# DEEPDIP-project/IncompressibleNavierStokes.jl

Measured on AMD Instinct MI355X. Metric: M lattice-cell updates/sec (RK4 step incl. Poisson), 3D TGV fp64, higher is better.
Workload: dtype f64; 1 GPU; TaylorGreenVortex3D 256^3 periodic fp64, RK44 + spectral Poisson, dt=0.001, Re=1e3; decomposition=single GPU, loop=timesteps_ (K steps, one native call)

## Files before the change

incompressiblenavierstokes.jl_amd/csrc/ins_fast3d_flux.hip:

```cpp
#include <algorithm>
#include <cstdlib>

#include "ins_internal.h"


namespace {

__global__ __launch_bounds__(256) void k_build_recs(GridDev g, double visc, Rec* __restrict__ r0, Rec* __restrict__ r1,
                                                    Rec* __restrict__ r2, int diffusion_only) {
  const int d = blockIdx.y;
  Rec* out = d == 0 ? r0 : (d == 1 ? r1 : r2);
  const int n = g.N[d];
  for (int idx = blockIdx.x * 256 + threadIdx.x; idx < n; idx += gridDim.x * 256) {
    const int ip = min(idx + 1, n - 1);
    Rec r;
    r.vs = visc * g.mdx[d][ip];
    r.vo = visc * g.mdxu[d][idx];
    r.a0 = 0.5 * g.A2[0][d][idx];
    r.b0 = 0.5 * g.A1[0][d][ip];
    r.a1 = 0.5 * g.A2[1][d][idx];
    r.b1 = 0.5 * g.A1[1][d][ip];
    r.a2 = 0.5 * g.A2[2][d][idx];
    r.b2 = 0.5 * g.A1[2][d][ip];
    r.rs = g.rdxu[d][idx];
// ... 334 lines not shown
      load_plane(B, k + 2);
      load_p(Pa, k + 3);
      if (bar) __builtin_amdgcn_s_barrier();
      body(Cc, A, k);
      if (++k >= k1) break;
      correct(B, Pb, Pa, k + 1);
      load_plane(Cc, k + 2);
      load_p(Pb, k + 3);
      if (bar) __builtin_amdgcn_s_barrier();
      body(A, B, k);
      if (++k >= k1) break;
    }
  }
}

__global__ __launch_bounds__(256) void k_zero_shell(GridDev g, double* __restrict__ F) {
  const int N0 = g.N[0], N1 = g.N[1], N2 = g.N[2];
  const long long nface_z = (long long)N0 * N1, nface_y = (long long)N0 * N2, nface_x = (long long)N1 * N2;
  const long long total = 2 * (nface_z + nface_y + nface_x);
  for (long long t = (long long)blockIdx.x * 256 + threadIdx.x; t < total; t += (long long)gridDim.x * 256) {
    long long r = t;
    long long c;
    if (r < 2 * nface_z) {
      const int side = r >= nface_z;
      r -= side * nface_z;
      c = r + (side ? (long long)(N2 - 1) * g.sx[2] : 0);
    } else if ((r -= 2 * nface_z) < 2 * nface_y) {
      const int side = r >= nface_y;
      r -= side * nface_y;
      const int ii = (int)(r % N0), kk = (int)(r / N0);
      c = ii + (side ? (long long)(N1 - 1) * g.sx[1] : 0) + kk * g.sx[2];
    } else {
      r -= 2 * nface_y;
      const int side = r >= nface_x;
      r -= side * nface_x;
      const int jj = (int)(r % N1), kk = (int)(r / N1);
      c = (side ? N0 - 1 : 0) + jj * g.sx[1] + kk * g.sx[2];
    }
    F[c] = 0.0;
    F[c + g.sc] = 0.0;
    F[c + 2 * g.sc] = 0.0;
  }
}

}

#define g_rows ((int)ins_opt(OPT_INS_FLUX_ROWS))
#define g_zchunk ((int)ins_opt(OPT_INS_FLUX_ZC))
#define g_xw ((int)ins_opt(OPT_INS_FLUX_XW))

extern "C" void ins_tune_flux3d(int rows, int zchunk, int xw) {
  ins_set_option("INS_FLUX_ROWS", (rows >= 2 && rows <= 4) ? rows : 0);
  ins_set_option("INS_FLUX_ZC", zchunk >= 1 ? zchunk : 0);
  ins_set_option("INS_FLUX_XW", (xw == 1 || xw == 2 || xw == 4) ? xw : 0);
}

int ins_flux3d_prepare(const ins_grid* G, double visc, hipStream_t s) {
  ins_grid* M = const_cast<ins_grid*>(G);
  const GridDev& g = G->g;
  if (!M->rec_dev) {
    const size_t n = (size_t)g.N[0] + g.N[1] + g.N[2];
    INS_HIP_TRY(hipMalloc(&M->rec_dev, n * sizeof(Rec)));
    M->rec_visc = -1.0;
  }
  if (M->rec_visc != visc) {
    Rec* r0 = reinterpret_cast<Rec*>(M->rec_dev);
    Rec* r1 = r0 + g.N[0];
    Rec* r2 = r1 + g.N[1];
    const int nmax = std::max(g.N[0], std::max(g.N[1], g.N[2]));
    hipLaunchKernelGGL(k_build_recs, dim3(cdiv(nmax, 256), 3), dim3(256), 0, s, g, visc, r0, r1, r2, 0);
    INS_LAUNCH_CHECK();
    M->rec_visc = visc;
  }
  return INS_OK;
}

template <int R, int XW, bool FUSE>
static int launch_flux(const ins_grid* G, const double* u, double* F, const RkEpi& epi, const double* pI, int corr_mode, hipStream_t s,
                       const void* recs = nullptr) {
  const GridDev& g = G->g;
  const Rec* r0 = reinterpret_cast<const Rec*>(recs ? recs : G->rec_dev);
  const Rec* r1 = r0 + g.N[0];
  const Rec* r2 = r1 + g.N[1];
  const int zc = g_zchunk ? g_zchunk : ((g.N[2] >= 384 || (pI && corr_mode == 3 && g.N[2] >= 128)) ? 8 : 4);
  const int bar = ins_opt(OPT_INS_FLUX_BAR) ? 1 : 0;
  const bool corr = pI != nullptr;
  const bool masked = !G->all_dof;
  constexpr int RC = R > 3 ? 3 : R;
  constexpr int RK = R > 2 ? 2 : R;
  const int reff = corr ? RK : (masked ? RC : R);
  const int xo = corr ? XOUT - 1 : XOUT;
  const int ntx = cdiv(g.N[0] - 2, xo * XW), nty = cdiv(g.N[1] - 2, (4 / XW) * reff), ntz = cdiv(g.N[2] - 2, zc);
  dim3 block(64, 4, 1);
  const unsigned nb = (unsigned)(8LL * ntx * ((nty + 7) / 8) * ntz);
  if (corr && corr_mode == 3) {
    if constexpr (FUSE) {
      constexpr int R3 = R > 2 ? 2 : R;
      const int nty3 = cdiv(g.N[1] - 2, (4 / XW) * R3), ntx3 = cdiv(g.N[0] - 2, (XOUT - 1) * XW);
      const unsigned nb3 = (unsigned)(8LL * ntx3 * ((nty3 + 7) / 8) * ntz);
      hipLaunchKernelGGL((k_momentum_flux<R3, false, true, XW, true, 3>), dim3(nb3), block, 0, s, g, r0, r1, r2, u, F, zc, ntx3, nty3, ntz, epi, pI, bar);
      INS_LAUNCH_CHECK();
      return INS_OK;
    } else {
      ins_set_error("in-kernel pressure correction needs the fused epilogue");
      return INS_ERR_UNSUPPORTED;
    }
  } else if (corr) {
    if (!(FUSE && G->uniform_exact && !masked)) {
      ins_set_error("in-kernel pressure correction needs the fused path on an exactly uniform periodic grid");
      return INS_ERR_UNSUPPORTED;
    }
    if constexpr (FUSE)
      {
        if (corr_mode == 2)
          hipLaunchKernelGGL((k_momentum_flux<RK, true, false, XW, true, 2>), dim3(nb), block, 0, s, g, r0, r1, r2, u, F, zc, ntx, nty, ntz, epi, pI, bar);
        else
          hipLaunchKernelGGL((k_momentum_flux<RK, true, false, XW, true, 1>), dim3(nb), block, 0, s, g, r0, r1, r2, u, F, zc, ntx, nty, ntz, epi, pI, bar);
      }
  } else if (G->uniform_exact && !masked)
    hipLaunchKernelGGL((k_momentum_flux<R, true, false, XW, FUSE, 0>), dim3(nb), block, 0, s, g, r0, r1, r2, u, F, zc, ntx, nty, ntz, epi, pI, bar);
  else if (!masked)
    hipLaunchKernelGGL((k_momentum_flux<R, false, false, XW, FUSE, 0>), dim3(nb), block, 0, s, g, r0, r1, r2, u, F, zc, ntx, nty, ntz, epi, pI, bar);
  else
    hipLaunchKernelGGL((k_momentum_flux<RC, false, true, XW, FUSE, 0>), dim3(nb), block, 0, s, g, r0, r1, r2, u, F, zc, ntx, nty, ntz, epi, pI, bar);
  INS_LAUNCH_CHECK();
  return INS_OK;
}

template <bool FUSE>
static int launch_flux_any(const ins_grid* G, const double* u, double* F, const RkEpi& epi, const double* pI, int corr_mode, hipStream_t s,
                           const void* recs = nullptr) {
  const int waves_x = cdiv(G->g.N[0] - 2, pI ? XOUT - 1 : XOUT);
  int xw = g_xw;
  if (!xw) {
    xw = waves_x >= 8 ? 4 : (waves_x >= 2 ? 2 : 1);
    while (xw > 1 && cdiv(waves_x, xw) * xw > waves_x) xw >>= 1;
  }
  const int rows = g_rows ? g_rows : 4;
#define INS_FLUX_CASE(RR)                                                          \
  if (rows == RR) {                                                                \
    if (xw == 4) return launch_flux<RR, 4, FUSE>(G, u, F, epi, pI, corr_mode, s, recs);  \
    if (xw == 2) return launch_flux<RR, 2, FUSE>(G, u, F, epi, pI, corr_mode, s, recs);  \
    return launch_flux<RR, 1, FUSE>(G, u, F, epi, pI, corr_mode, s, recs);               \
  }
  INS_FLUX_CASE(2)
  INS_FLUX_CASE(3)
  INS_FLUX_CASE(4)
#undef INS_FLUX_CASE
  return INS_ERR_INVALID;
}

bool ins_flux64_supported(const ins_grid* G);
int ins_k_flux64(const ins_grid* G, double visc, const double* u, double* F, const RkEpi* epi, const double* pI, int corr_mode, hipStream_t s,
                 int part = 0);

int ins_k_momentum_flux3d(const ins_grid* G, double visc, const double* u, double* F, bool zero_shell, hipStream_t s) {
  int rc;
  const long long from62 = ins_opt(OPT_INS_FLUX64_62_FROM);
  if (ins_flux64_supported(G) && (from62 <= 0 || G->g.N[0] - 2 < from62)) {
    if ((rc = ins_k_flux64(G, visc, u, F, nullptr, nullptr, 0, s))) return rc;
  } else {
    if ((rc = ins_flux3d_prepare(G, visc, s))) return rc;
    RkEpi epi;
    memset(&epi, 0, sizeof(epi));
    if ((rc = launch_flux_any<false>(G, u, F, epi, nullptr, 0, s))) return rc;
  }
  if (zero_shell) {
    const GridDev& g = G->g;
    const long long total = 2LL * ((long long)g.N[0] * g.N[1] + (long long)g.N[0] * g.N[2] + (long long)g.N[1] * g.N[2]);
    hipLaunchKernelGGL(k_zero_shell, dim3((unsigned)std::min<long long>((total + 255) / 256, 2048)), dim3(256), 0, s, g, F);
    INS_LAUNCH_CHECK();
  }
  return INS_OK;
}

bool ins_fast3d_supported(const ins_grid* G);
int ins_k_diffusion_flux3d(const ins_grid* G, double visc, const double* u, double* F, bool zero_shell, hipStream_t s) {
  const GridDev& g = G->g;
  if (!ins_fast3d_supported(G)) return INS_ERR_UNSUPPORTED;
  ins_grid* M = const_cast<ins_grid*>(G);
  if (!M->rec_diff_dev) {
    const size_t n = (size_t)g.N[0] + g.N[1] + g.N[2];
    INS_HIP_TRY(hipMalloc(&M->rec_diff_dev, n * sizeof(Rec)));
    M->rec_diff_visc = -1.0;
  }
  if (M->rec_diff_visc != visc) {
    Rec* r0 = reinterpret_cast<Rec*>(M->rec_diff_dev);
    Rec* r1 = r0 + g.N[0];
    Rec* r2 = r1 + g.N[1];
    const int nmax = std::max(g.N[0], std::max(g.N[1], g.N[2]));
    hipLaunchKernelGGL(k_build_recs, dim3(cdiv(nmax, 256), 3), dim3(256), 0, s, g, visc, r0, r1, r2, 1);
    INS_LAUNCH_CHECK();
    M->rec_diff_visc = visc;
  }
  RkEpi epi;
  memset(&epi, 0, sizeof(epi));
  int rc = launch_flux_any<false>(G, u, F, epi, nullptr, 0, s, M->rec_diff_dev);
  if (rc || !zero_shell) return rc;
  const long long total = 2LL * ((long long)g.N[0] * g.N[1] + (long long)g.N[0] * g.N[2] + (long long)g.N[1] * g.N[2]);
  hipLaunchKernelGGL(k_zero_shell, dim3((unsigned)std::min<long long>((total + 255) / 256, 2048)), dim3(256), 0, s, g, F);
  INS_LAUNCH_CHECK();
  return INS_OK;
}

bool ins_flux64m_supported(const ins_grid* G);
int ins_k_flux64m(const ins_grid* G, double visc, const double* u, double* k_out, const RkEpi& epi, const double* p_padded, hipStream_t s);

int ins_k_momentum_rk_fused(const ins_grid* G, double visc, const double* u_in, double* k_out, const RkEpi& epi, hipStream_t s) {
  if (ins_flux64_supported(G)) return ins_k_flux64(G, visc, u_in, k_out, &epi, nullptr, 0, s);
  if ((!ins_opt(OPT_INS_FLUX64M_SKIP_FIRST) || epi.wout) && ins_flux64m_supported(G)) return ins_k_flux64m(G, visc, u_in, k_out, epi, nullptr, s);
  int rc = ins_flux3d_prepare(G, visc, s);
  if (rc) return rc;
  return launch_flux_any<true>(G, u_in, k_out, epi, nullptr, 0, s);
}

int ins_k_momentum_rk_fused_corr(const ins_grid* G, double visc, const double* ustar_prev, const double* pI, double* k_out, const RkEpi& epi,
                                 hipStream_t s) {
  if (ins_flux64_supported(G)) return ins_k_flux64(G, visc, ustar_prev, k_out, &epi, pI, 1, s);
  int rc = ins_flux3d_prepare(G, visc, s);
  if (rc) return rc;
  return launch_flux_any<true>(G, ustar_prev, k_out, epi, pI, 1, s);
}

bool ins_fast3d_supported(const ins_grid* G);
bool ins_corr3_supported(const ins_grid* G) {
  const GridDev& g = G->g;
  if (g.D != 3 || !ins_fast3d_supported(G) || g.N[0] < 8 || g.N[1] < 8 || g.N[2] < 8) return false;
  for (int a = 0; a < 3; ++a)
    for (int sd = 0; sd < 2; ++sd)
      if (g.bc[a][sd] != INS_BC_PERIODIC && g.bc[a][sd] != INS_BC_DIRICHLET) return false;
  return true;
}
int ins_k_momentum_rk_fused_corr3(const ins_grid* G, double visc, const double* ustar_prev, const double* p_padded, double* k_out, const RkEpi& epi,
                                  hipStream_t s) {
  if (ins_flux64m_supported(G)) return ins_k_flux64m(G, visc, ustar_prev, k_out, epi, p_padded, s);
  int rc = ins_flux3d_prepare(G, visc, s);
  if (rc) return rc;
  return launch_flux_any<true>(G, ustar_prev, k_out, epi, p_padded, 3, s);
}

int ins_k_momentum_rk_fused_corr_slab(const ins_grid* G, double visc, const double* ustar_prev, const double* p_ext, double* k_out,
                                      const RkEpi& epi, hipStream_t s, int part) {
  if (ins_flux64_supported(G)) return ins_k_flux64(G, visc, ustar_prev, k_out, &epi, p_ext, 2, s, part);
  if (part == 1) return INS_OK;
  int rc = ins_flux3d_prepare(G, visc, s);
  if (rc) return rc;
  return launch_flux_any<true>(G, ustar_prev, k_out, epi, p_ext, 2, s);
}
```

incompressiblenavierstokes.jl_amd/csrc/ins_fft.hip:

```cpp
#include <cmath>

#include "ins_internal.h"

namespace {

template <typename C>
struct real_of;
template <>
struct real_of<double2> {
  using t = double;
};
template <>
struct real_of<float2> {
  using t = float;
};
template <typename C>
using real_t = typename real_of<C>::t;
template <typename C>
__device__ __forceinline__ C mkc(real_t<C> x, real_t<C> y) {
  C c;
  c.x = x;
  c.y = y;
  return c;
}
template <typename C>
__device__ __forceinline__ C cmul(C a, C b) { return mkc<C>(a.x * b.x - a.y * b.y, a.x * b.y + a.y * b.x); }
template <typename C>
__device__ __forceinline__ C cmulc(C a, C b) { return mkc<C>(a.x * b.x + a.y * b.y, a.y * b.x - a.x * b.y); }
template <typename C>
__device__ __forceinline__ C cadd(C a, C b) { return mkc<C>(a.x + b.x, a.y + b.y); }
template <typename C>
__device__ __forceinline__ C csub(C a, C b) { return mkc<C>(a.x - b.x, a.y - b.y); }
template <typename C>
__device__ __forceinline__ C mul_mi(C a) { return mkc<C>(a.y, -a.x); }
template <typename C>
__device__ __forceinline__ C mul_pi(C a) { return mkc<C>(-a.y, a.x); }

constexpr int fft_r3(int code) { return code >= 64 ? 5 : (code >= 32 ? 3 : 1); }
constexpr int fft_lg(int code) { return code & 31; }
constexpr int fft_len(int code) { return fft_r3(code) << fft_lg(code); }

template <int LOGN>
__host__ __device__ __forceinline__ int pos_of_freq(int k) {
  constexpr int LG = fft_lg(LOGN), R3 = fft_r3(LOGN);
  constexpr bool ODD = LG & 1;
  int p = 0, L = 1 << LG;
  if (R3 != 1) {
    p = (k % R3) * L;
    k /= R3;
  }
  if (ODD) {
    p += (k & 1) * (L / 2);
    k >>= 1;
    L /= 2;
  }
#pragma unroll
  for (int s = 0; s < LG / 2; ++s) {
    p += (k & 3) * (L / 4);
    k >>= 2;
    L /= 4;
  }
  return p;
}

template <int LOGN>
constexpr bool fft_swz_on() { return fft_r3(LOGN) == 1 && fft_len(LOGN) % 256 == 0; }
template <bool ON>
__host__ __device__ __forceinline__ int fft_swz(int i) {
  return ON ? ((i & ~15) | ((i + ((i >> 4) & 3) + 4 * ((i >> 6) & 3)) & 15)) : i;
}
__device__ __forceinline__ int fft_swz_g(int gg) { return (gg & ~15) | ((gg & 3) << 2) | ((gg >> 2) & 3); }

template <bool INV, typename C>
__device__ __forceinline__ void bfly3(C& x0, C& x1, C& x2) {
  using T = real_t<C>;
  constexpr T h = (T)0.86602540378443864676;
  const C t1 = cadd(x1, x2), d = csub(x1, x2);
  const C t2 = mkc<C>(x0.x - (T)0.5 * t1.x, x0.y - (T)0.5 * t1.y);
  const C t3 = INV ? mkc<C>(-h * d.y, h * d.x) : mkc<C>(h * d.y, -h * d.x);
  x0 = cadd(x0, t1);
  x1 = cadd(t2, t3);
  x2 = csub(t2, t3);
}

template <bool INV, typename C>
__device__ __forceinline__ void bfly5(C& x0, C& x1, C& x2, C& x3, C& x4) {
  using T = real_t<C>;
  constexpr T c1 = (T)0.30901699437494742410, c2 = (T)-0.80901699437494742410;
  constexpr T s1 = (T)0.95105651629515357212, s2 = (T)0.58778525229247312917;
  const C a = cadd(x1, x4), b = cadd(x2, x3), d = csub(x1, x4), e = csub(x2, x3);
  const C m1 = mkc<C>(x0.x + c1 * a.x + c2 * b.x, x0.y + c1 * a.y + c2 * b.y);
  const C m2 = mkc<C>(x0.x + c2 * a.x + c1 * b.x, x0.y + c2 * a.y + c1 * b.y);
  const C u = mkc<C>(s1 * d.x + s2 * e.x, s1 * d.y + s2 * e.y), v = mkc<C>(s2 * d.x - s1 * e.x, s2 * d.y - s1 * e.y);
  const C iu = INV ? mkc<C>(-u.y, u.x) : mkc<C>(u.y, -u.x), iv = INV ? mkc<C>(-v.y, v.x) : mkc<C>(v.y, -v.x);
  x0 = mkc<C>(x0.x + a.x + b.x, x0.y + a.y + b.y);
  x1 = cadd(m1, iu);
  x4 = csub(m1, iu);
  x2 = cadd(m2, iv);
  x3 = csub(m2, iv);
}

template <int LOGN, int NC, int SR, int SC, bool RFAST, int NT = 256, typename C>
__device__ __forceinline__ void fft_dif(C* __restrict__ buf, const C* __restrict__ tw, int t) {
  constexpr int N = fft_len(LOGN), R3 = fft_r3(LOGN), M = N / R3;
  constexpr bool ODD = fft_lg(LOGN) & 1;
  if (R3 == 3) {
    for (int w = t; w < M * NC; w += NT) {
      const int c = RFAST ? w / M : w % NC, j = RFAST ? w % M : w / NC;
      C* x = buf + c * SC;
      C a0 = x[j * SR], a1 = x[(j + M) * SR], a2 = x[(j + 2 * M) * SR];
      bfly3<false>(a0, a1, a2);
      x[j * SR] = a0;
      x[(j + M) * SR] = cmul(a1, tw[j]);
      x[(j + 2 * M) * SR] = cmul(a2, tw[2 * j]);
    }
    __syncthreads();
  }
  if (R3 == 5) {
    for (int w = t; w < M * NC; w += NT) {
      const int c = RFAST ? w / M : w % NC, j = RFAST ? w % M : w / NC;
      C* x = buf + c * SC;
      C a0 = x[j * SR], a1 = x[(j + M) * SR], a2 = x[(j + 2 * M) * SR], a3 = x[(j + 3 * M) * SR], a4 = x[(j + 4 * M) * SR];
      bfly5<false>(a0, a1, a2, a3, a4);
      x[j * SR] = a0;
      x[(j + M) * SR] = cmul(a1, tw[j]);
      x[(j + 2 * M) * SR] = cmul(a2, tw[2 * j]);
      x[(j + 3 * M) * SR] = cmul(a3, tw[3 * j]);
      x[(j + 4 * M) * SR] = cmul(a4, tw[4 * j]);
    }
    __syncthreads();
  }
  constexpr bool SWZ = RFAST && fft_swz_on<LOGN>();
  int L = M;
  if (ODD) {
    for (int w = t; w < (N / 2) * NC; w += NT) {
      const int c = RFAST ? w / (N / 2) : w % NC, jj = RFAST ? w % (N / 2) : w / NC;
      const int sub = jj / (M / 2), j = jj - sub * (M / 2);
      C* x = buf + c * SC + sub * M * SR;
      const int i0 = fft_swz<SWZ>(j) * SR, i1 = fft_swz<SWZ>(j + M / 2) * SR;
      const C a0 = x[i0], a1 = x[i1];
      x[i0] = cadd(a0, a1);
      x[i1] = cmul(csub(a0, a1), tw[fft_swz<SWZ>(j * R3)]);
    }
    L = M / 2;
    __syncthreads();
  }
#pragma unroll 1
  for (; L >= 4; L >>= 2) {
    const int Q = L / 4, step = N / L;
    for (int w = t; w < (N / 4) * NC; w += NT) {
      const int c = RFAST ? w / (N / 4) : w % NC, bb = RFAST ? w % (N / 4) : w / NC;
      const int sub = bb / (M / 4), b = bb - sub * (M / 4);
// ... 4 lines not shown
      const int e = g * L + j;
      const int i0 = fft_swz<SWZ>(e) * SR, i1 = fft_swz<SWZ>(e + Q) * SR, i2 = fft_swz<SWZ>(e + 2 * Q) * SR, i3 = fft_swz<SWZ>(e + 3 * Q) * SR;
      const C a0 = x[i0], a1 = x[i1], a2 = x[i2], a3 = x[i3];
      const C t0 = cadd(a0, a2), t1 = csub(a0, a2), t2 = cadd(a1, a3), t3 = mul_mi(csub(a1, a3));
      C y1 = cadd(t1, t3), y2 = csub(t0, t2), y3 = csub(t1, t3);
      if (L > 4) {
        const C w1 = tw[fft_swz<SWZ>(j * step)], w2 = cmul(w1, w1), w3 = cmul(w2, w1);
        y1 = cmul(y1, w1);
        y2 = cmul(y2, w2);
        y3 = cmul(y3, w3);
      }
      x[i0] = cadd(t0, t2);
      x[i1] = y1;
      x[i2] = y2;
      x[i3] = y3;
    }
    __syncthreads();
  }
}

template <int LOGN, int NC, int SR, int SC, bool RFAST, int NT = 256, typename C>
__device__ __forceinline__ void fft_dit(C* __restrict__ buf, const C* __restrict__ tw, int t) {
  constexpr int N = fft_len(LOGN), R3 = fft_r3(LOGN), M = N / R3;
  constexpr bool ODD = fft_lg(LOGN) & 1;
  constexpr bool SWZ = RFAST && fft_swz_on<LOGN>();
#pragma unroll 1
  for (int L = 4; L <= (ODD ? M / 2 : M); L <<= 2) {
    const int Q = L / 4, step = N / L;
    for (int w = t; w < (N / 4) * NC; w += NT) {
      const int c = RFAST ? w / (N / 4) : w % NC, bb = RFAST ? w % (N / 4) : w / NC;
      const int sub = bb / (M / 4), b = bb - sub * (M / 4);
      int g = b / Q;
      const int j = b - g * Q;
      if (SWZ && Q == 4) g = fft_swz_g(g);
      C* x = buf + c * SC + sub * M * SR;
      const int e = g * L + j;
      const int i0 = fft_swz<SWZ>(e) * SR, i1 = fft_swz<SWZ>(e + Q) * SR, i2 = fft_swz<SWZ>(e + 2 * Q) * SR, i3 = fft_swz<SWZ>(e + 3 * Q) * SR;
      C x0 = x[i0], x1 = x[i1], x2 = x[i2], x3 = x[i3];
      if (L > 4) {
        const C w1 = tw[fft_swz<SWZ>(j * step)], w2 = cmul(w1, w1), w3 = cmul(w2, w1);
        x1 = cmulc(x1, w1);
        x2 = cmulc(x2, w2);
        x3 = cmulc(x3, w3);
      }
      const C t0 = cadd(x0, x2), t1 = csub(x0, x2), t2 = cadd(x1, x3), t3 = mul_pi(csub(x1, x3));
      x[i0] = cadd(t0, t2);
      x[i1] = cadd(t1, t3);
      x[i2] = csub(t0, t2);
      x[i3] = csub(t1, t3);
    }
    __syncthreads();
  }
  if (ODD) {
    for (int w = t; w < (N / 2) * NC; w += NT) {
      const int c = RFAST ? w / (N / 2) : w % NC, jj = RFAST ? w % (N / 2) : w / NC;
      const int sub = jj / (M / 2), j = jj - sub * (M / 2);
      C* x = buf + c * SC + sub * M * SR;
      const int i0 = fft_swz<SWZ>(j) * SR, i1 = fft_swz<SWZ>(j + M / 2) * SR;
      const C x0 = x[i0], x1 = cmulc(x[i1], tw[fft_swz<SWZ>(j * R3)]);
      x[i0] = cadd(x0, x1);
      x[i1] = csub(x0, x1);
    }
    __syncthreads();
  }
  if (R3 == 3) {
    for (int w = t; w < M * NC; w += NT) {
      const int c = RFAST ? w / M : w % NC, j = RFAST ? w % M : w / NC;
      C* x = buf + c * SC;
      C a0 = x[j * SR], a1 = cmulc(x[(j + M) * SR], tw[j]), a2 = cmulc(x[(j + 2 * M) * SR], tw[2 * j]);
      bfly3<true>(a0, a1, a2);
      x[j * SR] = a0;
      x[(j + M) * SR] = a1;
      x[(j + 2 * M) * SR] = a2;
    }
    __syncthreads();
  }
  if (R3 == 5) {
    for (int w = t; w < M * NC; w += NT) {
      const int c = RFAST ? w / M : w % NC, j = RFAST ? w % M : w / NC;
      C* x = buf + c * SC;
      C a0 = x[j * SR], a1 = cmulc(x[(j + M) * SR], tw[j]), a2 = cmulc(x[(j + 2 * M) * SR], tw[2 * j]), a3 = cmulc(x[(j + 3 * M) * SR], tw[3 * j]),
        a4 = cmulc(x[(j + 4 * M) * SR], tw[4 * j]);
      bfly5<true>(a0, a1, a2, a3, a4);
      x[j * SR] = a0;
      x[(j + M) * SR] = a1;
      x[(j + 2 * M) * SR] = a2;
      x[(j + 3 * M) * SR] = a3;
      x[(j + 4 * M) * SR] = a4;
    }
    __syncthreads();
  }
}

struct PackMap {
  double2* packed;
  int nyl, nzl, cw;
};

template <int LOGN, int TK, bool INVERSE, bool PACKED, typename C = double2>
__global__ __launch_bounds__(256) void k_yfft(C* __restrict__ data, int kxn, int kxs, const C* __restrict__ tw_g, PackMap pm) {
  constexpr int N = fft_len(LOGN);
  extern __shared__ __align__(16) unsigned char lds_raw[];
  C* lds_dyn = reinterpret_cast<C*>(lds_raw);
  C* buf = lds_dyn;
  C* tw = lds_dyn + N * TK;
  const int t = threadIdx.x;
  const int col = t % TK;
  const int kx = blockIdx.x * TK + col;
  const bool live = kx < kxn;
  C* base = data + (long long)blockIdx.y * N * kxs + kx;
  long long pbase = 0, prow = 0, pq = 0;
  if (PACKED) {
    const int c = kx / pm.cw, kxl = kx - c * pm.cw;
    const int kxc = min(pm.cw, kxn - c * pm.cw);
    const long long nranks = N / pm.nyl;
    pbase = nranks * pm.nzl * pm.nyl * (long long)(c * pm.cw) + kxl + (long long)kxc * pm.nyl * blockIdx.y;
    prow = kxc;
    pq = (long long)kxc * pm.nyl * pm.nzl;
  }
  auto paddr = [&](int r) {
    const int q = r / pm.nyl, kyl = r - q * pm.nyl;
    return pbase + prow * kyl + pq * q;
  };
  for (int m = t; m < N; m += 256) tw[m] = tw_g[m];
  constexpr int RPT = 256 / TK;
  constexpr int NIT = N / RPT;
  {
    C v[NIT];
#pragma unroll
    for (int q = 0; q < NIT; ++q) {
      const int r = t / TK + q * RPT;
      v[q] = mkc<C>(0.0, 0.0);
      if (live) v[q] = (PACKED && INVERSE) ? static_cast<C*>((void*)pm.packed)[paddr(r)] : base[(long long)r * kxs];
    }
#pragma unroll
    for (int q = 0; q < NIT; ++q) buf[(t / TK + q * RPT) * TK + col] = v[q];
  }
  __syncthreads();
  if (INVERSE)
    fft_dit<LOGN, TK, TK, 1, false>(buf, tw, t);
  else
    fft_dif<LOGN, TK, TK, 1, false>(buf, tw, t);
  if (live)
#pragma unroll
    for (int q = 0; q < NIT; ++q) {
      const int r = t / TK + q * RPT;
      if (PACKED && !INVERSE)
        static_cast<C*>((void*)pm.packed)[paddr(r)] = buf[r * TK + col];
      else
        base[(long long)r * kxs] = buf[r * TK + col];
    }
}

template <int LOGN, int NP, int SRC, typename C = double2>
__global__ __launch_bounds__(256) void k_xfwd(GridDev g, const double* __restrict__ src, C* __restrict__ out, int n1,
                                              const C* __restrict__ tw_g, int kxs, int kz0, int skel) {
  using T = real_t<C>;
  constexpr int N = fft_len(LOGN);
  constexpr int KXN = N / 2 + 1;
  extern __shared__ __align__(16) unsigned char lds_raw[];
  C* lds_dyn = reinterpret_cast<C*>(lds_raw);
  C* buf = lds_dyn;
  C* tw = lds_dyn + NP * N;
  const int t = threadIdx.x;
  const int kz = kz0 + blockIdx.y;
  const int j0 = blockIdx.x * 2 * NP;
  constexpr bool SWZ = fft_swz_on<LOGN>();
  for (int m = t; m < N; m += 256) tw[fft_swz<SWZ>(m)] = tw_g[m];
  T* bufd = reinterpret_cast<T*>(buf);
  constexpr int NIT = (2 * NP * N) / 256;
  {
    T v[NIT];
#pragma unroll
    for (int q = 0; q < NIT; ++q) {
      const int idx = t + 256 * q;
      const int row = idx / N, i = idx - row * N;
      const int j = min(j0 + row, n1 - 1);
      if (SRC == 0) {
        v[q] = reinterpret_cast<const T*>(src)[i + (long long)N * (j + (long long)n1 * kz)];
      } else if (SRC == 6) {
        v[q] = (T)src[(g.ip_lo[0] + i) + (g.ip_lo[1] + j) * g.sx[1] + (g.ip_lo[2] + kz) * g.sx[2]];
      } else if (SRC == 5) {
        const float* sf = reinterpret_cast<const float*>(src);
        const int I0 = i + 1, I1 = j + 1, I2 = kz + 1;
        const long long c = I0 + I1 * g.sx[1] + I2 * g.sx[2];
        const long long cx = I0 == 1 ? c + (long long)(g.N[0] - 3) : c - 1;
        const long long cy = I1 == 1 ? c + (long long)(g.N[1] - 3) * g.sx[1] : c - g.sx[1];
        const long long cz = I2 == 1 ? c + (long long)(g.N[2] - 3) * g.sx[2] : c - g.sx[2];
        double d = ((double)sf[c] - (double)sf[cx]) * g.rdx[0][I0];
        d += ((double)sf[g.sc + c] - (double)sf[g.sc + cy]) * g.rdx[1][I1];
        d += ((double)sf[2 * g.sc + c] - (double)sf[2 * g.sc + cz]) * g.rdx[2][I2];
        v[q] = (T)(d * (g.dx[0][I0] * g.dx[1][I1] * g.dx[2][I2]));
      } else if (SRC == 4) {
        const int I0 = g.ip_lo[0] + i, I1 = g.ip_lo[1] + j, I2 = g.ip_lo[2] + kz;
        const long long c = I0 + I1 * g.sx[1] + I2 * g.sx[2];
        double d = (src[c] - src[c - 1]) * g.rdx[0][I0];
        d += (src[g.sc + c] - src[g.sc + c - g.sx[1]]) * g.rdx[1][I1];
        d += (src[2 * g.sc + c] - src[2 * g.sc + c - g.sx[2]]) * g.rdx[2][I2];
        v[q] = (T)(d * (g.dx[0][I0] * g.dx[1][I1] * g.dx[2][I2]));
      } else if (SRC == 3) {
        const int I0 = i + 1, I1 = j + 1;
        const long long c = I0 + I1 * g.sx[1];
        const long long cx = I0 == 1 ? c + (long long)(g.N[0] - 3) : c - 1;
        const long long cy = I1 == 1 ? c + (long long)(g.N[1] - 3) * g.sx[1] : c - g.sx[1];
        const double d = (src[c] - src[cx]) * g.rdx[0][I0] + (src[g.sc + c] - src[g.sc + cy]) * g.rdx[1][I1];
        v[q] = (T)(d * (g.dx[0][I0] * g.dx[1][I1]));
      } else {
        const int I0 = i + 1, I1 = j + 1, I2 = kz + 1;
        const long long c = I0 + I1 * g.sx[1] + I2 * g.sx[2];
        const long long cx = I0 == 1 ? c + (long long)(g.N[0] - 3) : c - 1;
        const long long cy = I1 == 1 ? c + (long long)(g.N[1] - 3) * g.sx[1] : c - g.sx[1];
        const long long cz = (SRC == 1 && I2 == 1) ? c + (long long)(g.N[2] - 3) * g.sx[2] : c - g.sx[2];
        double d = 0.0;
        d += (src[c] - src[cx]) * g.rdx[0][I0];
        d += (src[g.sc + c] - src[g.sc + cy]) * g.rdx[1][I1];
        d += (src[2 * g.sc + c] - src[2 * g.sc + cz]) * g.rdx[2][I2];
        const double om = g.dx[0][I0] * g.dx[1][I1] * g.dx[2][I2];
        v[q] = (T)(d * om);
      }
    }
#pragma unroll
    for (int q = 0; q < NIT; ++q) {
      const int idx = t + 256 * q;
      const int row = idx / N, i = idx - row * N;
      bufd[2 * ((row >> 1) * N + fft_swz<SWZ>(i)) + (row & 1)] = (j0 + row < n1) ? v[q] : (T)0;
    }
  }
  __syncthreads();
  if (!skel) fft_dif<LOGN, NP, 1, N, true>(buf, tw, t);
  for (int idx = t; idx < NP * KXN; idx += 256) {
    const int p = idx / KXN, s = idx - p * KXN;
    const int j = j0 + 2 * p;
    if (j >= n1) continue;
    const C zk = buf[p * N + fft_swz<SWZ>(pos_of_freq<LOGN>(s))];
    const C zm = buf[p * N + fft_swz<SWZ>(pos_of_freq<LOGN>((N - s) % N))];
    const C a = mkc<C>((T)0.5 * (zk.x + zm.x), (T)0.5 * (zk.y - zm.y));
    const C b = mkc<C>((T)0.5 * (zk.y + zm.y), (T)-0.5 * (zk.x - zm.x));
    const long long o = s + (long long)kxs * (j + (long long)n1 * kz);
    out[o] = a;
    out[o + kxs] = b;
  }
}

template <int LOGN, int NP, typename C = double2>
__global__ __launch_bounds__(256) void k_xinv(const C* __restrict__ in, real_t<C>* __restrict__ pI, int n1,
                                              const C* __restrict__ tw_g, int kxs, int skel) {
  using T = real_t<C>;
  constexpr int N = fft_len(LOGN);
  constexpr int KXN = N / 2 + 1;
  extern __shared__ __align__(16) unsigned char lds_raw[];
  C* lds_dyn = reinterpret_cast<C*>(lds_raw);
  C* buf = lds_dyn;
  C* tw = lds_dyn + NP * N;
  const int t = threadIdx.x;
  const int kz = blockIdx.y;
  const int j0 = blockIdx.x * 2 * NP;
  constexpr bool SWZ = fft_swz_on<LOGN>();
  for (int m = t; m < N; m += 256) tw[fft_swz<SWZ>(m)] = tw_g[m];
  constexpr int NIT = (NP * KXN + 255) / 256;
  {
    C av[NIT], bv[NIT];
#pragma unroll
    for (int q = 0; q < NIT; ++q) {
      const int idx = min(t + 256 * q, NP * KXN - 1);
      const int p = idx / KXN, s = idx - p * KXN;
      const int j = min(j0 + 2 * p, n1 - 2);
      const long long o = s + (long long)kxs * (j + (long long)n1 * kz);
      av[q] = in[o];
      bv[q] = in[o + kxs];
    }
#pragma unroll
    for (int q = 0; q < NIT; ++q) {
      const int idx = t + 256 * q;
      if (idx >= NP * KXN) break;
      const int p = idx / KXN, s = idx - p * KXN;
      C a = av[q], b = bv[q];
      if (j0 + 2 * p >= n1) a = b = mkc<C>(0, 0);
      if (s == 0 || s == N / 2) {
        a.y = 0;
        b.y = 0;
      }
      buf[p * N + fft_swz<SWZ>(pos_of_freq<LOGN>(s))] = mkc<C>(a.x - b.y, a.y + b.x);
      if (s != 0 && s != N / 2) buf[p * N + fft_swz<SWZ>(pos_of_freq<LOGN>(N - s))] = mkc<C>(a.x + b.y, b.x - a.y);
    }
  }
  __syncthreads();
  if (!skel) fft_dit<LOGN, NP, 1, N, true>(buf, tw, t);
  const T* bufd = reinterpret_cast<const T*>(buf);
  for (int idx = t; idx < 2 * NP * N; idx += 256) {
    const int row = idx / N, i = idx - row * N;
    const int j = j0 + row;
    if (j < n1) pI[i + (long long)N * (j + (long long)n1 * kz)] = bufd[2 * ((row >> 1) * N + fft_swz<SWZ>(i)) + (row & 1)];
  }
}

struct FdmZArgs {
  double2* data;
  long long nl;
  int n0h;
  const double *lx, *ly;
  const double* lz;
  const double2* wq;
  const double *ox, *oy;
  double h, tol;
  int singular;
  const double* meanf;
  double* partial;
};

template <int LOGN, int TK, bool DCT = false>
__global__ __launch_bounds__(256) void k_fdm_z(FdmZArgs a, const double2* __restrict__ tw_g) {
  constexpr int N = fft_len(LOGN);
  extern __shared__ double2 lds_dyn[];
  double2* buf = lds_dyn;
  double2* tw = lds_dyn + N * TK;
  __shared__ double red[4];
  const int t = threadIdx.x;
  const int col = t % TK;
  const long long line = (long long)blockIdx.x * TK + col;
  const bool live = line < a.nl;
  for (int m = t; m < N; m += 256) tw[m] = tw_g[m];
  constexpr int RPT = 256 / TK;
  constexpr int NIT = N / RPT;
  {
    double2 v[NIT];
#pragma unroll
    for (int q = 0; q < NIT; ++q) v[q] = live ? a.data[(long long)(t / TK + q * RPT) * a.nl + line] : make_double2(0.0, 0.0);
#pragma unroll
    for (int q = 0; q < NIT; ++q) {
      const int z = t / TK + q * RPT;
      const int r = DCT ? ((z & 1) ? N - 1 - (z >> 1) : (z >> 1)) : z;
      buf[r * TK + col] = v[q];
    }
  }
  __syncthreads();
  fft_dif<LOGN, TK, TK, 1, false>(buf, tw, t);
  __syncthreads();
  const double mf = a.singular ? *a.meanf : 0.0;
  const double inv = 1.0 / (a.h * (double)N);
  double acc = 0.0;
  for (int idx = t; idx < (N / 2 + 1) * TK; idx += 256) {
    const int c = idx % TK, k = idx / TK;
    const long long ln = (long long)blockIdx.x * TK + c;
    if (ln >= a.nl) continue;
    const int m = (int)(ln % a.n0h), j = (int)(ln / a.n0h);
    const int ia = 2 * m, ib = ia + 1;
    const int pk = pos_of_freq<LOGN>(k), pm = pos_of_freq<LOGN>((N - k) % N);
    const double2 zk = buf[pk * TK + c], zm = buf[pm * TK + c];
    const bool self = k == 0 || k == N / 2;
    double2 A = self ? make_double2(zk.x, 0.0) : make_double2(0.5 * (zk.x + zm.x), 0.5 * (zk.y - zm.y));
    double2 B = self ? make_double2(zk.y, 0.0) : make_double2(0.5 * (zk.y + zm.y), -0.5 * (zk.x - zm.x));
    if constexpr (DCT) {
      const double2 w = a.wq[k];
      const double2 ya = cmul(A, w), yb = cmul(B, w);
      double ca[2] = {ya.x, -ya.y}, cb[2] = {yb.x, -yb.y};
      const int kk[2] = {k, N - k};
#pragma unroll
      for (int q = 0; q < 2; ++q) {
        if (q == 1 && self) {
          ca[1] = k == 0 ? 0.0 : ca[0];
          cb[1] = k == 0 ? 0.0 : cb[0];
          break;
        }
        const double lyz = a.ly[j] + a.lz[kk[q]];
        const double la = a.lx[ia] + lyz, lb = a.lx[ib] + lyz;
        if (a.singular) {
          const double oa = a.ox[ia] * a.oy[j], ob = a.ox[ib] * a.oy[j];
          if (kk[q] == 0) {
            ca[q] -= mf * oa * (double)N;
            cb[q] -= mf * ob * (double)N;
          }
          ca[q] *= fabs(la) <= a.tol ? 0.0 : 1.0 / la;
          cb[q] *= fabs(lb) <= a.tol ? 0.0 : 1.0 / lb;
          if (kk[q] == 0) acc += (oa * ca[q] + ob * cb[q]) / a.h;
        } else {
          ca[q] /= la;
          cb[q] /= lb;
        }
      }
      const double2 wc = make_double2(w.x, -w.y);
      A = cmul(make_double2(ca[0], -ca[1]), wc);
      B = cmul(make_double2(cb[0], -cb[1]), wc);
      buf[pk * TK + c] = make_double2(inv * (A.x - B.y), inv * (A.y + B.x));
      if (!self) buf[pm * TK + c] = make_double2(inv * (A.x + B.y), inv * (B.x - A.y));
      continue;
    }
    const double lyz = a.ly[j] + a.lz[k];
    const double la = a.lx[ia] + lyz, lb = a.lx[ib] + lyz;
    if (a.singular) {
      const double oa = a.ox[ia] * a.oy[j], ob = a.ox[ib] * a.oy[j];
      if (k == 0) {
        A.x -= mf * oa * (double)N;
        B.x -= mf * ob * (double)N;
      }
      const double sa = fabs(la) <= a.tol ? 0.0 : 1.0 / la, sb = fabs(lb) <= a.tol ? 0.0 : 1.0 / lb;
      A.x *= sa;
      A.y *= sa;
      B.x *= sb;
      B.y *= sb;
      if (k == 0) acc += (oa * A.x + ob * B.x) / a.h;
    } else {
      A.x /= la;
      A.y /= la;
      B.x /= lb;
      B.y /= lb;
    }
    buf[pk * TK + c] = make_double2(inv * (A.x - B.y), inv * (A.y + B.x));
    if (!self) buf[pm * TK + c] = make_double2(inv * (A.x + B.y), inv * (B.x - A.y));
  }
  __syncthreads();
  fft_dit<LOGN, TK, TK, 1, false>(buf, tw, t);
  __syncthreads();
  if (live)
#pragma unroll
    for (int q = 0; q < NIT; ++q) {
      const int z = t / TK + q * RPT;
      const int r = DCT ? ((z & 1) ? N - 1 - (z >> 1) : (z >> 1)) : z;
      a.data[(long long)z * a.nl + line] = buf[r * TK + col];
    }
  if (a.singular) {
#pragma unroll
    for (int off = 32; off > 0; off >>= 1) acc += __shfl_down(acc, off, 64);
    if ((t & 63) == 0) red[t >> 6] = acc;
    __syncthreads();
    if (t == 0) a.partial[blockIdx.x] = red[0] + red[1] + red[2] + red[3];
  }
}

template <typename K>
int set_lds(K kernel, size_t lds) {
  if (lds > 64 * 1024) INS_HIP_TRY(hipFuncSetAttribute(reinterpret_cast<const void*>(kernel), hipFuncAttributeMaxDynamicSharedMemorySize, (int)lds));
  return INS_OK;
}

template <int LOGN, typename C = double2>
int launch_y(C* data, int kxn, int kxs, int nplanes, const C* tw, bool inverse, const PackMap* pm, hipStream_t s) {
  constexpr int N = fft_len(LOGN);
  constexpr int TK = (N <= 256 ? 16 : (N <= 512 ? 8 : 4)) * (int)(sizeof(double2) / sizeof(C));
  constexpr size_t lds = ((size_t)N * TK + N) * sizeof(C);
  dim3 grid((kxn + TK - 1) / TK, nplanes);
  PackMap none{nullptr, 1, 1, 1};
#define INS_Y_LAUNCH(INV, PK)                                                                                   \
  do {                                                                                                          \
    int rc = set_lds(&k_yfft<LOGN, TK, INV, PK, C>, lds);                                                       \
    if (rc) return rc;                                                                                          \
    hipLaunchKernelGGL((k_yfft<LOGN, TK, INV, PK, C>), grid, dim3(256), lds, s, data, kxn, kxs, tw, pm ? *pm : none);   \
  } while (0)
  if constexpr (sizeof(C) == sizeof(double2)) {
    if (pm) {
      if (inverse)
        INS_Y_LAUNCH(true, true);
      else
        INS_Y_LAUNCH(false, true);
      INS_LAUNCH_CHECK();
      return INS_OK;
    }
  }
  if (inverse)
    INS_Y_LAUNCH(true, false);
  else
    INS_Y_LAUNCH(false, false);
#undef INS_Y_LAUNCH
  INS_LAUNCH_CHECK();
  return INS_OK;
}

template <int LOGN>
int launch_xfwd(const GridDev& g, const double* src, int from_u, double2* out, int n1, int n2, const double2* tw, int kxs, hipStream_t s, int kz0) {
  constexpr int N = fft_len(LOGN);
  constexpr int NP = fft_r3(LOGN) == 5 ? 640 / N : (fft_r3(LOGN) == 3 ? 768 / N : (N >= 1024 ? 2 : (1024 / N > 16 ? 16 : 1024 / N)));
  constexpr size_t lds = ((size_t)NP * N + N) * sizeof(double2);
  dim3 grid((n1 + 2 * NP - 1) / (2 * NP), n2);
  if (from_u == 6)
    hipLaunchKernelGGL((k_xfwd<LOGN, NP, 6>), grid, dim3(256), lds, s, g, src, out, n1, tw, kxs, kz0, (int)ins_opt(OPT_INS_X_SKEL));
  else if (from_u == 5)
    hipLaunchKernelGGL((k_xfwd<LOGN, NP, 5>), grid, dim3(256), lds, s, g, src, out, n1, tw, kxs, kz0, (int)ins_opt(OPT_INS_X_SKEL));
  else if (from_u == 4)
    hipLaunchKernelGGL((k_xfwd<LOGN, NP, 4>), grid, dim3(256), lds, s, g, src, out, n1, tw, kxs, kz0, (int)ins_opt(OPT_INS_X_SKEL));
  else if (from_u == 3)
    hipLaunchKernelGGL((k_xfwd<LOGN, NP, 3>), grid, dim3(256), lds, s, g, src, out, n1, tw, kxs, kz0, (int)ins_opt(OPT_INS_X_SKEL));
  else if (from_u == 2)
    hipLaunchKernelGGL((k_xfwd<LOGN, NP, 2>), grid, dim3(256), lds, s, g, src, out, n1, tw, kxs, kz0, (int)ins_opt(OPT_INS_X_SKEL));
  else if (from_u)
    hipLaunchKernelGGL((k_xfwd<LOGN, NP, 1>), grid, dim3(256), lds, s, g, src, out, n1, tw, kxs, kz0, (int)ins_opt(OPT_INS_X_SKEL));
  else
    hipLaunchKernelGGL((k_xfwd<LOGN, NP, 0>), grid, dim3(256), lds, s, g, src, out, n1, tw, kxs, kz0, (int)ins_opt(OPT_INS_X_SKEL));
  INS_LAUNCH_CHECK();
  return INS_OK;
}
template <int LOGN>
int launch_xfwd32(const GridDev& g, const float* src, int from_u, float2* out, int n1, int n2, const float2* tw, int kxs, hipStream_t s) {
  constexpr int N = fft_len(LOGN);
  constexpr int NP = fft_r3(LOGN) == 5 ? 640 / N : (fft_r3(LOGN) == 3 ? 768 / N : (N >= 1024 ? 2 : (1024 / N > 16 ? 16 : 1024 / N)));
  constexpr size_t lds = ((size_t)NP * N + N) * sizeof(float2);
  dim3 grid((n1 + 2 * NP - 1) / (2 * NP), n2);
  const double* srcd = reinterpret_cast<const double*>(src);
  if (from_u)
    hipLaunchKernelGGL((k_xfwd<LOGN, NP, 5, float2>), grid, dim3(256), lds, s, g, srcd, out, n1, tw, kxs, 0, (int)ins_opt(OPT_INS_X_SKEL));
  else
    hipLaunchKernelGGL((k_xfwd<LOGN, NP, 0, float2>), grid, dim3(256), lds, s, g, srcd, out, n1, tw, kxs, 0, (int)ins_opt(OPT_INS_X_SKEL));
  INS_LAUNCH_CHECK();
  return INS_OK;
}

template <int LOGN, typename C = double2>
int launch_xinv(const C* in, real_t<C>* pI, int n1, int n2, const C* tw, int kxs, hipStream_t s) {
  constexpr int N = fft_len(LOGN);
  constexpr int NP = fft_r3(LOGN) == 5 ? 640 / N : (fft_r3(LOGN) == 3 ? 768 / N : (N >= 1024 ? 2 : (1024 / N > 16 ? 16 : 1024 / N)));
  constexpr size_t lds = ((size_t)NP * N + N) * sizeof(C);
  dim3 grid((n1 + 2 * NP - 1) / (2 * NP), n2);
  hipLaunchKernelGGL((k_xinv<LOGN, NP, C>), grid, dim3(256), lds, s, in, pI, n1, tw, kxs, (int)ins_opt(OPT_INS_X_SKEL));
  INS_LAUNCH_CHECK();
  return INS_OK;
}


struct YzArgs {
  double2* data;
  int kxn, kxs, n2, m, P;
  const double* ax;
  const double* ay;
  double c, scale;
  double2* edges;
  long long stride;
  double2* bc;
  double2* sol0;
  int skel;
};

__device__ __forceinline__ double yz_rcp(double x) {
  const double y = __builtin_amdgcn_rcp(x);
  return y * (2.0 - x * y);
}

template <int LOGN, int TK, int NT, int B, int PF>
__global__ __launch_bounds__(NT) void k_yz_fwd(YzArgs a, const double2* __restrict__ tw_g) {
  constexpr int N = fft_len(LOGN);
  constexpr int RPT = NT / TK, NIT = N / RPT;
  constexpr int NC = TK * B;
  static_assert(N % RPT == 0 && NIT >= 1, "tile shape");
  extern __shared__ __align__(16) unsigned char lds_raw[];
  double2* buf = reinterpret_cast<double2*>(lds_raw);
  double2* tw = buf + N * NC;
  const int t = threadIdx.x, col = t % TK, r0 = t / TK;
  const int kx = blockIdx.x * TK + col;
  const bool live = kx < a.kxn;
  const int part = blockIdx.y, z0 = part * a.m;
  const long long ps = (long long)N * a.kxs;
  double2* base = a.data + (long long)z0 * ps + kx;
  for (int i = t; i < N; i += NT) tw[i] = tw_g[i];
  const long long lines = (long long)N * a.kxn;
  double r_[NIT], pa[NIT];
  double2 gp[NIT], SA[NIT];
  bool sing[NIT];
#pragma unroll
  for (int q = 0; q < NIT; ++q) {
    const int row = r0 + q * RPT;
    const double sxy = live ? a.ax[kx] + a.ay[row] : 1.0;
    sing[q] = sxy == 0.0;
    const double sc = sing[q] ? 1.0 : sxy / a.c;
    const double sq = sqrt(sc * (4.0 + sc));
    const double lnr = -log1p(0.5 * (sc + sq));
    r_[q] = exp(lnr);
    pa[q] = r_[q];
    gp[q] = make_double2(0.0, 0.0);
    SA[q] = gp[q];
  }
  const int R = a.m / B;
  auto load_round = [&](double2 (&v)[B][NIT], int r) {
    const int rc = min(r, R - 1);
#pragma unroll
    for (int b = 0; b < B; ++b)
#pragma unroll
      for (int q = 0; q < NIT; ++q)
        if (live) v[b][q] = base[(long long)(rc * B + b) * ps + (long long)(r0 + q * RPT) * a.kxs];
  };
  auto pin = [&](double2 (&v)[B][NIT]) {
#pragma unroll
    for (int b = 0; b < B; ++b)
#pragma unroll
      for (int q = 0; q < NIT; ++q) asm volatile("" ::"v"(v[b][q].x), "v"(v[b][q].y));
  };
  auto round = [&](double2 (&v)[B][NIT], double2 (&vnext)[B][NIT], int r) {
#pragma unroll
    for (int b = 0; b < B; ++b)
#pragma unroll
      for (int q = 0; q < NIT; ++q) buf[(r0 + q * RPT) * NC + b * TK + col] = v[b][q];
    __syncthreads();
    load_round(v, r + PF);
    if (a.skel != 1) fft_dif<LOGN, NC, NC, 1, false, NT>(buf, tw, t);
    pin(vnext);
    if (live) {
#pragma unroll
      for (int b = 0; b < B; ++b) {
        const int k = r * B + b;
#pragma unroll
        for (int q = 0; q < NIT; ++q) {
          const int row = r0 + q * RPT;
          double2 g = buf[row * NC + b * TK + col];
          g.x *= a.scale;
          g.y *= a.scale;
          double2 out = g;
          if (sing[q]) {
            a.edges[(long long)part * a.stride + 2 * lines + k] = g;
          } else if (a.skel != 2) {
            const double rr = r_[q], E = pa[q] * pa[q];
            const double inv = (rr / a.c) * (1.0 - E) * yz_rcp(1.0 - E * rr * rr);
            gp[q].x = inv * (g.x + a.c * gp[q].x);
            gp[q].y = inv * (g.y + a.c * gp[q].y);
            SA[q].x += pa[q] * g.x;
            SA[q].y += pa[q] * g.y;
            pa[q] *= rr;
            out = gp[q];
          }
          base[(long long)k * ps + (long long)row * a.kxs] = out;
        }
      }
    }
    __syncthreads();
  };
  double2 va[B][NIT], vb[B][NIT];
#pragma unroll
  for (int b = 0; b < B; ++b)
#pragma unroll
    for (int q = 0; q < NIT; ++q) va[b][q] = vb[b][q] = make_double2(0.0, 0.0);
  load_round(va, 0);
  if constexpr (PF == 2) {
    load_round(vb, 1);
    for (int r = 0; r < R; r += 2) {
      round(va, vb, r);
      round(vb, va, r + 1);
    }
  } else {
    for (int r = 0; r < R; ++r) round(va, va, r);
  }
  if (live) {
    double2* e = a.edges + (long long)part * a.stride;
#pragma unroll
    for (int q = 0; q < NIT; ++q) {
      const long long l = (long long)(r0 + q * RPT) * a.kxn + kx;
      if (sing[q]) {
        e[l] = e[lines + l] = make_double2(0.0, 0.0);
      } else {
        const double lnr = log(r_[q]);
        const double rm1 = exp((a.m + 1.0) * lnr);
        const double idc = 1.0 / (-expm1((2.0 * a.m + 2.0) * lnr) * a.c);
        const double f = idc * (1.0 - rm1 * rm1);
        e[l] = make_double2(f * SA[q].x - rm1 * gp[q].x, f * SA[q].y - rm1 * gp[q].y);
        e[lines + l] = gp[q];
      }
    }
  }
}
// ... 434 lines not shown
  }
  __syncthreads();
  fft_dit<LX, NP, 1, N0, true, NT>(bufx, twx, t);
  for (int idx = t; idx < N1 * N0; idx += NT) {
    const int j = idx / N0, i = idx - j * N0;
    pI[i + (long long)N0 * j] = bufd[2 * ((j >> 1) * N0 + i) + (j & 1)];
  }
}

template <int LX, int LY>
int launch_xysolve2d(const GridDev& g, const double* src, int from_u, double* pI, const double2* twx, const double2* twy, const double* ax, const double* ay,
                     hipStream_t s) {
  constexpr int N0 = 1 << LX, N1 = 1 << LY, KXN = N0 / 2 + 1;
  constexpr int NT = N0 * N1 >= 2048 ? 1024 : 256;
  constexpr size_t lds = ((size_t)(N1 / 2) * N0 + (size_t)N1 * KXN + N0 + N1) * sizeof(double2);
  const double inv_n = 1.0 / ((double)N0 * N1);
  int rc;
  if (from_u) {
    if ((rc = set_lds(&k_xysolve2d<LX, LY, 3, NT>, lds))) return rc;
    hipLaunchKernelGGL((k_xysolve2d<LX, LY, 3, NT>), dim3(1), dim3(NT), lds, s, g, src, pI, twx, twy, ax, ay, inv_n);
  } else {
    if ((rc = set_lds(&k_xysolve2d<LX, LY, 0, NT>, lds))) return rc;
    hipLaunchKernelGGL((k_xysolve2d<LX, LY, 0, NT>), dim3(1), dim3(NT), lds, s, g, src, pI, twx, twy, ax, ay, inv_n);
  }
  INS_LAUNCH_CHECK();
  return INS_OK;
}

template <int LX, int LY>
int launch_xy(const GridDev& g, const double* src, int from_u, double2* spec, double* pI, int n2, const double2* twx, const double2* twy, int kxs,
              bool inverse, hipStream_t s) {
  constexpr int N0 = 1 << LX, N1 = 1 << LY, KXN = N0 / 2 + 1;
  constexpr int NT = N0 * N1 >= 2048 ? 1024 : 256;
  constexpr size_t lds = ((size_t)(N1 / 2) * N0 + (size_t)N1 * KXN + N0 + N1) * sizeof(double2);
  int rc;
  if (inverse) {
    if ((rc = set_lds(&k_xyinv<LX, LY, NT>, lds))) return rc;
    hipLaunchKernelGGL((k_xyinv<LX, LY, NT>), dim3(n2), dim3(NT), lds, s, spec, pI, twx, twy, kxs);
  } else if (from_u) {
    if ((rc = set_lds(&k_xyfwd<LX, LY, 1, NT>, lds))) return rc;
    hipLaunchKernelGGL((k_xyfwd<LX, LY, 1, NT>), dim3(n2), dim3(NT), lds, s, g, src, spec, twx, twy, kxs);
  } else {
    if ((rc = set_lds(&k_xyfwd<LX, LY, 0, NT>, lds))) return rc;
    hipLaunchKernelGGL((k_xyfwd<LX, LY, 0, NT>), dim3(n2), dim3(NT), lds, s, g, src, spec, twx, twy, kxs);
  }
  INS_LAUNCH_CHECK();
  return INS_OK;
}

}

#define INS_POW2_SWITCH(n, CALL)            \
  switch (n) {                              \
    case 16: return CALL(4);                \
    case 32: return CALL(5);                \
    case 64: return CALL(6);                \
    case 128: return CALL(7);               \
    case 256: return CALL(8);               \
    case 512: return CALL(9);               \
    case 1024: return CALL(10);             \
    case 96: return CALL(32 + 5);           \
    case 192: return CALL(32 + 6);          \
    case 384: return CALL(32 + 7);          \
    case 160: return CALL(64 + 5);          \
    case 320: return CALL(64 + 6);          \
    case 640: return CALL(64 + 7);          \
  }                                         \
  ins_set_error("own FFT: unsupported length %d", n); \
  return INS_ERR_UNSUPPORTED;

bool ins_ownfft_supported(const int np[3]) {
  if (ins_opt(OPT_INS_DISABLE_OWNFFT)) return false;
  for (int a = 0; a < 3; ++a)
    if (np[a] < 16 || np[a] > 1024 || (np[a] & (np[a] - 1))) return false;
  return ins_zsolve_supported(np[2]);
}
bool ins_ownfft_supported_slab(const int np[3]) {
  if (ins_opt(OPT_INS_DISABLE_OWNFFT)) return false;
  for (int a = 0; a < 2; ++a) {
    const bool pow2 = np[a] >= 16 && np[a] <= 1024 && !(np[a] & (np[a] - 1));
    const bool r3 = (np[a] == 96 || np[a] == 192 || np[a] == 384 || np[a] == 160 || np[a] == 320 || np[a] == 640) && !ins_opt(OPT_INS_OWNFFT_POW2_ONLY);
    if (!pow2 && !r3) return false;
  }
  return np[2] >= 2;
}
bool ins_ownfft_supported_mixed(const int np[3]) {
  if (ins_opt(OPT_INS_DISABLE_OWNFFT)) return false;
  for (int a = 0; a < 3; ++a) {
    const bool pow2 = np[a] >= 16 && np[a] <= 1024 && !(np[a] & (np[a] - 1));
    const bool r3 = (np[a] == 96 || np[a] == 192 || np[a] == 384 || np[a] == 160 || np[a] == 320 || np[a] == 640) && !ins_opt(OPT_INS_OWNFFT_POW2_ONLY);
    if (!pow2 && !r3) return false;
  }
  return ins_zsolve_supported(np[2]);
}

void ins_ownfft_permute_symbol(int n, const double* ay, double* out) {
  const int r3 = (n % 5 == 0) ? 5 : ((n % 3 == 0) ? 3 : 1), m = n / r3;
  int logm = 0;
  while ((1 << logm) < m) ++logm;
  for (int k = 0; k < n; ++k) {
    int p = 0, kk = k, L = m;
    if (r3 != 1) {
      p = (kk % r3) * m;
      kk /= r3;
    }
    if (logm & 1) {
      p += (kk & 1) * (L / 2);
      kk >>= 1;
      L /= 2;
    }
    for (int s = 0; s < logm / 2; ++s) {
      p += (kk & 3) * (L / 4);
      kk >>= 2;
      L /= 4;
    }
    out[p] = ay[k];
  }
}

bool ins_ownfft_xy_supported(int n0, int n1) {
  auto small = [](int n) { return n == 16 || n == 32 || n == 64; };
  return !ins_opt(OPT_INS_DISABLE_XYFUSED) && small(n0) && small(n1);
}
int ins_k_ownfft_xy(const ins_grid* G, const double* src, int from_u, double* phat, double* pI, int n0, int n1, int n2, const double* twx, const double* twy,
                    bool inverse, hipStream_t s, int kxs) {
  static const GridDev no_grid{};
  const GridDev& g = G ? G->g : no_grid;
  double2* sp = reinterpret_cast<double2*>(phat);
  const double2 *wx = reinterpret_cast<const double2*>(twx), *wy = reinterpret_cast<const double2*>(twy);
  auto lg = [](int n) { return n == 16 ? 4 : (n == 32 ? 5 : 6); };
#define INS_XY(A, B) \
  if (lg(n0) == A && lg(n1) == B) return launch_xy<A, B>(g, src, from_u, sp, pI, n2, wx, wy, kxs, inverse, s);
  INS_XY(4, 4) INS_XY(4, 5) INS_XY(4, 6) INS_XY(5, 4) INS_XY(5, 5) INS_XY(5, 6) INS_XY(6, 4) INS_XY(6, 5) INS_XY(6, 6)
#undef INS_XY
  ins_set_error("ins_k_ownfft_xy: unsupported plane %d x %d", n0, n1);
  return INS_ERR_UNSUPPORTED;
}

int ins_k_ownfft_xysolve2d(const ins_grid* G, const double* src, int from_u, double* pI, int n0, int n1, const double* twx, const double* twy, const double* ax,
                           const double* ay, hipStream_t s) {
  static const GridDev no_grid{};
  const GridDev& g = G ? G->g : no_grid;
  const double2 *wx = reinterpret_cast<const double2*>(twx), *wy = reinterpret_cast<const double2*>(twy);
  auto lg = [](int n) { return n == 16 ? 4 : (n == 32 ? 5 : 6); };
#define INS_XY(A, B) \
  if (lg(n0) == A && lg(n1) == B) return launch_xysolve2d<A, B>(g, src, from_u, pI, wx, wy, ax, ay, s);
  INS_XY(4, 4) INS_XY(4, 5) INS_XY(4, 6) INS_XY(5, 4) INS_XY(5, 5) INS_XY(5, 6) INS_XY(6, 4) INS_XY(6, 5) INS_XY(6, 6)
#undef INS_XY
  ins_set_error("ins_k_ownfft_xysolve2d: unsupported grid %d x %d", n0, n1);
  return INS_ERR_UNSUPPORTED;
}

int ins_k_ownfft_xfwd(const ins_grid* G, const double* src, int from_u, double* phat, int n0, int n1, int n2, const double* tw,
                      hipStream_t s, int kxs, int kz0) {
  if (kxs <= 0) kxs = n0 / 2 + 1;
  static const GridDev no_grid{};
  const GridDev& g = G ? G->g : no_grid;
  double2* out = reinterpret_cast<double2*>(phat);
  const double2* w = reinterpret_cast<const double2*>(tw);
#define CALL(LG) launch_xfwd<LG>(g, src, from_u, out, n1, n2, w, kxs, s, kz0)
  INS_POW2_SWITCH(n0, CALL)
#undef CALL
}

int ins_k_ownfft_xinv(const double* phat, double* pI, int n0, int n1, int n2, const double* tw, hipStream_t s, int kxs) {
  if (kxs <= 0) kxs = n0 / 2 + 1;
  const double2* in = reinterpret_cast<const double2*>(phat);
  const double2* w = reinterpret_cast<const double2*>(tw);
#define CALL(LG) launch_xinv<LG>(in, pI, n1, n2, w, kxs, s)
  INS_POW2_SWITCH(n0, CALL)
#undef CALL
}

int ins_ownfft_yz_partitions(int kxn, int n1, int n2) {
  if (ins_opt(OPT_INS_DISABLE_YZ_FUSED)) return 0;
  if (!ins_opt(OPT_INS_YZ_FUSED) && !ins_opt(OPT_INS_YZ_PARTITIONS)) return 0;
  if (!(n1 == 128 || n1 == 256 || n1 == 512) || n2 < 64 || (n2 & (n2 - 1))) return 0;
  const int forced = (int)ins_opt(OPT_INS_YZ_PARTITIONS);
  if (forced == 2 || forced == 4 || forced == 8 || forced == 16) return (n2 % forced == 0 && (n2 / forced) % 4 == 0) ? forced : 0;
  const int tiles = (kxn + 7) / 8;
  int P = 2;
  while (P < 16 && tiles * P < 240 && n2 / (2 * P) >= 8) P *= 2;
  return tiles * P >= 128 ? P : 0;
}
long long ins_ownfft_yz_scratch(int kxn, int n1, int n2, int P) {
  const long long lines = (long long)n1 * kxn;
  return (long long)P * (2 * lines + n2 / P) + (long long)P * 2 * lines + n2;
}
int ins_k_ownfft_yz_solve(double* phat, int kxn, int n1, int n2, int kxs, int P, const double* ax, const double* ay, double c, double scale, const double* tw_y,
                          double* scratch, hipStream_t s) {
  YzArgs a;
  a.data = reinterpret_cast<double2*>(phat);
  a.kxn = kxn;
  a.kxs = kxs;
  a.n2 = n2;
  a.m = n2 / P;
  a.P = P;
  a.ax = ax;
  a.ay = ay;
  a.c = c;
  a.scale = scale;
  const long long lines = (long long)n1 * kxn;
  a.stride = 2 * lines + a.m;
  a.edges = reinterpret_cast<double2*>(scratch);
  a.bc = a.edges + (long long)P * a.stride;
  a.sol0 = a.bc + (long long)P * 2 * lines;
  a.skel = (int)ins_opt(OPT_INS_YZ_SKEL);
  const double2* w = reinterpret_cast<const double2*>(tw_y);
  switch (n1) {
    case 128: return launch_yz<7>(a, w, s);
    case 256: return launch_yz<8>(a, w, s);
    case 512: return launch_yz<9>(a, w, s);
  }
  ins_set_error("fused y/z passes: unsupported length %d", n1);
  return INS_ERR_UNSUPPORTED;
}

int ins_k_ownfft_y(double* phat, int kxn, int n1, int n2, const double* tw, bool inverse, hipStream_t s, int kxs) {
  if (kxs <= 0) kxs = kxn;
  double2* d = reinterpret_cast<double2*>(phat);
  const double2* w = reinterpret_cast<const double2*>(tw);
#define CALL(LG) launch_y<LG>(d, kxn, kxs, n2, w, inverse, nullptr, s)
  INS_POW2_SWITCH(n1, CALL)
#undef CALL
}

int ins_k_ownfft_xfwd_f32(const ins_grid* G, const float* src, int from_u, float* phat, int n0, int n1, int n2, const float* tw, hipStream_t s, int kxs) {
  static const GridDev no_grid{};
  const GridDev& g = G ? G->g : no_grid;
  float2* out = reinterpret_cast<float2*>(phat);
  const float2* w = reinterpret_cast<const float2*>(tw);
#define CALL(LG) launch_xfwd32<LG>(g, src, from_u, out, n1, n2, w, kxs, s)
  INS_POW2_SWITCH(n0, CALL)
#undef CALL
}
int ins_k_ownfft_xinv_f32(const float* phat, float* pI, int n0, int n1, int n2, const float* tw, hipStream_t s, int kxs) {
  const float2* in = reinterpret_cast<const float2*>(phat);
  const float2* w = reinterpret_cast<const float2*>(tw);
#define CALL(LG) launch_xinv<LG, float2>(in, pI, n1, n2, w, kxs, s)
  INS_POW2_SWITCH(n0, CALL)
#undef CALL
}
int ins_k_ownfft_y_f32(float* phat, int kxn, int n1, int n2, const float* tw, bool inverse, hipStream_t s, int kxs) {
  float2* d = reinterpret_cast<float2*>(phat);
  const float2* w = reinterpret_cast<const float2*>(tw);
#define CALL(LG) launch_y<LG, float2>(d, kxn, kxs, n2, w, inverse, nullptr, s)
  INS_POW2_SWITCH(n1, CALL)
#undef CALL
}

int ins_k_ownfft_y_packed(double* phat, double* packed, int kxn, int n1, int nzl, int nyl, int cw, const double* tw, bool inverse,
                          hipStream_t s) {
  double2* d = reinterpret_cast<double2*>(phat);
  const double2* w = reinterpret_cast<const double2*>(tw);
  PackMap pm{reinterpret_cast<double2*>(packed), nyl, nzl, cw};
#define CALL(LG) launch_y<LG>(d, kxn, kxn, nzl, w, inverse, &pm, s)
  INS_POW2_SWITCH(n1, CALL)
#undef CALL
}

int ins_k_fdm_z(double* data, int n0, int n1, int nz, const double* lx, const double* ly, const double* lz, const double* ox, const double* oy,
                double h, double tol, int singular, const double* meanf, double* partial, const double* tw, int* nblk, hipStream_t s, const double* dct_w) {
  FdmZArgs a;
  a.wq = reinterpret_cast<const double2*>(dct_w);
  a.data = reinterpret_cast<double2*>(data);
  a.n0h = n0 / 2;
  a.nl = (long long)a.n0h * n1;
  a.lx = lx; a.ly = ly; a.lz = lz; a.ox = ox; a.oy = oy;
  a.h = h; a.tol = tol; a.singular = singular; a.meanf = meanf; a.partial = partial;
  constexpr int TK = 8;
  const unsigned nb = (unsigned)((a.nl + TK - 1) / TK);
  if (nblk) *nblk = (int)nb;
  const double2* w = reinterpret_cast<const double2*>(tw);
#define INS_FDMZ(LOG)                                                                                          \
  {                                                                                                             \
    const size_t lds = ((size_t)(1 << LOG) * TK + (1 << LOG)) * sizeof(double2);                                \
    if (dct_w) {                                                                                                \
      int rc = set_lds(&k_fdm_z<LOG, TK, true>, lds);                                                           \
      if (rc) return rc;                                                                                        \
      hipLaunchKernelGGL((k_fdm_z<LOG, TK, true>), dim3(nb), dim3(256), lds, s, a, w);                          \
    } else {                                                                                                    \
      int rc = set_lds(&k_fdm_z<LOG, TK>, lds);                                                                 \
      if (rc) return rc;                                                                                        \
      hipLaunchKernelGGL((k_fdm_z<LOG, TK>), dim3(nb), dim3(256), lds, s, a, w);                                \
    }                                                                                                           \
    break;                                                                                                      \
  }
  switch (nz) {
    case 32: INS_FDMZ(5)
    case 64: INS_FDMZ(6)
    case 128: INS_FDMZ(7)
    case 256: INS_FDMZ(8)
    case 512: INS_FDMZ(9)
    default: ins_set_error("ins_k_fdm_z: unsupported nz = %d", nz); return INS_ERR_UNSUPPORTED;
  }
#undef INS_FDMZ
  INS_LAUNCH_CHECK();
  return INS_OK;
}
```

incompressiblenavierstokes.jl_amd/csrc/ins_flux64.hip:

```cpp
#include <algorithm>
#include <cstdlib>
#include <cstring>

#include "ins_internal.h"
#include "ins_wave64.h"
#include "ins_flux_common.h"

namespace {

template <typename T, int R>
struct Plane {
  T v[3][R + 2];
  T h[3];
  T raw[3][R];
};

template <typename T, int R>
struct TExt {
  T t[R + 2];
  T th;
  T vm1;
};

template <typename T, int R, int XW, bool FUSE, int CORR, bool SKEL = false, int NW = 4, bool EXTRA = false>
// ... 383 lines not shown
        Wo = Wc;
      }
      C.v[0][rr] = ldb<T>(n0r, ucol, urow[rr]);
      C.v[1][rr] = ldb<T>(n1r, ucol, urow[rr]);
      C.v[2][rr] = ldb<T>(n2r, ucol, urow[rr]);
    }
    C.v[0][R + 1] = ldb<T>(n0r, ucol, urow[R + 1]);
    C.v[1][R + 1] = ldb<T>(n1r, ucol, urow[R + 1]);
    C.v[2][R + 1] = ldb<T>(n2r, ucol, urow[R + 1]);
    C.h[0] = ldb<T>(n0r, uhoff, 0);
    C.h[1] = ldb<T>(n1r, uhoff, 0);
    C.h[2] = ldb<T>(n2r, uhoff, 0);
    if constexpr (TMK) {
      if (tm) {
        hU_prev = ch0;
        CT.t[R + 1] = ldb<T>(ntr, ucol, urow[R + 1]);
        CT.th = ldb<T>(ntr, uhoff, 0);
        CT.vm1 = ldb<T>(n1r, ucol, urowm1);
      }
    }
  };

  Plane<T, R> P0, P1;
  TExt<T, R> TE0, TE1;
  if (!CORR) {
    load_plane(P0, k0 - 1);
    load_plane(P1, k0);
    zflux0(P0, P1);
    if constexpr (EXTRA) {
#pragma unroll
      for (int c = 0; c < 3; ++c)
#pragma unroll
        for (int rr = 0; rr < R; ++rr) Pz[c][rr] = P0.v[c][rr + 1];
      if (a.tm) {
        load_text(TE0, k0 - 1);
        load_text(TE1, k0);
        PzV0 = P0.v[1][0];
        hU_prev = P0.h[0];
        const rsrc_t rw = plane_rsrc(a_u + (long long)uplane(max(k0 - 2, 0)) * sz + 2 * a.sc, ubytes);
#pragma unroll
        for (int rr = 1; rr <= R; ++rr) {
          const T Wc = P0.v[2][rr], Wm2 = ldb<T>(rw, ucol, urow[rr]);
          const T Wn = next_h(Wc, rdlane(P0.h[2], 16 + rr)), Wp = prev_h(Wc, rdlane(P0.h[2], rr));
          wwprev[rr - 1] = k0 > 1 ? Wc * ((Wn + Wp - 2 * Wc) * nux + (P0.v[2][rr + 1] + P0.v[2][rr - 1] - 2 * Wc) * nuy + (P1.v[2][rr] + Wm2 - 2 * Wc) * nuz) : (T)0;
          Tz[rr - 1] = TE0.t[rr];
        }
      }
    }
    load_plane(P0, min(k0 + 1, k1));
    if constexpr (EXTRA) {
      if (a.tm) load_text(TE0, min(k0 + 1, k1));
    }
    int k = k0;
    while (true) {
      if (a.bar) __builtin_amdgcn_s_barrier();
      body(P1, P0, TE1, TE0, k, min(k + 2, k1));
      if (++k >= k1) break;
      if (a.bar) __builtin_amdgcn_s_barrier();
      body(P0, P1, TE0, TE1, k, min(k + 2, k1));
      if (++k >= k1) break;
    }
  } else {
    T Pa[R + 3], Pb[R + 3], Ha, Hb;
    load_p(Pa, Ha, k0 - 1);
    load_p(Pb, Hb, k0);
    load_plane(P0, k0 - 1);
    load_plane(P1, k0);
    correct(P0, Pa, Ha, Pb, Hb);
    load_p(Pa, Ha, k0 + 1);
    correct(P1, Pb, Hb, Pa, Ha);
    zflux0(P0, P1);
    if constexpr (EXTRA) {
#pragma unroll
      for (int c = 0; c < 3; ++c)
#pragma unroll
        for (int rr = 0; rr < R; ++rr) Pz[c][rr] = P0.v[c][rr + 1];
    }
    load_plane(P0, min(k0 + 1, k1));
    load_p(Pb, Hb, min(k0 + 2, k1 + 1));
    int k = k0;
    while (true) {
      if (a.bar) __builtin_amdgcn_s_barrier();
      correct(P0, Pa, Ha, Pb, Hb);
      load_p(Pa, Ha, min(k + 3, k1 + 1));
      body(P1, P0, TE1, TE0, k, min(k + 2, k1));
      if (++k >= k1) break;
      if (a.bar) __builtin_amdgcn_s_barrier();
      correct(P1, Pb, Hb, Pa, Ha);
      load_p(Pb, Hb, min(k + 3, k1 + 1));
      body(P0, P1, TE0, TE1, k, min(k + 2, k1));
      if (++k >= k1) break;
    }
  }
}

#define g_disable ((int)ins_opt(OPT_INS_DISABLE_FLUX64))
#define g_rows ((int)ins_opt(OPT_INS_FLUX64_ROWS))
#define g_rows_corr ((int)ins_opt(OPT_INS_FLUX64_ROWS_CORR))
#define g_zchunk ((int)ins_opt(OPT_INS_FLUX64_ZC))
#define g_zchunk_corr ((int)ins_opt(OPT_INS_FLUX64_ZC_CORR))
#define g_xw ((int)ins_opt(OPT_INS_FLUX64_XW))
#define g_lds ((int)ins_opt(OPT_INS_FLUX64_LDS))
#define g_skel ((int)ins_opt(OPT_INS_FLUX64_SKEL))

template <typename T, int R, int XW, bool FUSE, int NW>
int launch_range(const ins_grid* G, FluxArgs& a, int corr_mode, hipStream_t s) {
  const unsigned nb = (unsigned)(8LL * a.ntx * ((a.nty + 7) / 8) * a.ntz);
  if (nb == 0) return INS_OK;
  const dim3 block(64, NW, 1);
  if constexpr (NW <= 8 && R == 4 && sizeof(T) == 8) {
    if (g_skel && corr_mode == 0) {
      hipLaunchKernelGGL((k_flux64<T, R, XW, FUSE, 0, true, NW>), dim3(nb), block, (size_t)g_lds, s, a);
      INS_LAUNCH_CHECK();
      return INS_OK;
    }
  }
  if (a.tm && corr_mode != 0) {
    ins_set_error("temperature stage inside the stage kernel: no in-kernel pressure correction");
    return INS_ERR_UNSUPPORTED;
  }
  if (a.epi.extra || a.epi.gtemp || a.epi.wout || a.tm) {
    if constexpr (FUSE && R == 2 && NW == 4 && sizeof(T) == 8) {
      if (corr_mode == 0) {
        hipLaunchKernelGGL((k_flux64<T, R, XW, true, 0, false, NW, true>), dim3(nb), block, (size_t)g_lds, s, a);
        INS_LAUNCH_CHECK();
        return INS_OK;
      }
      if (corr_mode == 1) {
        hipLaunchKernelGGL((k_flux64<T, R, XW, true, 1, false, NW, true>), dim3(nb), block, (size_t)g_lds, s, a);
        INS_LAUNCH_CHECK();
        return INS_OK;
      }
    }
    ins_set_error("stage kernel with an extra force term: fp64, fused epilogue, 2 rows, 4 wavefronts, no slab correction");
    return INS_ERR_UNSUPPORTED;
  }
  if (corr_mode == 0)
    hipLaunchKernelGGL((k_flux64<T, R, XW, FUSE, 0, false, NW>), dim3(nb), block, (size_t)g_lds, s, a);
  else if constexpr (FUSE && R <= 5) {
    if (corr_mode == 1)
      hipLaunchKernelGGL((k_flux64<T, R, XW, true, 1, false, NW>), dim3(nb), block, (size_t)g_lds, s, a);
    else
      hipLaunchKernelGGL((k_flux64<T, R, XW, true, 2, false, NW>), dim3(nb), block, (size_t)g_lds, s, a);
  } else {
    ins_set_error("in-kernel pressure correction needs the fused epilogue and <= 5 rows per thread");
    return INS_ERR_UNSUPPORTED;
  }
  INS_LAUNCH_CHECK();
  return INS_OK;
}

constexpr int ZB = 4;
template <typename T, int R, int XW, bool FUSE, int NW = 4>
int launch(const ins_grid* G, FluxArgs& a, int corr_mode, int part, hipStream_t s) {
  const GridDev& g = G->g;
  a.ntx = cdiv(g.N[0] - 2, 64 * XW);
  a.nty = cdiv(g.N[1] - 2, (NW / XW) * R);
  const int nzl = g.N[2] - 2;
  a.k_lo = 1;
  a.k_hi = nzl + 1;
  a.kB = 0;
  if (part != 0 && nzl <= 2 * ZB) {
    if (part == 1) return INS_OK;
    part = 0;
  }
  if (part == 1) {
    a.k_lo = 1 + ZB;
    a.k_hi = nzl + 1 - ZB;
  } else if (part == 2) {
    a.zc = ZB;
    a.kB = nzl + 1 - ZB;
  }
  a.ntz = part == 2 ? 2 : cdiv(a.k_hi - a.k_lo, a.zc);
  return launch_range<T, R, XW, FUSE, NW>(G, a, corr_mode, s);
}

}

extern "C" void ins_tune_flux64(int disable, int rows, int rows_corr, int zchunk, int xw, int skel, int burst_unused, int lds) {
  if (disable >= 0) ins_set_option("INS_DISABLE_FLUX64", disable);
  if (rows >= 0) ins_set_option("INS_FLUX64_ROWS", rows);
  if (rows_corr >= 0) ins_set_option("INS_FLUX64_ROWS_CORR", rows_corr);
  if (zchunk >= 0) ins_set_option("INS_FLUX64_ZC", zchunk);
  if (xw >= 0) ins_set_option("INS_FLUX64_XW", xw);
  if (skel >= 0) ins_set_option("INS_FLUX64_SKEL", skel);
  (void)burst_unused;
  if (lds >= 0) ins_set_option("INS_FLUX64_LDS", lds);
}

bool ins_flux64_supported(const ins_grid* G) {
  const GridDev& g = G->g;
  return !g_disable && g.D == 3 && G->all_dof && G->uniform_exact && g.N[0] - 2 >= 66 && g.N[1] - 2 >= 8 && g.N[2] - 2 >= 4;
}

template <typename T>
static int flux64_dispatch(const ins_grid* G, double visc, const T* u, T* F, const RkEpi* epi, const T* pI, int corr_mode, hipStream_t s, int part) {
  const GridDev& g = G->g;
  FluxArgs a;
  memset(&a, 0, sizeof(a));
  a.u = u;
  a.pI = pI;
  a.F = F;
  a.sc = g.sc;
  a.N0 = g.N[0];
  a.N1 = g.N[1];
  a.N2 = g.N[2];
  const int n2 = g.N[2] - 2;
  a.X = make_dir(G, 0, visc);
  a.Y = make_dir(G, 1, visc);
  a.Z = make_dir(G, 2, visc);
  if (epi) a.epi = *epi;
  if (epi && epi->tstage) {
    a.te = *epi->tstage;
    a.tm = 1;
    a.epi.tstage = nullptr;
  }
  const int waves_x = cdiv(g.N[0] - 2, 64);
  const int xwo = (corr_mode && ins_opt(OPT_INS_FLUX64_XW_CORR)) ? (int)ins_opt(OPT_INS_FLUX64_XW_CORR) : g_xw;
  int xw = xwo ? xwo : (waves_x >= 8 ? 2 : (waves_x >= 4 ? 4 : (waves_x >= 2 ? 2 : 1)));
  if (!xwo)
    while (xw > 1 && cdiv(waves_x, xw) * xw > waves_x) xw >>= 1;
  int rows = corr_mode ? (g_rows_corr ? g_rows_corr : 2) : (g_rows ? g_rows : 4);
  rows = std::min(std::max(rows, 2), corr_mode ? 5 : 6);
  constexpr bool F32 = sizeof(T) == 4;
  if (F32) rows = corr_mode ? (ins_opt(OPT_INS_F32_CORR_ROWS) == 4 ? 4 : 2) : 4;
  const int nwo = (int)ins_opt(OPT_INS_FLUX64_NW);
  const int zco = (corr_mode && g_zchunk_corr) ? g_zchunk_corr : g_zchunk;
  auto tiles = [&](int nw_, int zc_) {
    return (long long)cdiv(g.N[0] - 2, 64 * xw) * cdiv(g.N[1] - 2, (nw_ / xw) * rows) * cdiv(n2, zc_);
  };
  const long long mintiles = ins_opt(OPT_INS_FLUX64_MINTILES) > 0 ? ins_opt(OPT_INS_FLUX64_MINTILES) : 256;
  int nw = nwo == 16 ? 16 : (nwo == 8 ? 8 : (nwo == 4 ? 4 : 0));
  int zc = zco;
  if (!nw) {
    nw = 4;
    if (xw <= 8 && !g_lds) {
      for (int z : {64}) {
        const int zt = zco ? zco : z;
        if (n2 >= zt && tiles(8, zt) >= mintiles) {
          nw = 8;
          zc = zt;
          break;
        }
      }
    }
  }
  if (!zc) {
    const bool small_plane = (long long)(g.N[0] - 2) * (g.N[1] - 2) <= 256LL * 256;
    zc = n2 >= 256 && small_plane ? 64 : (n2 >= 128 ? 32 : (n2 >= 64 ? 16 : (n2 >= 32 ? 8 : 4)));
    if (n2 < 256)
      while (zc > 4 && tiles(nw, zc) < 2 * mintiles) zc >>= 1;
  }
  if (rows != 2 && nw == 16) nw = 8;
  if (epi && (epi->extra || epi->gtemp || epi->wout || epi->tstage)) {
    rows = 2;
    nw = 4;
    if (!zco) zc = n2 >= 128 ? 32 : (n2 >= 64 ? 16 : (n2 >= 32 ? 8 : 4));
  }
  a.zc = zc;
  a.bar = ins_opt(OPT_INS_FLUX64_NOBAR) ? 0 : 1;
  {
    const long long o = ins_opt(OPT_INS_FLUX64_NT);
    a.nt = o == 0 ? ((epi && !F32) ? 9 : 0) : (o == 16 ? 0 : (int)o);
  }
#define INS_F64_CASE(RR, FUSE)                                                        \
  if constexpr (!F32 || RR == 2 || RR == 4) {                                         \
    if (rows == RR) {                                                                 \
      if constexpr (RR == 2 && !F32) {                                                \
        if (nw == 16) {                                                               \
          if (xw == 4) return launch<T, RR, 4, FUSE, 16>(G, a, corr_mode, part, s);   \
          if (xw == 2) return launch<T, RR, 2, FUSE, 16>(G, a, corr_mode, part, s);   \
          return launch<T, RR, 1, FUSE, 16>(G, a, corr_mode, part, s);                \
        }                                                                             \
      }                                                                               \
      if (nw >= 8) {                                                                  \
        if (xw == 4) return launch<T, RR, 4, FUSE, 8>(G, a, corr_mode, part, s);      \
        if (xw == 2) return launch<T, RR, 2, FUSE, 8>(G, a, corr_mode, part, s);      \
        return launch<T, RR, 1, FUSE, 8>(G, a, corr_mode, part, s);                   \
      }                                                                               \
      if (xw == 4) return launch<T, RR, 4, FUSE>(G, a, corr_mode, part, s);           \
      if (xw == 2) return launch<T, RR, 2, FUSE>(G, a, corr_mode, part, s);           \
      return launch<T, RR, 1, FUSE>(G, a, corr_mode, part, s);                        \
    }                                                                                 \
  }
  if (epi) {
    INS_F64_CASE(2, true)
    INS_F64_CASE(3, true)
    INS_F64_CASE(4, true)
    INS_F64_CASE(5, true)
    INS_F64_CASE(6, true)
  } else {
    INS_F64_CASE(2, false)
    INS_F64_CASE(3, false)
    INS_F64_CASE(4, false)
    INS_F64_CASE(5, false)
    INS_F64_CASE(6, false)
  }
#undef INS_F64_CASE
  return INS_ERR_INVALID;
}

bool ins_flux128_supported(const ins_grid* G, const RkEpi* epi, int corr_mode, bool f32);
int ins_k_flux128(const ins_grid* G, double visc, const double* u, double* F, const RkEpi* epi, const double* pI, int corr_mode, hipStream_t s, int part);
int ins_k_flux128_f32(const ins_grid* G, double visc, const float* u, float* F, const RkEpi* epi, const float* pI, int corr_mode, hipStream_t s, int part);

int ins_k_flux64(const ins_grid* G, double visc, const double* u, double* F, const RkEpi* epi, const double* pI, int corr_mode, hipStream_t s,
                 int part) {
  if (ins_flux128_supported(G, epi, corr_mode, false)) return ins_k_flux128(G, visc, u, F, epi, pI, corr_mode, s, part);
  return flux64_dispatch<double>(G, visc, u, F, epi, pI, corr_mode, s, part);
}
int ins_k_flux64_f32(const ins_grid* G, double visc, const float* u, float* F, const RkEpi* epi, const float* pI, int corr_mode, hipStream_t s,
                     int part) {
  if (ins_flux128_supported(G, epi, corr_mode, true) && !ins_opt(OPT_INS_F32_ONE_COLUMN)) return ins_k_flux128_f32(G, visc, u, F, epi, pI, corr_mode, s, part);
  return flux64_dispatch<float>(G, visc, u, F, epi, pI, corr_mode, s, part);
}
```

incompressiblenavierstokes.jl_amd/csrc/ins_internal.h:

```cpp
#pragma once

#include <hip/hip_runtime.h>
#include <hipfft/hipfft.h>

#include <cstdint>
#include <cstdio>
#include <cstring>
#include <string>
#include <vector>

#include "ins_hip.h"

#define INS_EPS 2.220446049250313e-16
#define INS_MAX_STAGES 16

void ins_set_error(const char* fmt, ...);

#define INS_HIP_TRY(expr)                                                                   \
  do {                                                                                      \
    hipError_t _e = (expr);                                                                 \
    if (_e != hipSuccess) {                                                                 \
      ins_set_error("%s:%d: %s -> %s", __FILE__, __LINE__, #expr, hipGetErrorString(_e));   \
      return INS_ERR_HIP;                                                                   \
    }                                                                                       \
  } while (0)

#define INS_FFT_TRY(expr)                                                         \
  do {                                                                            \
    hipfftResult _r = (expr);                                                     \
    if (_r != HIPFFT_SUCCESS) {                                                   \
      ins_set_error("%s:%d: %s -> hipfftResult %d", __FILE__, __LINE__, #expr, (int)_r); \
      return INS_ERR_FFT;                                                         \
    }                                                                             \
  } while (0)

#define INS_REQUIRE(cond, msg)                                        \
  do {                                                                \
    if (!(cond)) {                                                    \
      ins_set_error("%s:%d: %s (%s)", __FILE__, __LINE__, msg, #cond); \
      return INS_ERR_INVALID;                                         \
    }                                                                 \
  } while (0)

#define INS_LAUNCH_CHECK() INS_HIP_TRY(hipGetLastError())

#define INS_OPT_LIST(X)          \
  X(INS_DISABLE_FAST3D)          \
  X(INS_K1_LDS)                  \
  X(INS_FLUX_ROWS)               \
  X(INS_FLUX_ZC)                 \
  X(INS_FLUX_XW)                 \
  X(INS_FLUX_BAR)                \
  X(INS_FLUX64_62_FROM)          \
  X(INS_DISABLE_FLUX128)         \
  X(INS_DISABLE_YZ_FUSED)        \
  X(INS_YZ_FUSED)                \
  X(INS_YZ_SKEL)                 \
  X(INS_YZ_PARTITIONS)           \
  X(INS_F32_ONE_COLUMN)          \
  X(INS_FLUX128_CORR)            \
  X(INS_FLUX128_XW)              \
  X(INS_FLUX128_ROWS)            \
  X(INS_FLUX128_ROWS_CORR)       \
  X(INS_FLUX128_NW)              \
  X(INS_FLUX128_ZC)              \
  X(INS_DISABLE_FDM_ZDCT)        \
  X(INS_DISABLE_FDM_ZFFT)        \
  X(INS_DISABLE_FDM_XFFT)        \
  X(INS_DISABLE_FDM_XYFFT)       \
  X(INS_DISABLE_OWNFFT)          \
  X(INS_OWNFFT_POW2_ONLY)        \
  X(INS_FIELDS_NO_MARCH)         \
  X(INS_FIELDS_ROWS)             \
  X(INS_FIELDS_NOBAR)            \
  X(INS_FIELDS_ZC)               \
  X(INS_DISABLE_FLUX2D)          \
  X(INS_DISABLE_FLUX64M)         \
  X(INS_DISABLE_SMAGFORCE)       \
  X(INS_DISABLE_SMAGFORCE_GEN)   \
  X(INS_SMAGFORCE_FORCE_GEN)     \
  X(INS_SMAGFORCE_ZC)            \
  X(INS_SMAGFORCE_BAR)         \
  X(INS_FLUX64M_ZC)              \
  X(INS_FLUX64M_NOBAR)           \
  X(INS_FLUX64M_XW)              \
  X(INS_FLUX64M_ROWS)            \
  X(INS_FLUX64M_SKIP_FIRST)      \
  X(INS_DISABLE_FLUX64)          \
  X(INS_FLUX64_ROWS)             \
  X(INS_FLUX64_ROWS_CORR)        \
  X(INS_FLUX64_ZC)               \
  X(INS_FLUX64_ZC_CORR)          \
  X(INS_FLUX64_XW)               \
  X(INS_FLUX64_LDS)              \
  X(INS_FLUX64_SKEL)             \
  X(INS_FLUX64_NW)               \
  X(INS_FLUX64_NT)               \
  X(INS_FLUX64_NOBAR)            \
  X(INS_FLUX64_MINTILES)         \
  X(INS_FLUX64_XW_CORR)          \
  X(INS_UNIFORM_BITWISE)         \
  X(INS_PHAT_DENSE)              \
  X(INS_DISABLE_FDM_FUSED)       \
  X(INS_DISABLE_FDM_FOLD)        \
  X(INS_DISABLE_FDM_UNFOLD4)     \
  X(INS_DISABLE_FDM_FOLDFUSE)    \
  X(INS_DISABLE_INKERNEL_CORR)   \
  X(INS_RK_KEEP_K)               \
  X(INS_DISABLE_EXT_FUSED)       \
  X(INS_EXT_TEMP_SPLIT)          \
  X(INS_DISABLE_FUSED_RK)        \
  X(INS_DISABLE_STEP_CHAIN)      \
  X(INS_DISABLE_STEP_GRAPH)      \
  X(INS_DISABLE_LINE3)           \
  X(INS_DISABLE_XYFUSED)         \
  X(INS_DISABLE_CORR2D)          \
  X(INS_SPECTRUM_ROCFFT)         \
  X(INS_X_SKEL)                  \
  X(INS_LINE3_TK)                \
  X(INS_LINE3_WGS)               \
  X(INS_STEP_GRAPH)              \
  X(INS_ZSOLVE_SKEL)             \
  X(INS_ZSOLVE_TK)               \
  X(INS_ZSOLVE_RADIX4)           \
  X(INS_ZSOLVE_NT)               \
  X(INS_ZSOLVE_WGS)              \
  X(INS_DISABLE_ZSOLVE)          \
  X(INS_ZTRI_SKEL)               \
  X(INS_CG_HOSTSYNC)             \
  X(INS_CG_BATCH)                \
  X(INS_F32_CORR_ROWS)           \
  X(INS_F32_FP64_SPECTRA)        \
  X(INS_F32_HIPFFT_PROJECT)      \
  X(INS_F32_SPLIT_GRADIENT)      \
  X(INS_FFT_ALLOW_RESET)         \
  X(INS_DISABLE_ADJ_TILED)     \
  X(INS_DISABLE_FILTER_TILED)
#define INS_OPT_ENUM(id) OPT_##id,
enum InsOptId { INS_OPT_LIST(INS_OPT_ENUM) INS_OPT_COUNT };
#undef INS_OPT_ENUM
long long ins_opt(int id);
long long ins_opt_epoch();

struct GridDev {
  int D;
  int N[3];
  long long sx[3];
  long long sc;
  const double* dx[3];
  const double* dxu[3];
  const double* rdx[3];
  const double* rdxu[3];
  const double* mdx[3];
  const double* mdxu[3];
  const double* A1[3][3];
  const double* A2[3][3];
  int iu_lo[3][3], iu_hi[3][3];
  int ip_lo[3], ip_hi[3];
  int bc[3][2];
  double bc_u[3][2][3];
};

struct ins_grid {
  ins_grid_desc_t desc;
  std::vector<double> host;
  double* dev = nullptr;
  size_t dev_count = 0;
  GridDev g;
  bool all_periodic = false;
  bool uniform = false;
  double h[3] = {0, 0, 0};
  long long ncell = 0;
  bool all_dof = false;
  bool uniform_exact = false;
  void* rec_dev = nullptr;
  double rec_visc = -1.0;
  void* rec_diff_dev = nullptr;
  double rec_diff_visc = -1.0;
  double* red_dev = nullptr;
  double* red_host = nullptr;
  double* gradbar_dev = nullptr;
  size_t gradbar_count = 0;
};

enum PoissonKind { POISSON_SPECTRAL = 0, POISSON_CG = 1, POISSON_FDM = 2 };

struct ins_fdm;
int ins_fdm_create(int D, const int n[3], const double* const V[3], const double* const lam[3], int singular, ins_fdm** out);
int ins_fdm_destroy(ins_fdm* F);
int ins_fdm_enable_zfft(ins_fdm* F, double hz, const double* lam_z_host);
int ins_fdm_enable_zdct(ins_fdm* F, double hz, const double* lam_z_host);
int ins_fdm_enable_xfft(ins_fdm* F, double hx, const double* lam_x_host);
int ins_fdm_enable_xyfft(ins_fdm* F, double hx, double hy, const double* lam_x_host, const double* lam_y_host);
int ins_fdm_solve(ins_fdm* F, hipStream_t s, const ins_grid* G = nullptr, const double* u = nullptr, bool folded_io = false);
int ins_fdm_fold_mask(const ins_fdm* F);
bool ins_fdm_takes_u(const ins_fdm* F);
double* ins_fdm_buffer(ins_fdm* F);
const double* ins_fdm_mean(ins_fdm* F);

struct ins_poisson {
  PoissonKind kind;
  const ins_grid* grid;
  hipfftHandle plan_fwd = 0, plan_inv = 0;
  bool plans = false;
  double* pI = nullptr;
  hipfftDoubleComplex* phat = nullptr;
  double* ahat[3] = {nullptr, nullptr, nullptr};
  int np[3] = {1, 1, 1};
  int kmax[3] = {1, 1, 1};
  void* work = nullptr;
  size_t work_bytes = 0;
  hipStream_t plan_stream = nullptr;
  bool zfused = false;
  bool ownfft = false;
  bool y3 = false;
  int kxs = 0;
  double* tw = nullptr;
  double* tw_x = nullptr;
  double* tw_y = nullptr;
  int yz_P = 0;
  double* yz_scratch = nullptr;
  double abstol = 0, reltol = 0;
  long long maxiter = 0;
  double *r = nullptr, *L = nullptr, *q = nullptr, *dinv = nullptr;
  bool bordered = false;
  bool singular = true;
  long long ndof = 0;
  long long last_iter = 0;
  double last_res = 0;
  double* cg_scal = nullptr;
  double* cg_host = nullptr;
  struct ins_comm* comm = nullptr;
  ins_fdm* fdm = nullptr;
};

struct ins_rk_ext;
void ins_rk_ext_free(ins_rk_ext* e);
struct ins_rk {
  const ins_grid* grid;
  ins_poisson* ps;
  int nstage;
  std::vector<double> A, c;
  double* ustart = nullptr;
  std::vector<double*> ku;
  double* p = nullptr;
  double* ub[2] = {nullptr, nullptr};
  std::vector<double*> vb;
  const double* force = nullptr;
  ins_rk_ext* ext = nullptr;
  bool profiling = false;
  std::vector<hipEvent_t> prof_events;
  void* step_graph = nullptr;
};

struct Rec {
  double vs, vo, a0, b0, a1, b1, a2, b2, rs, ro, pad[6];
};

struct RkEpi {
  int n;
  int write_k;
  double coef[INS_MAX_STAGES + 1];
  const double* k[INS_MAX_STAGES + 1];
  double coef_self;
  double self_in;
  double c0m1;
  const double* ustart;
  double* ustar;
  double* ustart_out;
  const double* extra;
  const double* gtemp;
  double ga2;
  int gdir;
  double* wout;
  const struct TempEpi* tstage;
};

struct TempEpi {
  const double* temp;
  const double* tempstart;
  double* temp_out;
  double* ktemp_out;
  int n;
  double coef[INS_MAX_STAGES];
  const double* k[INS_MAX_STAGES];
  double c_self, a4, dcoef;
};


int ins_k_apply_bc_u(const ins_grid* grid, double* u, int dudt, const double* const* planes, hipStream_t s);
int ins_k_apply_bc_p(const ins_grid* grid, double* p, hipStream_t s);
int ins_k_apply_bc_p_fields(const ins_grid* grid, double* p, int nf, hipStream_t s);
int ins_k_momentum(const ins_grid* grid, double visc, const double* u, double* F, hipStream_t s);
int ins_k_divergence(const ins_grid* grid, const double* u, double* div, hipStream_t s);
int ins_k_diffusion_overwrite(const ins_grid* grid, double visc, const double* u, double* F, hipStream_t s);
int ins_k_scalewithvolume(const ins_grid* grid, double* p, hipStream_t s);
int ins_k_applypressure(const ins_grid* grid, double* u, const double* p, hipStream_t s);
int ins_k_laplacian(const ins_grid* grid, const double* p, double* L, hipStream_t s);
int ins_k_project(const ins_grid* grid, ins_poisson* ps, double* u, double* p, hipStream_t s);
int ins_k_momentum_rk_fused(const ins_grid* G, double visc, const double* u_in, double* k_out, const RkEpi& epi, hipStream_t s);
bool ins_flux2d_supported(const ins_grid* G);
int ins_k_flux2d(const ins_grid* G, double visc, const double* u, double* F, const RkEpi* epi, hipStream_t s, const double* pI = nullptr);
int ins_k_project_periodic_solve_only_2d(const ins_grid* G, ins_poisson* ps, const double* u, hipStream_t s);
int ins_k_momentum_rk_fused_generic(const ins_grid* G, double visc, const double* u_in, double* k_out, const RkEpi& epi, hipStream_t s);
int ins_k_momentum_rk_fused_corr(const ins_grid* G, double visc, const double* ustar_prev, const double* pI, double* k_out, const RkEpi& epi,
                                 hipStream_t s);
int ins_k_momentum_rk_fused_corr_slab(const ins_grid* G, double visc, const double* ustar_prev, const double* p_ext, double* k_out,
                                      const RkEpi& epi, hipStream_t s, int part = 0);
bool ins_corr3_supported(const ins_grid* G);
int ins_k_momentum_rk_fused_corr3(const ins_grid* G, double visc, const double* ustar_prev, const double* p_padded, double* k_out, const RkEpi& epi,
                                  hipStream_t s);
bool ins_k_project_fdm_fused(const ins_poisson* ps);
int ins_k_project_fdm_solve_only(const ins_grid* G, ins_poisson* ps, const double* u, double* p, hipStream_t s);
int ins_k_project_periodic_fused_2d(const ins_grid* G, ins_poisson* ps, double* u, double* p, bool keep_p, hipStream_t s);
bool ins_poisson_own2d(const ins_poisson* ps);
int ins_k_project_periodic_solve_only(const ins_grid* G, ins_poisson* ps, const double* u, hipStream_t s);
int ins_k_poisson_solve(ins_poisson* ps, double* p, hipStream_t s);
int ins_k_reduce(const ins_grid* grid, int op, const double* a, const double* b, const int lo[3], const int hi[3], double* out,
                 hipStream_t s);

int ins_validate_real_plans(hipfftHandle fwd, hipfftHandle inv, int rank, const int* n, int batch);
int ins_fft_make_real_plans(hipfftHandle* fwd, hipfftHandle* inv, int rank, int* n, int batch);
void ins_fft_solver_released();
bool ins_zsolve_supported(int nz);
bool ins_ownfft_supported(const int np[3]);
bool ins_ownfft_supported_slab(const int np[3]);
bool ins_ownfft_supported_mixed(const int np[3]);
void ins_ownfft_permute_symbol(int n, const double* ay, double* out);
int ins_k_ownfft_xfwd(const ins_grid* G, const double* src, int from_u, double* phat, int n0, int n1, int n2, const double* tw, hipStream_t s,
                      int kxs = 0, int kz0 = 0);
int ins_k_ownfft_xinv(const double* phat, double* pI, int n0, int n1, int n2, const double* tw, hipStream_t s, int kxs = 0);
int ins_k_ownfft_y(double* phat, int kxn, int n1, int n2, const double* tw, bool inverse, hipStream_t s, int kxs = 0);
bool ins_ownfft_xy_supported(int n0, int n1);
int ins_k_ownfft_xy(const ins_grid* G, const double* src, int from_u, double* phat, double* pI, int n0, int n1, int n2, const double* twx, const double* twy,
                    bool inverse, hipStream_t s, int kxs);
int ins_k_ownfft_xysolve2d(const ins_grid* G, const double* src, int from_u, double* pI, int n0, int n1, const double* twx, const double* twy, const double* ax,
                           const double* ay, hipStream_t s);
bool ins_line3_supported(int n);
void ins_line3_permute_symbol(int n, const double* ay, double* out);
int ins_line3_pos_of_freq(int n, int k);
int ins_k_line3_z(double* phat, int kxn, int n1, int n2, const double* tw, hipStream_t s, int kxs);
int ins_k_line3_y(double* phat, int kxn, int n1, int n2, const double* tw, bool inverse, hipStream_t s, int kxs);
int ins_k_line3_y_f32(float* phat, int kxn, int n1, int n2, const float* tw, bool inverse, hipStream_t s, int kxs);
int ins_ownfft_yz_partitions(int kxn, int n1, int n2);
long long ins_ownfft_yz_scratch(int kxn, int n1, int n2, int P);
int ins_k_ownfft_yz_solve(double* phat, int kxn, int n1, int n2, int kxs, int P, const double* ax, const double* ay, double c, double scale, const double* tw_y,
                          double* scratch, hipStream_t s);
int ins_k_ownfft_y_packed(double* phat, double* packed, int kxn, int n1, int nzl, int nyl, int cw, const double* tw, bool inverse,
                          hipStream_t s);
int ins_zsolve_twiddles(int nz, double** out);
int ins_k_fdm_z(double* data, int n0, int n1, int nz, const double* lx, const double* ly, const double* lz, const double* ox, const double* oy,
                double h, double tol, int singular, const double* meanf, double* partial, const double* tw, int* nblk, hipStream_t s, const double* dct_w = nullptr);
int ins_k_zsolve(double* data, int nz, long long nl, const double* ax, int kxn, const double* ay, const double* az, const double* tw,
                 double inv_n, bool zero_mean, hipStream_t s, int kxs = 0);

int ins_comm_allreduce_internal(struct ins_comm* c, double* buf, long long count, int op, hipStream_t s);
int ins_comm_halo_scalar_internal(struct ins_comm* c, const ins_grid* G, double* p, hipStream_t s);

static inline hipStream_t as_stream(void* s) { return reinterpret_cast<hipStream_t>(s); }
static inline unsigned cdiv(long long a, long long b) { return (unsigned)((a + b - 1) / b); }
```

incompressiblenavierstokes.jl_amd/csrc/ins_options.hip:

```cpp
#include <atomic>
#include <cstdlib>
#include <cstring>

#include "ins_internal.h"

namespace {

struct Opt {
  const char* name;
  std::atomic<long long> value;
  std::atomic<int> state;
};

#define INS_OPT_ROW(id) {#id, {0}, {0}},
Opt g_opts[INS_OPT_COUNT] = {INS_OPT_LIST(INS_OPT_ROW)};
#undef INS_OPT_ROW

std::atomic<long long> g_epoch{0};

long long from_env(const char* name) {
  const char* v = getenv(name);
  if (!v) return 0;
  if (!*v) return 1;
  char* end = nullptr;
  const long long x = strtoll(v, &end, 10);
  if (end == v) {
    return 1;
  }
  return x;
}

}

long long ins_opt(int id) {
  Opt& o = g_opts[id];
  if (o.state.load(std::memory_order_acquire) == 0) {
    o.value.store(from_env(o.name), std::memory_order_relaxed);
    o.state.store(1, std::memory_order_release);
  }
  return o.value.load(std::memory_order_relaxed);
}

long long ins_opt_epoch() { return g_epoch.load(std::memory_order_relaxed); }

static int find(const char* name) {
  if (!name) return -1;
  for (int i = 0; i < INS_OPT_COUNT; ++i)
    if (!strcmp(name, g_opts[i].name)) return i;
  return -1;
}

extern "C" int ins_set_option(const char* name, int64_t value) {
  const int id = find(name);
  if (id < 0) {
    ins_set_error("ins_set_option: unknown option '%s'", name ? name : "(null)");
    return INS_ERR_INVALID;
  }
  g_opts[id].value.store(value, std::memory_order_relaxed);
  g_opts[id].state.store(1, std::memory_order_release);
  g_epoch.fetch_add(1, std::memory_order_relaxed);
  return INS_OK;
}

extern "C" int ins_get_option(const char* name, int64_t* value) {
  const int id = find(name);
  if (id < 0 || !value) {
    ins_set_error("ins_get_option: unknown option '%s'", name ? name : "(null)");
    return INS_ERR_INVALID;
  }
  *value = ins_opt(id);
  return INS_OK;
}

extern "C" int ins_option_count(void) { return INS_OPT_COUNT; }

extern "C" const char* ins_option_name(int i) { return (i >= 0 && i < INS_OPT_COUNT) ? g_opts[i].name : nullptr; }
```

incompressiblenavierstokes.jl_amd/csrc/ins_poisson.hip:

```cpp
#include <cmath>
#include <cstdlib>

#include "ins_internal.h"

namespace {

template <int D, bool WRAP = false>
__global__ __launch_bounds__(256) void k_div_to_pI(GridDev g, const double* __restrict__ u, double* __restrict__ pI, int n0, int n1) {
  const int ii = blockIdx.x * 64 + threadIdx.x;
  const int jj = blockIdx.y * 4 + threadIdx.y;
  const int kk = D == 3 ? (int)blockIdx.z : 0;
  if (ii >= n0 || jj >= n1) return;
  const int I[3] = {g.ip_lo[0] + ii, g.ip_lo[1] + jj, D == 3 ? g.ip_lo[2] + kk : 0};
  const long long c = I[0] + I[1] * g.sx[1] + I[2] * g.sx[2];
  double d = 0.0;
#pragma unroll
  for (int a = 0; a < D; ++a) {
    const double* ua = u + a * g.sc;
    const long long cm = (WRAP && I[a] == 1) ? c + (long long)(g.N[a] - 3) * g.sx[a] : c - g.sx[a];
    d += (ua[c] - ua[cm]) * g.rdx[a][I[a]];
  }
  double om = g.dx[0][I[0]] * g.dx[1][I[1]];
  if (D == 3) om = om * g.dx[2][I[2]];
  pI[ii + (long long)n0 * (jj + (long long)n1 * kk)] = d * om;
// ... 634 lines not shown
  flat_partial(s, partial);
}
__global__ __launch_bounds__(256) void k_cgd_precond(GridDev g, long long n, const double* __restrict__ sc, const double* __restrict__ r,
                                                     const double* __restrict__ dinv, double* __restrict__ L, double* __restrict__ partial) {
  if (sc[CG_DONE] != 0.0) return;
  double s = 0.0;
  for (long long t = (long long)blockIdx.x * 256 + threadIdx.x; t < n; t += (long long)gridDim.x * 256) {
    bool inp;
    flat_cell(g, t, inp);
    if (inp) {
      const double rv = r[t], z = -rv * dinv[t];
      L[t] = z;
      s += z * rv;
    }
  }
  flat_partial(s, partial);
}
__global__ __launch_bounds__(256) void k_cgd_dir(long long n, const double* __restrict__ sc, const double* __restrict__ L, double* __restrict__ q) {
  if (sc[CG_DONE] != 0.0) return;
  const double beta = sc[CG_BETA];
  for (long long t = (long long)blockIdx.x * 256 + threadIdx.x; t < n; t += (long long)gridDim.x * 256) q[t] = L[t] + beta * q[t];
}
__global__ __launch_bounds__(256) void k_cgd_dot(GridDev g, long long n, const double* __restrict__ sc, const double* __restrict__ a,
                                                 const double* __restrict__ b, double* __restrict__ partial) {
  if (sc[CG_DONE] != 0.0) return;
  double s = 0.0;
  for (long long t = (long long)blockIdx.x * 256 + threadIdx.x; t < n; t += (long long)gridDim.x * 256) {
    bool inp;
    flat_cell(g, t, inp);
    if (inp) s += a[t] * b[t];
  }
  flat_partial(s, partial);
}
__global__ __launch_bounds__(256) void k_cgd_update(GridDev g, long long n, const double* __restrict__ sc, double* __restrict__ p, double* __restrict__ r,
                                                    const double* __restrict__ q, const double* __restrict__ L, double* __restrict__ partial) {
  if (sc[CG_DONE] != 0.0) return;
  const double alpha = sc[CG_ALPHA];
  double s = 0.0;
  for (long long t = (long long)blockIdx.x * 256 + threadIdx.x; t < n; t += (long long)gridDim.x * 256) {
    bool inp;
    flat_cell(g, t, inp);
    p[t] += alpha * q[t];
    const double rv = r[t] - alpha * L[t];
    r[t] = rv;
    if (inp) s += rv * rv;
  }
  flat_partial(s, partial);
}

struct BoxLaunch {
  dim3 grid, block;
  int nblk;
};

inline BoxLaunch full_box(const GridDev& g) {
  BoxLaunch l;
  l.block = dim3(64, 4, 1);
  l.grid = dim3(cdiv(g.N[0], 64), cdiv(g.N[1], 4), (unsigned)g.N[2]);
  l.nblk = (int)(l.grid.x * l.grid.y * l.grid.z);
  return l;
}

}

extern "C" int ins_poisson_spectral_create(const ins_grid_t* G, ins_poisson_t** out) {
  INS_REQUIRE(G && out, "null argument");
  INS_REQUIRE(G->all_periodic, "Spectral psolver requires periodic boundary conditions.");
  INS_REQUIRE(G->uniform, "Spectral psolver requires uniform grid spacing.");
  const GridDev& g = G->g;
  for (int a = 0; a < g.D; ++a) INS_REQUIRE(g.N[a] % 2 == 0, "Spectral psolver requires even number of volumes.");
  ins_poisson* ps = new ins_poisson();
  ps->kind = POISSON_SPECTRAL;
  ps->grid = G;
  const int D = g.D;
  long long nreal = 1, ncplx = 1;
  double om = 1.0;
  for (int a = 0; a < D; ++a) {
    ps->np[a] = g.ip_hi[a] - g.ip_lo[a];
    ps->kmax[a] = a == 0 ? ps->np[a] / 2 + 1 : ps->np[a];
    nreal *= ps->np[a];
    ncplx *= ps->kmax[a];
    om *= G->h[a];
  }
  int rc = INS_OK;
  auto fail = [&](int code) {
    ins_poisson_destroy(ps);
    return code;
  };
  ps->ownfft = D == 3 && ins_ownfft_supported_mixed(ps->np);
  const int np2[3] = {ps->np[0], 16, ps->np[1]};
  const bool own2d = D == 2 && ins_ownfft_supported(np2);
  if (own2d) ps->ownfft = true;
  if (ps->ownfft) {
    ps->kxs = ins_opt(OPT_INS_PHAT_DENSE) ? ps->kmax[0] : ((ps->kmax[0] + 7) & ~7);
    ncplx = (long long)ps->kxs * ps->kmax[1] * ps->kmax[2];
  }
  if (hipMalloc(&ps->pI, nreal * sizeof(double)) != hipSuccess || hipMalloc(&ps->phat, ncplx * sizeof(hipfftDoubleComplex)) != hipSuccess ||
      hipMemset(ps->phat, 0, ncplx * sizeof(hipfftDoubleComplex)) != hipSuccess) {
    ins_set_error("hipMalloc(pI/phat) failed for %lld cells", nreal);
    return fail(INS_ERR_HIP);
  }
  for (int a = 0; a < D; ++a) {
    std::vector<double> ah(ps->kmax[a]);
    for (int k = 0; k < ps->kmax[a]; ++k) {
      const double sn = std::sin(M_PI * ((double)k / ps->np[a]));
      ah[k] = 4 * om * sn * sn / (G->h[a] * G->h[a]);
    }
    if (ps->ownfft && D == 3 && a == 1) {
      ps->y3 = ins_line3_supported(ps->np[1]) && ins_ownfft_yz_partitions(ps->kmax[0], ps->np[1], ps->np[2]) == 0;
      std::vector<double> perm(ah.size());
      if (ps->y3)
        ins_line3_permute_symbol(ps->np[1], ah.data(), perm.data());
      else
        ins_ownfft_permute_symbol(ps->np[1], ah.data(), perm.data());
      ah.swap(perm);
    }
    if (hipMalloc(&ps->ahat[a], ah.size() * sizeof(double)) != hipSuccess ||
        hipMemcpy(ps->ahat[a], ah.data(), ah.size() * sizeof(double), hipMemcpyHostToDevice) != hipSuccess) {
      ins_set_error("ahat upload failed");
      return fail(INS_ERR_HIP);
    }
  }
  if (own2d) {
    if ((rc = ins_zsolve_twiddles(ps->np[0], &ps->tw_x))) return fail(rc);
    if ((rc = ins_zsolve_twiddles(ps->np[1], &ps->tw))) return fail(rc);
    if (hipMalloc(&ps->ahat[2], sizeof(double)) != hipSuccess || hipMemset(ps->ahat[2], 0, sizeof(double)) != hipSuccess) return fail(INS_ERR_HIP);
    ps->zfused = true;
  } else if (ps->ownfft) {
    if ((rc = ins_zsolve_twiddles(ps->np[0], &ps->tw_x))) return fail(rc);
    if ((rc = ins_zsolve_twiddles(ps->np[1], &ps->tw_y))) return fail(rc);
    if ((rc = ins_zsolve_twiddles(ps->np[2], &ps->tw))) return fail(rc);
    ps->zfused = true;
    ps->yz_P = ins_ownfft_yz_partitions(ps->kmax[0], ps->np[1], ps->np[2]);
    if (ps->yz_P) {
      const long long nc = ins_ownfft_yz_scratch(ps->kmax[0], ps->np[1], ps->np[2], ps->yz_P);
      if (hipMalloc(&ps->yz_scratch, nc * 2 * sizeof(double)) != hipSuccess) {
        ins_set_error("hipMalloc(yz scratch) failed");
        return fail(INS_ERR_HIP);
      }
    }
  } else {
    int nfull[3] = {ps->np[2], ps->np[1], ps->np[0]};
    ps->zfused = D == 3 && ins_zsolve_supported(ps->np[2]);
    rc = ps->zfused ? ins_fft_make_real_plans(&ps->plan_fwd, &ps->plan_inv, 2, nfull + 1, ps->np[2])
                    : ins_fft_make_real_plans(&ps->plan_fwd, &ps->plan_inv, D, nfull + (3 - D), 1);
    if (rc) return fail(rc);
    ps->plans = true;
    if (ps->zfused && (rc = ins_zsolve_twiddles(ps->np[2], &ps->tw))) return fail(rc);
  }
  *out = ps;
  return INS_OK;
}

static int ownfft_transform(ins_poisson* ps, const double* from_u, hipStream_t s, int src_code = 1) {
  const int n0 = ps->np[0], n1 = ps->np[1], n2 = ps->np[2], kxn = ps->kmax[0], kxs = ps->kxs;
  double* ph = reinterpret_cast<double*>(ps->phat);
  int rc;
  if (ps->grid->g.D == 2) {
    if (ins_ownfft_xy_supported(n0, n1))
      return ins_k_ownfft_xysolve2d(ps->grid, ps->pI, 0, ps->pI, n0, n1, ps->tw_x, ps->tw, ps->ahat[0], ps->ahat[1], s);
    if ((rc = ins_k_ownfft_xfwd(ps->grid, ps->pI, false, ph, n0, n1, 1, ps->tw_x, s, kxs))) return rc;
    if ((rc = ins_k_zsolve(ph, n1, (long long)kxs, ps->ahat[0], kxn, ps->ahat[2], ps->ahat[1], ps->tw, 1.0 / ((double)n0 * n1), true, s, kxs))) return rc;
    return ins_k_ownfft_xinv(ph, ps->pI, n0, n1, 1, ps->tw_x, s, kxs);
  }
  if (!ps->y3 && !ps->yz_P && (src_code == 1 || !from_u) && ins_ownfft_xy_supported(n0, n1)) {
    if ((rc = ins_k_ownfft_xy(ps->grid, from_u ? from_u : ps->pI, from_u ? 1 : 0, ph, nullptr, n0, n1, n2, ps->tw_x, ps->tw_y, false, s, kxs))) return rc;
    const double inv_n = 1.0 / ((double)n0 * n1 * n2);
    if ((rc = ins_k_zsolve(ph, n2, (long long)kxs * n1, ps->ahat[0], kxn, ps->ahat[1], ps->ahat[2], ps->tw, inv_n, true, s, kxs))) return rc;
    return ins_k_ownfft_xy(nullptr, nullptr, 0, ph, ps->pI, n0, n1, n2, ps->tw_x, ps->tw_y, true, s, kxs);
  }
  if ((rc = ins_k_ownfft_xfwd(ps->grid, from_u ? from_u : ps->pI, from_u ? src_code : 0, ph, n0, n1, n2, ps->tw_x, s, kxs))) return rc;
  if (ps->yz_P && !ins_opt(OPT_INS_DISABLE_YZ_FUSED)) {
    const ins_grid* G = ps->grid;
    const double c = G->h[0] * G->h[1] / G->h[2];
    if ((rc = ins_k_ownfft_yz_solve(ph, kxn, n1, n2, kxs, ps->yz_P, ps->ahat[0], ps->ahat[1], c, -1.0 / ((double)n0 * n1), ps->tw_y, ps->yz_scratch, s))) return rc;
    return ins_k_ownfft_xinv(ph, ps->pI, n0, n1, n2, ps->tw_x, s, kxs);
  }
  if ((rc = ps->y3 ? ins_k_line3_y(ph, kxn, n1, n2, ps->tw_y, false, s, kxs) : ins_k_ownfft_y(ph, kxn, n1, n2, ps->tw_y, false, s, kxs))) return rc;
  const double inv_n = 1.0 / ((double)n0 * n1 * n2);
  if ((rc = ins_k_zsolve(ph, n2, (long long)kxs * n1, ps->ahat[0], kxn, ps->ahat[1], ps->ahat[2], ps->tw, inv_n, true, s, kxs))) return rc;
  if ((rc = ps->y3 ? ins_k_line3_y(ph, kxn, n1, n2, ps->tw_y, true, s, kxs) : ins_k_ownfft_y(ph, kxn, n1, n2, ps->tw_y, true, s, kxs))) return rc;
  return ins_k_ownfft_xinv(ph, ps->pI, n0, n1, n2, ps->tw_x, s, kxs);
}

static int spectral_transform(ins_poisson* ps, hipStream_t s) {
  const GridDev& g = ps->grid->g;
  if (ps->ownfft) return ownfft_transform(ps, nullptr, s);
  INS_FFT_TRY(hipfftSetStream(ps->plan_fwd, s));
  INS_FFT_TRY(hipfftSetStream(ps->plan_inv, s));
  INS_FFT_TRY(hipfftExecD2Z(ps->plan_fwd, ps->pI, ps->phat));
  double inv_n = 1.0;
  for (int a = 0; a < g.D; ++a) inv_n /= ps->np[a];
  if (ps->zfused) {
    int rc = ins_k_zsolve(reinterpret_cast<double*>(ps->phat), ps->np[2], (long long)ps->kmax[0] * ps->kmax[1], ps->ahat[0], ps->kmax[0],
                          ps->ahat[1], ps->ahat[2], ps->tw, inv_n, true, s);
    if (rc) return rc;
    INS_FFT_TRY(hipfftExecZ2D(ps->plan_inv, ps->phat, ps->pI));
    return INS_OK;
  }
  dim3 block(64, 4, 1), grid(cdiv(ps->kmax[0], 64), cdiv(ps->kmax[1], 4), g.D == 3 ? ps->kmax[2] : 1);
  if (g.D == 2)
    hipLaunchKernelGGL(k_symbol<2>, grid, block, 0, s, ps->phat, ps->ahat[0], ps->ahat[1], (const double*)nullptr, ps->kmax[0],
                       ps->kmax[1], inv_n);
  else
    hipLaunchKernelGGL(k_symbol<3>, grid, block, 0, s, ps->phat, ps->ahat[0], ps->ahat[1], ps->ahat[2], ps->kmax[0], ps->kmax[1],
                       inv_n);
  INS_LAUNCH_CHECK();
  INS_FFT_TRY(hipfftExecZ2D(ps->plan_inv, ps->phat, ps->pI));
  return INS_OK;
}

static int spectral_solve(ins_poisson* ps, double* p, hipStream_t s) {
  const GridDev& g = ps->grid->g;
  dim3 block(64, 4, 1), grid(cdiv(ps->np[0], 64), cdiv(ps->np[1], 4), g.D == 3 ? ps->np[2] : 1);
  if (g.D == 2)
    hipLaunchKernelGGL((k_pack<2, true>), grid, block, 0, s, g, p, ps->pI, ps->np[0], ps->np[1]);
  else
    hipLaunchKernelGGL((k_pack<3, true>), grid, block, 0, s, g, p, ps->pI, ps->np[0], ps->np[1]);
  INS_LAUNCH_CHECK();
  int rc = spectral_transform(ps, s);
  if (rc) return rc;
  if (g.D == 2)
    hipLaunchKernelGGL((k_pack<2, false>), grid, block, 0, s, g, p, ps->pI, ps->np[0], ps->np[1]);
  else
    hipLaunchKernelGGL((k_pack<3, false>), grid, block, 0, s, g, p, ps->pI, ps->np[0], ps->np[1]);
  INS_LAUNCH_CHECK();
  return INS_OK;
}

extern "C" int ins_poisson_cg_create(const ins_grid_t* G, double abstol, double reltol, int64_t maxiter, ins_poisson_t** out) {
  INS_REQUIRE(G && out, "null argument");
  const GridDev& g = G->g;
  for (int a = 0; a < 2 && a < g.D; ++a)
    INS_REQUIRE(g.bc[a][0] != INS_BC_HALO && g.bc[a][1] != INS_BC_HALO, "slabs are cut along z only");
  ins_poisson* ps = new ins_poisson();
  ps->kind = POISSON_CG;
  ps->grid = G;
  ps->abstol = abstol;
  ps->reltol = reltol;
  long long ndof = 1;
  for (int a = 0; a < g.D; ++a) ndof *= g.ip_hi[a] - g.ip_lo[a];
  ps->maxiter = maxiter > 0 ? maxiter : ndof;
  ps->ndof = ndof;
  for (int a = 0; a < g.D; ++a)
    if (g.bc[a][0] == INS_BC_PRESSURE || g.bc[a][1] == INS_BC_PRESSURE) ps->singular = false;
  const size_t bytes = G->ncell * sizeof(double);
  if (hipMalloc(&ps->r, bytes) != hipSuccess || hipMalloc(&ps->L, bytes) != hipSuccess || hipMalloc(&ps->q, bytes) != hipSuccess ||
      hipMalloc(&ps->dinv, bytes) != hipSuccess) {
    ins_set_error("hipMalloc(cg scratch) failed");
    ins_poisson_destroy(ps);
    return INS_ERR_HIP;
  }
  BoxLaunch l = full_box(g);
  if (g.D == 2)
    hipLaunchKernelGGL(k_cg_diag<2>, l.grid, l.block, 0, 0, g, ps->dinv);
  else
    hipLaunchKernelGGL(k_cg_diag<3>, l.grid, l.block, 0, 0, g, ps->dinv);
  if (hipDeviceSynchronize() != hipSuccess) {
    ins_set_error("cg diag kernel failed");
    ins_poisson_destroy(ps);
    return INS_ERR_HIP;
  }
  *out = ps;
  return INS_OK;
}

static int finish_sum(const ins_grid* G, double* partial_dev, int nblk, hipStream_t s, double* out) {
  std::vector<double> h(nblk);
  INS_HIP_TRY(hipMemcpyAsync(h.data(), partial_dev, nblk * sizeof(double), hipMemcpyDeviceToHost, s));
  INS_HIP_TRY(hipStreamSynchronize(s));
  double v = 0.0;
  for (int i = 0; i < nblk; ++i) v += h[i];
  *out = v;
  return INS_OK;
}


static int cg_solve_device(ins_poisson* ps, double* p, hipStream_t s) {
  const ins_grid* G = ps->grid;
  const GridDev& g = G->g;
  const long long n = G->ncell;
  if (!ps->cg_scal) {
    INS_HIP_TRY(hipMalloc(&ps->cg_scal, (CG_NSCAL + CG_NPART) * sizeof(double)));
    INS_HIP_TRY(hipHostMalloc(&ps->cg_host, CG_NSCAL * sizeof(double)));
  }
  double* sc = ps->cg_scal;
  double* partial = sc + CG_NSCAL;
  const unsigned nb = (unsigned)std::min<long long>((n + 255) / 256, CG_NPART);
  int rc;
  const double maxit = (double)ps->maxiter;
  auto fold = [&](int stage) -> int {
    hipLaunchKernelGGL(k_cgd_fold, dim3(1), dim3(1024), 0, s, partial, (int)nb, sc);
    if (ps->comm) {
      int r2 = ins_comm_allreduce_internal(ps->comm, sc + CG_SUM, 1, 0, s);
      if (r2) return r2;
    }
    hipLaunchKernelGGL(k_cgd_scalars, dim3(1), dim3(1), 0, s, sc, stage, ps->reltol, ps->abstol, maxit);
    INS_LAUNCH_CHECK();
    return INS_OK;
  };
  const bool bordered = ps->bordered && ps->singular;
  if (bordered) {
    INS_REQUIRE(!ps->comm, "bordered CG on slabs is not implemented");
    double sum;
    if ((rc = ins_k_reduce(G, 3, p, nullptr, g.ip_lo, g.ip_hi, &sum, s))) return rc;
    if (g.D == 2)
      hipLaunchKernelGGL(k_shift<2>, full_box(g).grid, full_box(g).block, 0, s, g, p, sum / (double)ps->ndof);
    else
      hipLaunchKernelGGL(k_shift<3>, full_box(g).grid, full_box(g).block, 0, s, g, p, sum / (double)ps->ndof);
  }
  hipLaunchKernelGGL(k_cgd_init, dim3(nb), dim3(256), 0, s, g, n, p, ps->r, ps->q, ps->L, partial);
  if ((rc = fold(0))) return rc;
  const long long batch = ins_opt(OPT_INS_CG_BATCH) > 0 ? ins_opt(OPT_INS_CG_BATCH) : 32;
  long long issued = 0;
  while (true) {
    INS_HIP_TRY(hipMemcpyAsync(ps->cg_host, sc, CG_NSCAL * sizeof(double), hipMemcpyDeviceToHost, s));
    INS_HIP_TRY(hipStreamSynchronize(s));
    if (ps->cg_host[CG_DONE] != 0.0 || issued >= ps->maxiter) break;
    for (long long b = 0; b < batch && issued < ps->maxiter; ++b, ++issued) {
      hipLaunchKernelGGL(k_cgd_precond, dim3(nb), dim3(256), 0, s, g, n, sc, ps->r, ps->dinv, ps->L, partial);
      if ((rc = fold(1))) return rc;
      hipLaunchKernelGGL(k_cgd_dir, dim3(nb), dim3(256), 0, s, n, sc, ps->L, ps->q);
      if ((rc = ins_k_apply_bc_p(G, ps->q, s))) return rc;
      if (ps->comm && (rc = ins_comm_halo_scalar_internal(ps->comm, G, ps->q, s))) return rc;
// ... 229 lines not shown
    if (uni && (rc = ins_fdm_enable_zdct(ps->fdm, hz, lam[2]))) {
      ins_poisson_destroy(ps);
      return rc;
    }
  }
  *out = ps;
  return INS_OK;
}

int ins_k_poisson_solve(ins_poisson* ps, double* p, hipStream_t s) {
  switch (ps->kind) {
    case POISSON_SPECTRAL: return spectral_solve(ps, p, s);
    case POISSON_FDM: return fdm_solve(ps, p, s);
    default: return cg_solve(ps, p, s);
  }
}

extern "C" int ins_poisson_solve_f64(ins_poisson_t* ps, double* p, void* stream) {
  INS_REQUIRE(ps && p, "null argument");
  return ins_k_poisson_solve(ps, p, as_stream(stream));
}

int ins_fdm_modes(const ins_fdm* F);
extern "C" int ins_dbg_fdm_modes(const ins_poisson_t* ps) { return (ps && ps->kind == POISSON_FDM) ? ins_fdm_modes(ps->fdm) : -1; }
extern "C" int ins_dbg_fdm_fold_mask(const ins_poisson_t* ps) { return (ps && ps->kind == POISSON_FDM) ? ins_fdm_fold_mask(ps->fdm) : -1; }

extern "C" int ins_poisson_last_info(const ins_poisson_t* ps, int64_t* iterations, double* residual) {
  INS_REQUIRE(ps, "null argument");
  if (iterations) *iterations = ps->last_iter;
  if (residual) *residual = ps->last_res;
  return INS_OK;
}

bool ins_k_project_fdm_fused(const ins_poisson* ps) { return ps->kind == POISSON_FDM && !ins_opt(OPT_INS_DISABLE_FDM_FUSED); }
static int fdm_rhs(const ins_grid* G, ins_poisson* ps, const double* u, double* buf, int fm, hipStream_t s) {
  const GridDev& g = G->g;
  const dim3 block(64, 4, 1);
  if (fm) {
    const int n0 = ps->np[0], n1 = ps->np[1], n2 = g.D == 3 ? ps->np[2] : 1;
    const dim3 grid(cdiv((fm & 1) ? n0 / 2 : n0, 64), cdiv((fm & 2) ? n1 / 2 : n1, 4), (g.D == 3 && (fm & 4)) ? n2 / 2 : n2);
#define INS_DIVFOLD(DD, MM) \
  case MM: hipLaunchKernelGGL((k_div_to_pI_fold<DD, MM>), grid, block, 0, s, g, u, buf, n0, n1, n2); break;
    if (g.D == 2) {
      switch (fm & 3) {
        INS_DIVFOLD(2, 1)
        INS_DIVFOLD(2, 2)
        INS_DIVFOLD(2, 3)
      }
    } else {
      switch (fm & 7) {
        INS_DIVFOLD(3, 1)
        INS_DIVFOLD(3, 2)
        INS_DIVFOLD(3, 3)
        INS_DIVFOLD(3, 4)
        INS_DIVFOLD(3, 5)
        INS_DIVFOLD(3, 6)
        INS_DIVFOLD(3, 7)
      }
    }
#undef INS_DIVFOLD
  } else {
    const dim3 grid(cdiv(ps->np[0], 64), cdiv(ps->np[1], 4), g.D == 3 ? ps->np[2] : 1);
    if (g.D == 2)
      hipLaunchKernelGGL(k_div_to_pI<2>, grid, block, 0, s, g, u, buf, ps->np[0], ps->np[1]);
    else
      hipLaunchKernelGGL(k_div_to_pI<3>, grid, block, 0, s, g, u, buf, ps->np[0], ps->np[1]);
  }
  INS_LAUNCH_CHECK();
  return INS_OK;
}

static int fdm_unpack(const ins_grid* G, ins_poisson* ps, double* u, double* p, const double* buf, int fm, hipStream_t s) {
  const GridDev& g = G->g;
  const dim3 block(64, 4, 1);
  const int n0 = ps->np[0], n1 = ps->np[1], n2 = g.D == 3 ? ps->np[2] : 1;
  bool pressure_side = false;
  for (int a = 0; a < g.D; ++a) pressure_side = pressure_side || g.bc[a][0] == INS_BC_PRESSURE || g.bc[a][1] == INS_BC_PRESSURE;
  if (g.D == 3 && fm && !pressure_side && !((fm & 1) && (n0 & 1)) && !((fm & 2) && (n1 & 1)) && !((fm & 4) && (n2 & 1)) && !ins_opt(OPT_INS_DISABLE_FDM_UNFOLD4)) {
    const dim3 grid(cdiv((fm & 1) ? n0 / 2 : n0, 64), cdiv((fm & 2) ? n1 / 2 : n1, 4), (fm & 4) ? n2 / 2 : n2);
    if (u)
      hipLaunchKernelGGL(k_unfold_grad3<true>, grid, block, 0, s, g, u, p, buf, n0, n1, n2, ins_fdm_mean(ps->fdm), fm);
    else
      hipLaunchKernelGGL(k_unfold_grad3<false>, grid, block, 0, s, g, u, p, buf, n0, n1, n2, ins_fdm_mean(ps->fdm), fm);
    INS_LAUNCH_CHECK();
    return INS_OK;
  }
  const dim3 gridp(cdiv(n0 + 2, 64), cdiv(n1 + 2, 4), g.D == 3 ? n2 + 2 : 1);
  if (g.D == 2) {
    if (u)
      hipLaunchKernelGGL((k_unpack_grad_bc<2, true>), gridp, block, 0, s, g, u, p, buf, n0, n1, ins_fdm_mean(ps->fdm), fm, 1);
    else
      hipLaunchKernelGGL((k_unpack_grad_bc<2, false>), gridp, block, 0, s, g, u, p, buf, n0, n1, ins_fdm_mean(ps->fdm), fm, 1);
  } else {
    if (u)
      hipLaunchKernelGGL((k_unpack_grad_bc<3, true>), gridp, block, 0, s, g, u, p, buf, n0, n1, ins_fdm_mean(ps->fdm), fm, n2);
    else
      hipLaunchKernelGGL((k_unpack_grad_bc<3, false>), gridp, block, 0, s, g, u, p, buf, n0, n1, ins_fdm_mean(ps->fdm), fm, n2);
  }
  INS_LAUNCH_CHECK();
  return INS_OK;
}

int ins_k_project_fdm_solve_only(const ins_grid* G, ins_poisson* ps, const double* u, double* p, hipStream_t s) {
  int rc, fm = 0;
  double* buf = ins_fdm_buffer(ps->fdm);
  if (ins_fdm_takes_u(ps->fdm)) {
    if ((rc = ins_fdm_solve(ps->fdm, s, G, u))) return rc;
  } else {
    fm = ins_opt(OPT_INS_DISABLE_FDM_FOLDFUSE) ? 0 : ins_fdm_fold_mask(ps->fdm);
    if ((rc = fdm_rhs(G, ps, u, buf, fm, s))) return rc;
    if ((rc = ins_fdm_solve(ps->fdm, s, nullptr, nullptr, fm != 0))) return rc;
  }
  return fdm_unpack(G, ps, nullptr, p, buf, fm, s);
}

int ins_k_project(const ins_grid* G, ins_poisson* ps, double* u, double* p, hipStream_t s) {
  const GridDev& g = G->g;
  int rc;
  if (ps->kind == POISSON_SPECTRAL) {
    dim3 block(64, 4, 1), grid(cdiv(ps->np[0], 64), cdiv(ps->np[1], 4), g.D == 3 ? ps->np[2] : 1);
    if (g.D == 2)
      hipLaunchKernelGGL(k_div_to_pI<2>, grid, block, 0, s, g, u, ps->pI, ps->np[0], ps->np[1]);
    else
      hipLaunchKernelGGL(k_div_to_pI<3>, grid, block, 0, s, g, u, ps->pI, ps->np[0], ps->np[1]);
    INS_LAUNCH_CHECK();
    if ((rc = spectral_transform(ps, s))) return rc;
    dim3 gridp(cdiv(g.N[0], 64), cdiv(g.N[1], 4), (unsigned)g.N[2]);
    if (g.D == 2)
      hipLaunchKernelGGL(k_grad_from_pI<2>, gridp, block, 0, s, g, u, p, ps->pI, ps->np[0], ps->np[1], 1);
    else
      hipLaunchKernelGGL(k_grad_from_pI<3>, gridp, block, 0, s, g, u, p, ps->pI, ps->np[0], ps->np[1], ps->np[2]);
    INS_LAUNCH_CHECK();
    return INS_OK;
  }
  if (ps->kind == POISSON_FDM && !ins_opt(OPT_INS_DISABLE_FDM_FUSED)) {
    double* buf = ins_fdm_buffer(ps->fdm);
    int fm = 0;
    if (ins_fdm_takes_u(ps->fdm)) {
      if ((rc = ins_fdm_solve(ps->fdm, s, G, u))) return rc;
    } else {
      fm = ins_opt(OPT_INS_DISABLE_FDM_FOLDFUSE) ? 0 : ins_fdm_fold_mask(ps->fdm);
      if ((rc = fdm_rhs(G, ps, u, buf, fm, s))) return rc;
      if ((rc = ins_fdm_solve(ps->fdm, s, nullptr, nullptr, fm != 0))) return rc;
    }
    return fdm_unpack(G, ps, u, p, buf, fm, s);
  }
  if ((rc = ins_k_divergence(G, u, p, s))) return rc;
  if ((rc = ins_k_scalewithvolume(G, p, s))) return rc;
  if ((rc = ins_k_poisson_solve(ps, p, s))) return rc;
  if ((rc = ins_k_apply_bc_p(G, p, s))) return rc;
  return ins_k_applypressure(G, u, p, s);
}

int ins_k_project_periodic_fused(const ins_grid* G, ins_poisson* ps, double* u, double* p, bool keep_p, hipStream_t s, double* uout) {
  const GridDev& g = G->g;
  dim3 block(64, 4, 1), grid(cdiv(ps->np[0], 64), cdiv(ps->np[1], 4), ps->np[2]);
  int rc;
  double* dst = uout ? uout : u;
  if (ps->ownfft) {
    rc = ownfft_transform(ps, u, s);
  } else {
    hipLaunchKernelGGL((k_div_to_pI<3, true>), grid, block, 0, s, g, u, ps->pI, ps->np[0], ps->np[1]);
    INS_LAUNCH_CHECK();
    rc = spectral_transform(ps, s);
  }
  if (rc) return rc;
  if (keep_p)
    hipLaunchKernelGGL(k_grad_ghost3<true>, grid, block, 0, s, g, dst, p, ps->pI, ps->np[0], ps->np[1], ps->np[2], (const double*)u);
  else
    hipLaunchKernelGGL(k_grad_ghost3<false>, grid, block, 0, s, g, dst, p, ps->pI, ps->np[0], ps->np[1], ps->np[2], (const double*)u);
  INS_LAUNCH_CHECK();
  return INS_OK;
}

int ins_k_project_periodic_fused_2d(const ins_grid* G, ins_poisson* ps, double* u, double* p, bool keep_p, hipStream_t s) {
  const GridDev& g = G->g;
  const int n0 = ps->np[0], n1 = ps->np[1], kxn = ps->kmax[0], kxs = ps->kxs;
  double* ph = reinterpret_cast<double*>(ps->phat);
  int rc;
  if (ins_ownfft_xy_supported(n0, n1)) {
    if ((rc = ins_k_ownfft_xysolve2d(G, u, 1, ps->pI, n0, n1, ps->tw_x, ps->tw, ps->ahat[0], ps->ahat[1], s))) return rc;
  } else {
    if ((rc = ins_k_ownfft_xfwd(G, u, 3, ph, n0, n1, 1, ps->tw_x, s, kxs))) return rc;
    if ((rc = ins_k_zsolve(ph, n1, (long long)kxs, ps->ahat[0], kxn, ps->ahat[2], ps->ahat[1], ps->tw, 1.0 / ((double)n0 * n1), true, s, kxs))) return rc;
    if ((rc = ins_k_ownfft_xinv(ph, ps->pI, n0, n1, 1, ps->tw_x, s, kxs))) return rc;
  }
  dim3 block(64, 4, 1), grid(cdiv(n0, 64), cdiv(n1, 4), 1);
  if (keep_p)
    hipLaunchKernelGGL((k_grad_ghost<2, true>), grid, block, 0, s, g, u, p, ps->pI, n0, n1, 1);
  else
    hipLaunchKernelGGL((k_grad_ghost<2, false>), grid, block, 0, s, g, u, p, ps->pI, n0, n1, 1);
  INS_LAUNCH_CHECK();
  return INS_OK;
}

int ins_k_project_periodic_solve_only_2d(const ins_grid* G, ins_poisson* ps, const double* u, hipStream_t s) {
  const int n0 = ps->np[0], n1 = ps->np[1], kxn = ps->kmax[0], kxs = ps->kxs;
  double* ph = reinterpret_cast<double*>(ps->phat);
  int rc;
  if (ins_ownfft_xy_supported(n0, n1)) return ins_k_ownfft_xysolve2d(G, u, 1, ps->pI, n0, n1, ps->tw_x, ps->tw, ps->ahat[0], ps->ahat[1], s);
  if ((rc = ins_k_ownfft_xfwd(G, u, 3, ph, n0, n1, 1, ps->tw_x, s, kxs))) return rc;
  if ((rc = ins_k_zsolve(ph, n1, (long long)kxs, ps->ahat[0], kxn, ps->ahat[2], ps->ahat[1], ps->tw, 1.0 / ((double)n0 * n1), true, s, kxs))) return rc;
  return ins_k_ownfft_xinv(ph, ps->pI, n0, n1, 1, ps->tw_x, s, kxs);
}

bool ins_poisson_own2d(const ins_poisson* ps) { return ps->kind == POISSON_SPECTRAL && ps->ownfft && ps->grid->g.D == 2; }

int ins_k_project_periodic_solve_only(const ins_grid* G, ins_poisson* ps, const double* u, hipStream_t s) {
  const GridDev& g = G->g;
  if (ps->ownfft) return ownfft_transform(ps, u, s);
  dim3 block(64, 4, 1), grid(cdiv(ps->np[0], 64), cdiv(ps->np[1], 4), ps->np[2]);
  hipLaunchKernelGGL((k_div_to_pI<3, true>), grid, block, 0, s, g, u, ps->pI, ps->np[0], ps->np[1]);
  INS_LAUNCH_CHECK();
  return spectral_transform(ps, s);
}

bool ins_k_spectral_own3d(const ins_poisson* ps) { return ps->kind == POISSON_SPECTRAL && ps->ownfft && ps->grid->g.D == 3; }
int ins_k_spectral_solve_from_u32(ins_poisson* ps, const float* u32, hipStream_t s) {
  return ownfft_transform(ps, reinterpret_cast<const double*>(u32), s, 5);
}
const double* ins_k_spectral_pI(const ins_poisson* ps) { return ps->pI; }

bool ins_zsolve_f32_supported(int nz);
int ins_k_zsolve_f32(float* data, int nz, long long nl, const double* ax, int kxn, const double* ay, const double* az, const float* tw, double inv_n,
                     bool zero_mean, hipStream_t s, int kxs);
int ins_k_ownfft_xfwd_f32(const ins_grid* G, const float* src, int from_u, float* phat, int n0, int n1, int n2, const float* tw, hipStream_t s, int kxs);
int ins_k_ownfft_xinv_f32(const float* phat, float* pI, int n0, int n1, int n2, const float* tw, hipStream_t s, int kxs);
int ins_k_ownfft_y_f32(float* phat, int kxn, int n1, int n2, const float* tw, bool inverse, hipStream_t s, int kxs);
bool ins_k_spectral_own3d_f32(const ins_poisson* ps) { return ins_k_spectral_own3d(ps) && ins_zsolve_f32_supported(ps->np[2]); }
int ins_k_spectral_solve_f32(ins_poisson* ps, const float* u32, float* pI32, float* phat32, int kxs32, const float* twx, const float* twy,
                             const float* twz, hipStream_t s) {
  const int n0 = ps->np[0], n1 = ps->np[1], n2 = ps->np[2], kxn = ps->kmax[0];
  int rc;
  if ((rc = ins_k_ownfft_xfwd_f32(ps->grid, u32 ? u32 : pI32, u32 ? 1 : 0, phat32, n0, n1, n2, twx, s, kxs32))) return rc;
  if ((rc = ps->y3 ? ins_k_line3_y_f32(phat32, kxn, n1, n2, twy, false, s, kxs32) : ins_k_ownfft_y_f32(phat32, kxn, n1, n2, twy, false, s, kxs32))) return rc;
  const double inv_n = 1.0 / ((double)n0 * n1 * n2);
  if ((rc = ins_k_zsolve_f32(phat32, n2, (long long)kxs32 * n1, ps->ahat[0], kxn, ps->ahat[1], ps->ahat[2], twz, inv_n, true, s, kxs32))) return rc;
  if ((rc = ps->y3 ? ins_k_line3_y_f32(phat32, kxn, n1, n2, twy, true, s, kxs32) : ins_k_ownfft_y_f32(phat32, kxn, n1, n2, twy, true, s, kxs32))) return rc;
  return ins_k_ownfft_xinv_f32(phat32, pI32, n0, n1, n2, twx, s, kxs32);
}

extern "C" int ins_project_f64(const ins_grid_t* G, ins_poisson_t* ps, double* u, double* p, void* stream) {
  INS_REQUIRE(G && ps && u && p, "null argument");
  INS_REQUIRE(ps->grid == G, "psolver was created for a different grid");
  return ins_k_project(G, ps, u, p, as_stream(stream));
}
```

incompressiblenavierstokes.jl_amd/csrc/ins_rk.hip:

```cpp
#include <cstdlib>

#include "ins_internal.h"


int ins_k_momentum_generic(const ins_grid* G, double visc, const double* u, double* F, hipStream_t s);
int ins_k_momentum_fast3d(const ins_grid* G, double visc, const double* u, double* F, hipStream_t s);
int ins_k_momentum_fast3d_opts(const ins_grid* G, double visc, const double* u, double* F, bool zero_shell, hipStream_t s);
bool ins_fast3d_supported(const ins_grid* G);
bool ins_flux64_supported(const ins_grid* G);

int ins_k_momentum_rk_fused(const ins_grid* G, double visc, const double* u_in, double* k_out, const RkEpi& epi, hipStream_t s);
int ins_k_project_periodic_fused(const ins_grid* G, ins_poisson* ps, double* u, double* p, bool keep_p, hipStream_t s, double* uout = nullptr);

int ins_k_momentum(const ins_grid* G, double visc, const double* u, double* F, hipStream_t s) {
  if (ins_fast3d_supported(G)) return ins_k_momentum_fast3d(G, visc, u, F, s);
  return ins_k_momentum_generic(G, visc, u, F, s);
}

namespace {

struct Combine {
  int n;
  double coef[INS_MAX_STAGES + 1];
  const double* k[INS_MAX_STAGES + 1];
};

__global__ __launch_bounds__(256) void k_combine(long long n, const double* ustart, double* u, Combine cb) {
  const long long stride = (long long)gridDim.x * 256 * 2;
  for (long long t = ((long long)blockIdx.x * 256 + threadIdx.x) * 2; t < n; t += stride) {
    if (t + 1 < n) {
      double2 v = *reinterpret_cast<const double2*>(ustart + t);
      for (int j = 0; j < cb.n; ++j) {
        const double2 kv = *reinterpret_cast<const double2*>(cb.k[j] + t);
        v.x += cb.coef[j] * kv.x;
        v.y += cb.coef[j] * kv.y;
      }
      *reinterpret_cast<double2*>(u + t) = v;
    } else {
      double v = ustart[t];
      for (int j = 0; j < cb.n; ++j) v += cb.coef[j] * cb.k[j][t];
      u[t] = v;
    }
  }
}

}

static int combine_n(long long nvec, const double* base, double* out, int nterms, const double* coefs, const double* const* ks, void* stream);

extern "C" int ins_combine_f64(const ins_grid_t* G, const double* base, double* out, int nterms, const double* coefs,
                               const double* const* ks, void* stream) {
  INS_REQUIRE(G && base && out, "null argument");
  return combine_n(G->ncell * G->g.D, base, out, nterms, coefs, ks, stream);
}

extern "C" int ins_combine_scalar_f64(const ins_grid_t* G, const double* base, double* out, int nterms, const double* coefs,
                                      const double* const* ks, void* stream) {
  INS_REQUIRE(G && base && out, "null argument");
  return combine_n(G->ncell, base, out, nterms, coefs, ks, stream);
}

static int combine_n(long long nvec, const double* base, double* out, int nterms, const double* coefs, const double* const* ks, void* stream) {
  INS_REQUIRE(nterms >= 0 && nterms <= INS_MAX_STAGES + 1 && (nterms == 0 || (coefs && ks)), "bad stage terms");
  Combine cb;
  cb.n = 0;
  for (int q = 0; q < nterms; ++q) {
    if (coefs[q] == 0.0) continue;
    INS_REQUIRE(ks[q], "null stage field");
    cb.coef[cb.n] = coefs[q];
    cb.k[cb.n] = ks[q];
    ++cb.n;
  }
  const unsigned nblk = (unsigned)std::min<long long>((nvec / 2 + 255) / 256, 8192);
  hipLaunchKernelGGL(k_combine, dim3(nblk), dim3(256), 0, as_stream(stream), nvec, base, out, cb);
  INS_LAUNCH_CHECK();
  return INS_OK;
}

static void step_graph_free(ins_rk* rk);
bool ins_k_spectral_own3d(const ins_poisson* ps);

extern "C" int ins_rk_create(const ins_grid_t* G, ins_poisson_t* ps, int nstage, const double* A, const double* c, ins_rk_t** out) {
  INS_REQUIRE(G && ps && A && c && out, "null argument");
  INS_REQUIRE(ps->grid == G, "psolver was created for a different grid");
  INS_REQUIRE(nstage >= 1 && nstage <= INS_MAX_STAGES, "unsupported number of stages");
  for (int i = 0; i < nstage; ++i)
    for (int j = i + 1; j < nstage; ++j) INS_REQUIRE(A[i * nstage + j] == 0.0, "shifted tableau must be lower triangular (explicit method)");
  ins_rk* rk = new ins_rk();
  rk->grid = G;
  rk->ps = ps;
  rk->nstage = nstage;
  rk->A.assign(A, A + nstage * nstage);
  rk->c.assign(c, c + nstage);
  const size_t vbytes = (size_t)G->ncell * G->g.D * sizeof(double);
  bool ok = hipMalloc(&rk->ustart, vbytes) == hipSuccess && hipMalloc(&rk->p, G->ncell * sizeof(double)) == hipSuccess;
  rk->ku.assign(nstage, nullptr);
  for (int i = 0; ok && i < nstage; ++i) ok = hipMalloc(&rk->ku[i], vbytes) == hipSuccess;
  if (ok) ok = hipMemset(rk->p, 0, G->ncell * sizeof(double)) == hipSuccess && hipMemset(rk->ustart, 0, vbytes) == hipSuccess;
  for (int i = 0; ok && i < nstage; ++i) ok = hipMemset(rk->ku[i], 0, vbytes) == hipSuccess;
  if (!ok) {
    ins_set_error("ins_rk_create: device allocation of %d vector fields failed", nstage + 1);
    ins_rk_destroy(rk);
    return INS_ERR_HIP;
  }
  *out = rk;
  return INS_OK;
}

extern "C" int ins_rk_destroy(ins_rk_t* rk) {
  if (!rk) return INS_OK;
  if (rk->ustart) (void)hipFree(rk->ustart);
  if (rk->p) (void)hipFree(rk->p);
  for (double* k : rk->ku)
    if (k) (void)hipFree(k);
  for (double* v : rk->vb)
    if (v && v != rk->ub[0] && v != rk->ub[1]) (void)hipFree(v);
  for (double* b : rk->ub)
    if (b) (void)hipFree(b);
  for (hipEvent_t e : rk->prof_events) (void)hipEventDestroy(e);
  ins_rk_ext_free(rk->ext);
  step_graph_free(rk);
  delete rk;
  return INS_OK;
}

extern "C" int ins_rk_profile_enable(ins_rk_t* rk, int enable) {
  INS_REQUIRE(rk, "null argument");
  rk->profiling = enable != 0;
  return INS_OK;
}

extern "C" int ins_rk_profile_read(ins_rk_t* rk, double* momentum_ms, int64_t* momentum_launches) {
  INS_REQUIRE(rk && momentum_ms && momentum_launches, "null argument");
  double total = 0.0;
  const size_t n = rk->prof_events.size() / 2;
  for (size_t i = 0; i < n; ++i) {
    float ms = 0.f;
    INS_HIP_TRY(hipEventSynchronize(rk->prof_events[2 * i + 1]));
    INS_HIP_TRY(hipEventElapsedTime(&ms, rk->prof_events[2 * i], rk->prof_events[2 * i + 1]));
    total += ms;
  }
  for (hipEvent_t e : rk->prof_events) (void)hipEventDestroy(e);
  rk->prof_events.clear();
  *momentum_ms = total;
  *momentum_launches = (int64_t)n;
  return INS_OK;
}

extern "C" int ins_rk_pressure(const ins_rk_t* rk, double** p) {
  INS_REQUIRE(rk && p, "null argument");
  *p = rk->p;
  return INS_OK;
}

extern "C" int ins_rk_set_bodyforce(ins_rk_t* rk, const double* force) {
  INS_REQUIRE(rk, "null argument");
  rk->force = force;
  return INS_OK;
}

extern "C" int ins_rk_stage_force(const ins_rk_t* rk, int i, double** ku) {
  INS_REQUIRE(rk && ku, "null argument");
  INS_REQUIRE(i >= 0 && i < rk->nstage, "stage index out of range");
  *ku = rk->ku[i];
  return INS_OK;
}

static int rk_step_fused_periodic(ins_rk* rk, double visc, double* u, double dt, hipStream_t s, int chain = 0) {
  const ins_grid* G = rk->grid;
  const int ns = rk->nstage;
  const size_t vbytes = (size_t)G->ncell * 3 * sizeof(double);
  for (int b = 0; b < 2; ++b)
    if (!rk->ub[b]) {
      INS_HIP_TRY(hipMalloc(&rk->ub[b], vbytes));
      INS_HIP_TRY(hipMemsetAsync(rk->ub[b], 0, vbytes, s));
    }
  int rc;
  const bool raw_in = chain & 1, raw_out = chain & 2;
  if (!raw_in && (rc = ins_k_apply_bc_u(G, u, 0, nullptr, s))) return rc;
  const bool no_corr = ins_opt(OPT_INS_DISABLE_INKERNEL_CORR) != 0;
  const bool inkernel = !no_corr && G->uniform_exact && ns > 1 && G->g.N[0] >= 8 && G->g.N[1] >= 8 && G->g.N[2] >= 8;
  const bool keep_k = ins_opt(OPT_INS_RK_KEEP_K) != 0;
  bool vbasis = inkernel && !keep_k;
  for (int i = 0; vbasis && i < ns; ++i) vbasis = rk->A[i * ns + i] != 0.0;
  if (vbasis && (int)rk->vb.size() < ns - 1) {
    rk->vb.resize(ns - 1, nullptr);
    for (int m = 0; m < ns - 1; ++m)
      if (!rk->vb[m]) {
        if (m < 2 && rk->ub[m]) {
          rk->vb[m] = rk->ub[m];
          continue;
        }
        INS_HIP_TRY(hipMalloc(&rk->vb[m], vbytes));
        INS_HIP_TRY(hipMemsetAsync(rk->vb[m], 0, vbytes, s));
      }
  }
  const double* in = u;
  for (int i = 0; i < ns; ++i) {
    double* out = (i == ns - 1 && ns > 1) ? u : (vbasis ? rk->vb[i] : rk->ub[i & 1]);
    RkEpi epi;
    memset(&epi, 0, sizeof(epi));
    if (vbasis) {
      double beta[INS_MAX_STAGES];
      for (int m = i - 1; m >= 0; --m) {
        double v = rk->A[i * ns + m];
        for (int j = m + 1; j < i; ++j) v -= beta[j] * rk->A[j * ns + m];
        beta[m] = v / rk->A[m * ns + m];
      }
      const bool flux64 = ins_flux64_supported(G);
      for (int m = 0; m < i; ++m) {
        if (beta[m] == 0.0) continue;
        epi.c0m1 -= beta[m];
        if (m == i - 1 && flux64) {
          epi.self_in = beta[m];
          continue;
        }
        epi.coef[epi.n] = beta[m];
        epi.k[epi.n] = rk->vb[m];
        ++epi.n;
      }
    } else {
      for (int j = 0; j < i; ++j) {
        const double coef = dt * rk->A[i * ns + j];
        if (coef == 0.0) continue;
        epi.coef[epi.n] = coef;
        epi.k[epi.n] = rk->ku[j];
        ++epi.n;
      }
      for (int i2 = i + 1; i2 < ns; ++i2)
        if (rk->A[i2 * ns + i] != 0.0) epi.write_k = 1;
    }
    if (rk->force) {
      double cf = dt * rk->A[i * ns + i];
      if (!vbasis)
        for (int j = 0; j < i; ++j) cf += dt * rk->A[i * ns + j];
      epi.coef[epi.n] = cf;
      epi.k[epi.n] = rk->force;
      ++epi.n;
    }
    epi.coef_self = dt * rk->A[i * ns + i];
    epi.ustart = (i == 0) ? nullptr : (raw_in ? rk->ustart : u);
    epi.ustar = out;
    if (i == 0 && raw_in) epi.ustart_out = rk->ustart;
    hipEvent_t e0 = nullptr, e1 = nullptr;
    if (rk->profiling) {
      INS_HIP_TRY(hipEventCreate(&e0));
      INS_HIP_TRY(hipEventCreate(&e1));
      INS_HIP_TRY(hipEventRecord(e0, s));
    }
    rc = (inkernel && (i > 0 || raw_in)) ? ins_k_momentum_rk_fused_corr(G, visc, in, rk->ps->pI, rk->ku[i], epi, s)
                             : ins_k_momentum_rk_fused(G, visc, in, rk->ku[i], epi, s);
    if (rc) return rc;
    if (rk->profiling) {
      INS_HIP_TRY(hipEventRecord(e1, s));
      rk->prof_events.push_back(e0);
      rk->prof_events.push_back(e1);
    }
    rc = (inkernel && (i < ns - 1 || raw_out)) ? ins_k_project_periodic_solve_only(G, rk->ps, out, s)
                                               : ins_k_project_periodic_fused(G, rk->ps, out, rk->p, i == ns - 1, s);
    if (rc) return rc;
    in = out;
  }
  if (ns == 1) INS_HIP_TRY(hipMemcpyAsync(u, rk->ub[0], vbytes, hipMemcpyDeviceToDevice, s));
  return INS_OK;
}

static int rk_step_fused_periodic_2d(ins_rk* rk, double visc, double* u, double dt, hipStream_t s, int chain = 0) {
  const ins_grid* G = rk->grid;
  const int ns = rk->nstage;
  const size_t vbytes = (size_t)G->ncell * 2 * sizeof(double);
  for (int b = 0; b < 2; ++b)
    if (!rk->ub[b]) {
      INS_HIP_TRY(hipMalloc(&rk->ub[b], vbytes));
      INS_HIP_TRY(hipMemsetAsync(rk->ub[b], 0, vbytes, s));
    }
  int rc;
  const bool raw_in = chain & 1, raw_out = chain & 2;
  if (!raw_in && (rc = ins_k_apply_bc_u(G, u, 0, nullptr, s))) return rc;
  const bool incorr = ns > 1 && !ins_opt(OPT_INS_DISABLE_INKERNEL_CORR) && !ins_opt(OPT_INS_DISABLE_CORR2D) && G->g.N[0] >= 6 && G->g.N[1] >= 6;
  if (chain && !incorr) {
    ins_set_error("chained 2-D steps need the in-register correction");
    return INS_ERR_INVALID;
  }
  const double* in = u;
  for (int i = 0; i < ns; ++i) {
    double* out = (i == ns - 1 && ns > 1) ? u : rk->ub[i & 1];
    RkEpi epi;
    memset(&epi, 0, sizeof(epi));
    for (int j = 0; j < i; ++j) {
      const double coef = dt * rk->A[i * ns + j];
      if (coef == 0.0) continue;
      epi.coef[epi.n] = coef;
      epi.k[epi.n] = rk->ku[j];
      ++epi.n;
    }
    if (rk->force) {
      double cf = 0.0;
      for (int j = 0; j <= i; ++j) cf += dt * rk->A[i * ns + j];
      epi.coef[epi.n] = cf;
      epi.k[epi.n] = rk->force;
      ++epi.n;
    }
    for (int i2 = i + 1; i2 < ns; ++i2)
      if (rk->A[i2 * ns + i] != 0.0) epi.write_k = 1;
    epi.coef_self = dt * rk->A[i * ns + i];
    epi.ustart = (i == 0) ? nullptr : (raw_in ? rk->ustart : u);
    epi.ustar = out;
    if (i == 0 && raw_in) epi.ustart_out = rk->ustart;
    hipEvent_t e0 = nullptr, e1 = nullptr;
    if (rk->profiling) {
      INS_HIP_TRY(hipEventCreate(&e0));
      INS_HIP_TRY(hipEventCreate(&e1));
      INS_HIP_TRY(hipEventRecord(e0, s));
    }
    if ((rc = ins_k_flux2d(G, visc, in, rk->ku[i], &epi, s, (incorr && (i > 0 || raw_in)) ? rk->ps->pI : nullptr))) return rc;
    if (rk->profiling) {
      INS_HIP_TRY(hipEventRecord(e1, s));
      rk->prof_events.push_back(e0);
      rk->prof_events.push_back(e1);
    }
    rc = (incorr && (i < ns - 1 || raw_out)) ? ins_k_project_periodic_solve_only_2d(G, rk->ps, out, s) : ins_k_project_periodic_fused_2d(G, rk->ps, out, rk->p, i == ns - 1, s);
    if (rc) return rc;
    in = out;
  }
  if (ns == 1) INS_HIP_TRY(hipMemcpyAsync(u, rk->ub[0], vbytes, hipMemcpyDeviceToDevice, s));
  return INS_OK;
}

struct StepGraph {
  hipStream_t gs = nullptr;
  hipEvent_t ev_in = nullptr, ev_out = nullptr;
  hipGraphExec_t exec = nullptr;
  double* u = nullptr;
  double dt = 0.0, visc = 0.0;
  const double* force = nullptr;
  int kind = 0;
  long long epoch = -1;
  long long replays = 0;
  bool broken = false;
};

static void step_graph_free(ins_rk* rk) {
  StepGraph* g = static_cast<StepGraph*>(rk->step_graph);
  if (!g) return;
  if (g->exec) (void)hipGraphExecDestroy(g->exec);
  if (g->ev_in) (void)hipEventDestroy(g->ev_in);
  if (g->ev_out) (void)hipEventDestroy(g->ev_out);
  if (g->gs) (void)hipStreamDestroy(g->gs);
  delete g;
  rk->step_graph = nullptr;
}

extern "C" long long ins_dbg_rk_graph_replays(const ins_rk_t* rk) { return (rk && rk->step_graph) ? static_cast<const StepGraph*>(rk->step_graph)->replays : 0; }

static int step_graph_kind(const ins_rk* rk, bool chain_ok) {
  const ins_grid* G = rk->grid;
  if (!ins_opt(OPT_INS_STEP_GRAPH) || ins_opt(OPT_INS_DISABLE_STEP_GRAPH) || rk->profiling || rk->ext) return 0;
  if (ins_opt(OPT_INS_DISABLE_FUSED_RK) || !G->all_periodic || rk->ps->kind != POISSON_SPECTRAL) return 0;
  if (G->g.D == 3) {
    if (!(G->all_dof && ins_fast3d_supported(G) && ins_k_spectral_own3d(rk->ps))) return 0;
    for (int a = 0; a < 3; ++a)
      if (rk->ps->np[a] < 2) return 0;
    return chain_ok ? 1 : 2;
  }
  return (ins_poisson_own2d(rk->ps) && ins_flux2d_supported(G)) ? (chain_ok ? 1 : 2) : 0;
}

static int chain_step(ins_rk* rk, double visc, double* u, double dt, hipStream_t s, int chain) {
  return rk->grid->g.D == 2 ? rk_step_fused_periodic_2d(rk, visc, u, dt, s, chain) : rk_step_fused_periodic(rk, visc, u, dt, s, chain);
}

template <typename F>
static bool step_graph_capture(StepGraph* g, F&& enqueue) {
  if (g->exec) {
    (void)hipGraphExecDestroy(g->exec);
    g->exec = nullptr;
  }
  if (!g->gs && hipStreamCreateWithFlags(&g->gs, hipStreamNonBlocking) != hipSuccess) return false;
  if (!g->ev_in && hipEventCreateWithFlags(&g->ev_in, hipEventDisableTiming) != hipSuccess) return false;
  if (!g->ev_out && hipEventCreateWithFlags(&g->ev_out, hipEventDisableTiming) != hipSuccess) return false;
  if (hipStreamBeginCapture(g->gs, hipStreamCaptureModeThreadLocal) != hipSuccess) {
    (void)hipGetLastError();
    return false;
  }
  const int rc = enqueue(g->gs);
  hipGraph_t graph = nullptr;
  const hipError_t e = hipStreamEndCapture(g->gs, &graph);
  bool ok = rc == INS_OK && e == hipSuccess && graph != nullptr;
  if (ok) ok = hipGraphInstantiate(&g->exec, graph, nullptr, nullptr, 0) == hipSuccess;
  if (graph) (void)hipGraphDestroy(graph);
  if (!ok) {
    (void)hipGetLastError();
    g->exec = nullptr;
  }
  return ok;
}

extern "C" int ins_rk_steps_f64(ins_rk_t* rk, double visc, double* u, double t, double dt, int nsteps, void* stream) {
  INS_REQUIRE(rk && u && nsteps >= 0, "bad argument");
  const ins_grid* G = rk->grid;
  hipStream_t s = as_stream(stream);
  const GridDev& g = G->g;
  const bool no_fuse = ins_opt(OPT_INS_DISABLE_FUSED_RK) != 0, no_corr = ins_opt(OPT_INS_DISABLE_INKERNEL_CORR) != 0,
             no_chain = ins_opt(OPT_INS_DISABLE_STEP_CHAIN) != 0;
  bool ok = !no_fuse && !no_corr && !no_chain && !rk->force && g.D == 3 && G->all_periodic && G->all_dof && rk->ps->kind == POISSON_SPECTRAL && ins_fast3d_supported(G) &&
            G->uniform_exact && rk->nstage > 1 && g.N[0] >= 8 && g.N[1] >= 8 && g.N[2] >= 8;
  const bool ok2d = !no_fuse && !no_corr && !no_chain && !ins_opt(OPT_INS_DISABLE_CORR2D) && !rk->force && !rk->ext && g.D == 2 && rk->ps->kind == POISSON_SPECTRAL &&
                    ins_poisson_own2d(rk->ps) && ins_flux2d_supported(G) && rk->nstage > 1 && g.N[0] >= 6 && g.N[1] >= 6;
  const int gkind = step_graph_kind(rk, (ok || ok2d) && nsteps >= 2);
  if (gkind && nsteps >= 3) {
    StepGraph* sg = static_cast<StepGraph*>(rk->step_graph);
    if (!sg) rk->step_graph = sg = new StepGraph();
    int rc, done = 0;
    if ((rc = gkind == 1 ? chain_step(rk, visc, u, dt, s, 2) : ins_rk_step_f64(rk, visc, u, t, dt, nullptr, stream))) return rc;
    done = 1;
    const int last_direct = gkind == 1 ? 1 : 0;
    const int nreplay = nsteps - done - last_direct;
// ... 213 lines not shown
```

incompressiblenavierstokes.jl_amd/csrc/ins_rk_ext.hip:

```cpp
#include <cstring>
#include <vector>

#include "ins_internal.h"

int ins_k_momentum_generic(const ins_grid* G, double visc, const double* u, double* F, hipStream_t s);
int ins_k_momentum_fast3d_opts(const ins_grid* G, double visc, const double* u, double* F, bool zero_shell, hipStream_t s);
int ins_k_momentum_rk_fused(const ins_grid* G, double visc, const double* u_in, double* k_out, const RkEpi& epi, hipStream_t s);
int ins_k_project_periodic_fused(const ins_grid* G, ins_poisson* ps, double* u, double* p, bool keep_p, hipStream_t s, double* uout = nullptr);
int ins_k_project(const ins_grid* G, ins_poisson* ps, double* u, double* p, hipStream_t s);
bool ins_fast3d_supported(const ins_grid* G);
bool ins_flux64_supported(const ins_grid* G);
int ins_k_temp_stage(const ins_grid* G, double a4, double coef, const double* u, const double* temp, const double* w, const double* tempstart, int n,
                     const double* coefs, const double* const* ks, double c_self, double* ktemp_out, double* temp_out, hipStream_t s, const double* pI,
                     const double* diff = nullptr);
int ins_k_diffusion_overwrite(const ins_grid* G, double visc, const double* u, double* F, hipStream_t s);
bool ins_flux64m_supported(const ins_grid* G);
bool ins_smagforce_supported(const ins_grid* G);
int ins_k_smagforce(const ins_grid* G, double theta, const double* u, const double* pI, double* sout, hipStream_t s);
int ins_k_diffusion_flux3d(const ins_grid* G, double visc, const double* u, double* F, bool zero_shell, hipStream_t s);
int ins_k_momentum_rk_fused_corr(const ins_grid* G, double visc, const double* ustar_prev, const double* pI, double* k_out, const RkEpi& epi, hipStream_t s);
int ins_k_project_periodic_solve_only(const ins_grid* G, ins_poisson* ps, const double* u, hipStream_t s);
int ins_k_smagtensor_corr(const ins_grid* G, double theta, const double* ustar, const double* pI, double* sig, hipStream_t s);

struct ins_rk_ext {
  int closure = 0;
  double theta = 0.0;
  bool temp_on = false;
  ins_temperature_desc_t td;
  double* sigma = nullptr;
  double* E = nullptr;
  double* diff = nullptr;
  double* tempstart = nullptr;
  double* w = nullptr;
  double* tb[2] = {nullptr, nullptr};
  std::vector<double*> ktemp;
};

void ins_rk_ext_free(ins_rk_ext* e) {
  if (!e) return;
  for (double* p : {e->sigma, e->E, e->diff, e->tempstart, e->w, e->tb[0], e->tb[1]})
    if (p) (void)hipFree(p);
  for (double* p : e->ktemp)
    if (p) (void)hipFree(p);
  delete e;
}

static ins_rk_ext* ext_of(ins_rk* rk) {
  if (!rk->ext) rk->ext = new ins_rk_ext();
  return rk->ext;
}

extern "C" int ins_rk_set_closure(ins_rk_t* rk, int32_t kind, double theta) {
  INS_REQUIRE(rk, "null argument");
  INS_REQUIRE(kind == 0 || kind == 1, "closure kind: 0 (none) or 1 (Smagorinsky)");
  ins_rk_ext* e = ext_of(rk);
  e->closure = kind;
  e->theta = theta;
  return INS_OK;
}

extern "C" int ins_rk_set_temperature(ins_rk_t* rk, const ins_temperature_desc_t* desc) {
  INS_REQUIRE(rk, "null argument");
  ins_rk_ext* e = ext_of(rk);
  e->temp_on = desc != nullptr;
  if (desc) {
    INS_REQUIRE(desc->gdir >= 0 && desc->gdir < rk->grid->g.D, "gdir out of range");
    e->td = *desc;
  }
  return INS_OK;
}

static long long g_fused_steps = 0, g_tiled_steps = 0;
extern "C" long long ins_dbg_ext_tiled_steps(void) { return g_tiled_steps; }
extern "C" long long ins_dbg_ext_fused_steps(void) { return g_fused_steps; }

static int zalloc(double** p, size_t bytes, hipStream_t s) {
  if (*p) return INS_OK;
  INS_HIP_TRY(hipMalloc(p, bytes));
  INS_HIP_TRY(hipMemsetAsync(*p, 0, bytes, s));
  return INS_OK;
}

extern "C" int ins_rk_step_ext_f64(ins_rk_t* rk, double visc, double* u, double* temp, double t, double dt, void* stream) {
  INS_REQUIRE(rk && u, "null argument");
  ins_rk_ext* e = rk->ext;
  const bool closure = e && e->closure == 1, with_temp = e && e->temp_on;
  INS_REQUIRE(with_temp == (temp != nullptr), "a temperature field needs ins_rk_set_temperature and vice versa");
  if (!closure && !with_temp) return ins_rk_step_f64(rk, visc, u, t, dt, nullptr, stream);
  const ins_grid* G = rk->grid;
  const GridDev& g = G->g;
  hipStream_t s = as_stream(stream);
  const int ns = rk->nstage, D = g.D;
  const size_t sbytes = (size_t)G->ncell * sizeof(double), vbytes = sbytes * D;
  int rc;
  auto need_sigma = [&]() { return zalloc(&e->sigma, sbytes * (D * (D + 1) / 2), s); };
  if (closure && (rc = zalloc(&e->E, vbytes, s))) return rc;
  if (with_temp) {
    if ((rc = zalloc(&e->tempstart, sbytes, s))) return rc;
    if (e->td.dodissipation && (rc = zalloc(&e->diff, vbytes, s))) return rc;
    if ((int)e->ktemp.size() < ns) e->ktemp.resize(ns, nullptr);
    for (int i = 0; i < ns; ++i)
      if ((rc = zalloc(&e->ktemp[i], sbytes, s))) return rc;
    INS_HIP_TRY(hipMemcpyAsync(e->tempstart, temp, sbytes, hipMemcpyDeviceToDevice, s));
  }
  const ins_temperature_desc_t& td = e->td;
  auto bc_temp = [&]() { return with_temp ? ins_apply_bc_temp_f64(G, td.bc, td.val, nullptr, temp, stream) : INS_OK; };
  auto temp_rhs = [&](const double* v, int i) -> int {
    if (!with_temp) return INS_OK;
    int r;
    INS_HIP_TRY(hipMemsetAsync(e->ktemp[i], 0, sbytes, s));
    if ((r = ins_convection_diffusion_temp_f64(G, td.a4, v, temp, e->ktemp[i], stream))) return r;
    if (td.dodissipation && (r = ins_dissipation_f64(G, visc, td.diss_coef, v, e->diff, e->ktemp[i], stream))) return r;
    return INS_OK;
  };
  auto temp_combine = [&](int i) -> int {
    if (!with_temp) return INS_OK;
    double coefs[INS_MAX_STAGES];
    const double* ks[INS_MAX_STAGES];
    int n = 0;
    for (int j = 0; j <= i; ++j) {
      coefs[n] = dt * rk->A[i * ns + j];
      ks[n] = e->ktemp[j];
      ++n;
    }
    return ins_combine_scalar_f64(G, e->tempstart, temp, n, coefs, ks, stream);
  };

  bool fused = !ins_opt(OPT_INS_DISABLE_FUSED_RK) && !ins_opt(OPT_INS_DISABLE_EXT_FUSED) && D == 3 && G->all_periodic && G->all_dof &&
               rk->ps->kind == POISSON_SPECTRAL && ins_fast3d_supported(G) && ins_flux64_supported(G);
  for (int a = 0; fused && a < 3; ++a) fused = rk->ps->np[a] >= 2;

  if (fused) {
    ++g_fused_steps;
    for (int b = 0; b < 2; ++b)
      if ((rc = zalloc(&rk->ub[b], vbytes, s))) return rc;
    if (with_temp) {
      for (int b = 0; b < 2; ++b)
        if ((rc = zalloc(&e->tb[b], sbytes, s))) return rc;
      if (td.dodissipation && (rc = zalloc(&e->w, vbytes, s))) return rc;
    }
    if ((rc = ins_k_apply_bc_u(G, u, 0, nullptr, s))) return rc;
    if ((rc = bc_temp())) return rc;
    bool vbasis = ns > 1 && !ins_opt(OPT_INS_RK_KEEP_K);
    for (int i = 0; vbasis && i < ns; ++i) vbasis = rk->A[i * ns + i] != 0.0;
    const bool tin_kernel = with_temp && !ins_opt(OPT_INS_EXT_TEMP_SPLIT);
    const bool smag1 = closure && ins_smagforce_supported(G);
    const bool incorr = vbasis && !tin_kernel && !ins_opt(OPT_INS_DISABLE_INKERNEL_CORR) && g.N[0] >= 34 && g.N[1] >= 8 && g.N[2] >= 8;
    const double* in = u;
    const double* tin = temp;
    for (int i = 0; i < ns; ++i) {
      const bool last = i == ns - 1 && ns > 1;
      double* out = last ? u : (vbasis ? rk->ku[i] : rk->ub[i & 1]);
      double* corrected = (last || incorr) ? out : rk->ub[i & 1];
      double* tout = with_temp ? (last ? temp : e->tb[i & 1]) : nullptr;
      const bool corr_in = incorr && i > 0;
      if (smag1) {
        if ((rc = ins_k_smagforce(G, e->theta, in, corr_in ? rk->ps->pI : nullptr, e->E, s))) return rc;
      } else if (closure) {
        if ((rc = need_sigma())) return rc;
        rc = corr_in ? ins_k_smagtensor_corr(G, e->theta, in, rk->ps->pI, e->sigma, s) : ins_smagtensor_f64(G, e->theta, in, e->sigma, stream);
        if (rc) return rc;
        if ((rc = ins_k_apply_bc_p_fields(G, e->sigma, D * (D + 1) / 2, s))) return rc;
        if ((rc = ins_divoftensor_f64(G, e->sigma, e->E, stream))) return rc;
      }
      RkEpi epi;
      memset(&epi, 0, sizeof(epi));
      if (vbasis) {
        double beta[INS_MAX_STAGES];
        for (int m = i - 1; m >= 0; --m) {
          double v = rk->A[i * ns + m];
          for (int j = m + 1; j < i; ++j) v -= beta[j] * rk->A[j * ns + m];
          beta[m] = v / rk->A[m * ns + m];
        }
        for (int m = 0; m < i; ++m) {
// ... 228 lines not shown
```

Baseline: 6625 M cell-updates/s.

## Order Poisson x-FFT planes to follow the flux kernel's z-chunk write order

The flux stage kernel now reports its z-chunking (chunk size and k range), and the RK step hands this to the spectral Poisson solve. The forward x-FFT kernel remaps blockIdx.y with a plane permutation so it reads first the z-planes the flux kernel wrote last, which are the most likely to still sit in L2/MALL cache. It also adds an option flag and debug/timing entry points. The cost is a small amount of index arithmetic per block, and the benefit depends on how much of the last-written data actually stays in cache.

New measurement: 6494 M cell-updates/s. 2.0% lower.

```diff
diff --git a/incompressiblenavierstokes.jl_amd/csrc/ins_fast3d_flux.hip b/incompressiblenavierstokes.jl_amd/csrc/ins_fast3d_flux.hip
--- a/incompressiblenavierstokes.jl_amd/csrc/ins_fast3d_flux.hip
+++ b/incompressiblenavierstokes.jl_amd/csrc/ins_fast3d_flux.hip
@@ -510,7 +510,7 @@
 
 bool ins_flux64_supported(const ins_grid* G);
 int ins_k_flux64(const ins_grid* G, double visc, const double* u, double* F, const RkEpi* epi, const double* pI, int corr_mode, hipStream_t s,
-                 int part = 0);
+                 int part = 0, StageChunks* chunks = nullptr);
 
 int ins_k_momentum_flux3d(const ins_grid* G, double visc, const double* u, double* F, bool zero_shell, hipStream_t s) {
   int rc;
@@ -564,8 +564,9 @@
 bool ins_flux64m_supported(const ins_grid* G);
 int ins_k_flux64m(const ins_grid* G, double visc, const double* u, double* k_out, const RkEpi& epi, const double* p_padded, hipStream_t s);
 
-int ins_k_momentum_rk_fused(const ins_grid* G, double visc, const double* u_in, double* k_out, const RkEpi& epi, hipStream_t s) {
-  if (ins_flux64_supported(G)) return ins_k_flux64(G, visc, u_in, k_out, &epi, nullptr, 0, s);
+int ins_k_momentum_rk_fused(const ins_grid* G, double visc, const double* u_in, double* k_out, const RkEpi& epi, hipStream_t s, StageChunks* chunks) {
+  if (chunks) *chunks = StageChunks();
+  if (ins_flux64_supported(G)) return ins_k_flux64(G, visc, u_in, k_out, &epi, nullptr, 0, s, 0, chunks);
   if ((!ins_opt(OPT_INS_FLUX64M_SKIP_FIRST) || epi.wout) && ins_flux64m_supported(G)) return ins_k_flux64m(G, visc, u_in, k_out, epi, nullptr, s);
   int rc = ins_flux3d_prepare(G, visc, s);
   if (rc) return rc;
@@ -573,8 +574,9 @@
 }
 
 int ins_k_momentum_rk_fused_corr(const ins_grid* G, double visc, const double* ustar_prev, const double* pI, double* k_out, const RkEpi& epi,
-                                 hipStream_t s) {
-  if (ins_flux64_supported(G)) return ins_k_flux64(G, visc, ustar_prev, k_out, &epi, pI, 1, s);
+                                 hipStream_t s, StageChunks* chunks) {
+  if (chunks) *chunks = StageChunks();
+  if (ins_flux64_supported(G)) return ins_k_flux64(G, visc, ustar_prev, k_out, &epi, pI, 1, s, 0, chunks);
   int rc = ins_flux3d_prepare(G, visc, s);
   if (rc) return rc;
   return launch_flux_any<true>(G, ustar_prev, k_out, epi, pI, 1, s);
diff --git a/incompressiblenavierstokes.jl_amd/csrc/ins_fft.hip b/incompressiblenavierstokes.jl_amd/csrc/ins_fft.hip
--- a/incompressiblenavierstokes.jl_amd/csrc/ins_fft.hip
+++ b/incompressiblenavierstokes.jl_amd/csrc/ins_fft.hip
@@ -1,3 +1,4 @@
+#include <atomic>
 #include <cmath>
 
 #include "ins_internal.h"
@@ -308,9 +309,26 @@
     }
 }
 
+__host__ __device__ inline int xfwd_plane(int b, int n2, int zc) {
+  if (zc <= 0 || zc >= n2) return zc > 0 ? n2 - 1 - b : b;
+  const int nfull = n2 / zc, rem = n2 - nfull * zc;
+  const int head = (zc - rem) * nfull;
+  int m, c;
+  if (b < head) {
+    const int q = b / nfull;
+    m = zc - 1 - q;
+    c = b - q * nfull;
+  } else {
+    const int bb = b - head, q = bb / (nfull + 1);
+    m = rem - 1 - q;
+    c = bb - q * (nfull + 1);
+  }
+  return c * zc + m;
+}
+
 template <int LOGN, int NP, int SRC, typename C = double2>
 __global__ __launch_bounds__(256) void k_xfwd(GridDev g, const double* __restrict__ src, C* __restrict__ out, int n1,
-                                              const C* __restrict__ tw_g, int kxs, int kz0, int skel) {
+                                              const C* __restrict__ tw_g, int kxs, int kz0, int skel, int order_zc) {
   using T = real_t<C>;
   constexpr int N = fft_len(LOGN);
   constexpr int KXN = N / 2 + 1;
@@ -319,7 +337,7 @@
   C* buf = lds_dyn;
   C* tw = lds_dyn + NP * N;
   const int t = threadIdx.x;
-  const int kz = kz0 + blockIdx.y;
+  const int kz = kz0 + (SRC == 1 ? xfwd_plane((int)blockIdx.y, (int)gridDim.y, order_zc) : (int)blockIdx.y);
   const int j0 = blockIdx.x * 2 * NP;
   constexpr bool SWZ = fft_swz_on<LOGN>();
   for (int m = t; m < N; m += 256) tw[fft_swz<SWZ>(m)] = tw_g[m];
@@ -621,26 +639,31 @@
   return INS_OK;
 }
 
+static std::atomic<int> g_xfwd_last_zc{0};
+extern "C" int ins_dbg_xfwd_last_zc(void) { return g_xfwd_last_zc.load(); }
+
 template <int LOGN>
-int launch_xfwd(const GridDev& g, const double* src, int from_u, double2* out, int n1, int n2, const double2* tw, int kxs, hipStream_t s, int kz0) {
+int launch_xfwd(const GridDev& g, const double* src, int from_u, double2* out, int n1, int n2, const double2* tw, int kxs, hipStream_t s, int kz0, int order_zc) {
   constexpr int N = fft_len(LOGN);
   constexpr int NP = fft_r3(LOGN) == 5 ? 640 / N : (fft_r3(LOGN) == 3 ? 768 / N : (N >= 1024 ? 2 : (1024 / N > 16 ? 16 : 1024 / N)));
   constexpr size_t lds = ((size_t)NP * N + N) * sizeof(double2);
   dim3 grid((n1 + 2 * NP - 1) / (2 * NP), n2);
+  if (from_u != 1 || kz0 != 0 || order_zc < 0) order_zc = 0;
+  g_xfwd_last_zc.store(order_zc);
   if (from_u == 6)
-    hipLaunchKernelGGL((k_xfwd<LOGN, NP, 6>), grid, dim3(256), lds, s, g, src, out, n1, tw, kxs, kz0, (int)ins_opt(OPT_INS_X_SKEL));
+    hipLaunchKernelGGL((k_xfwd<LOGN, NP, 6>), grid, dim3(256), lds, s, g, src, out, n1, tw, kxs, kz0, (int)ins_opt(OPT_INS_X_SKEL), 0);
   else if (from_u == 5)
-    hipLaunchKernelGGL((k_xfwd<LOGN, NP, 5>), grid, dim3(256), lds, s, g, src, out, n1, tw, kxs, kz0, (int)ins_opt(OPT_INS_X_SKEL));
+    hipLaunchKernelGGL((k_xfwd<LOGN, NP, 5>), grid, dim3(256), lds, s, g, src, out, n1, tw, kxs, kz0, (int)ins_opt(OPT_INS_X_SKEL), 0);
   else if (from_u == 4)
-    hipLaunchKernelGGL((k_xfwd<LOGN, NP, 4>), grid, dim3(256), lds, s, g, src, out, n1, tw, kxs, kz0, (int)ins_opt(OPT_INS_X_SKEL));
+    hipLaunchKernelGGL((k_xfwd<LOGN, NP, 4>), grid, dim3(256), lds, s, g, src, out, n1, tw, kxs, kz0, (int)ins_opt(OPT_INS_X_SKEL), 0);
   else if (from_u == 3)
-    hipLaunchKernelGGL((k_xfwd<LOGN, NP, 3>), grid, dim3(256), lds, s, g, src, out, n1, tw, kxs, kz0, (int)ins_opt(OPT_INS_X_SKEL));
+    hipLaunchKernelGGL((k_xfwd<LOGN, NP, 3>), grid, dim3(256), lds, s, g, src, out, n1, tw, kxs, kz0, (int)ins_opt(OPT_INS_X_SKEL), 0);
   else if (from_u == 2)
-    hipLaunchKernelGGL((k_xfwd<LOGN, NP, 2>), grid, dim3(256), lds, s, g, src, out, n1, tw, kxs, kz0, (int)ins_opt(OPT_INS_X_SKEL));
+    hipLaunchKernelGGL((k_xfwd<LOGN, NP, 2>), grid, dim3(256), lds, s, g, src, out, n1, tw, kxs, kz0, (int)ins_opt(OPT_INS_X_SKEL), 0);
   else if (from_u)
-    hipLaunchKernelGGL((k_xfwd<LOGN, NP, 1>), grid, dim3(256), lds, s, g, src, out, n1, tw, kxs, kz0, (int)ins_opt(OPT_INS_X_SKEL));
+    hipLaunchKernelGGL((k_xfwd<LOGN, NP, 1>), grid, dim3(256), lds, s, g, src, out, n1, tw, kxs, kz0, (int)ins_opt(OPT_INS_X_SKEL), order_zc);
   else
-    hipLaunchKernelGGL((k_xfwd<LOGN, NP, 0>), grid, dim3(256), lds, s, g, src, out, n1, tw, kxs, kz0, (int)ins_opt(OPT_INS_X_SKEL));
+    hipLaunchKernelGGL((k_xfwd<LOGN, NP, 0>), grid, dim3(256), lds, s, g, src, out, n1, tw, kxs, kz0, (int)ins_opt(OPT_INS_X_SKEL), 0);
   INS_LAUNCH_CHECK();
   return INS_OK;
 }
@@ -652,9 +675,9 @@
   dim3 grid((n1 + 2 * NP - 1) / (2 * NP), n2);
   const double* srcd = reinterpret_cast<const double*>(src);
   if (from_u)
-    hipLaunchKernelGGL((k_xfwd<LOGN, NP, 5, float2>), grid, dim3(256), lds, s, g, srcd, out, n1, tw, kxs, 0, (int)ins_opt(OPT_INS_X_SKEL));
+    hipLaunchKernelGGL((k_xfwd<LOGN, NP, 5, float2>), grid, dim3(256), lds, s, g, srcd, out, n1, tw, kxs, 0, (int)ins_opt(OPT_INS_X_SKEL), 0);
   else
-    hipLaunchKernelGGL((k_xfwd<LOGN, NP, 0, float2>), grid, dim3(256), lds, s, g, srcd, out, n1, tw, kxs, 0, (int)ins_opt(OPT_INS_X_SKEL));
+    hipLaunchKernelGGL((k_xfwd<LOGN, NP, 0, float2>), grid, dim3(256), lds, s, g, srcd, out, n1, tw, kxs, 0, (int)ins_opt(OPT_INS_X_SKEL), 0);
   INS_LAUNCH_CHECK();
   return INS_OK;
 }
@@ -1395,13 +1418,13 @@
 }
 
 int ins_k_ownfft_xfwd(const ins_grid* G, const double* src, int from_u, double* phat, int n0, int n1, int n2, const double* tw,
-                      hipStream_t s, int kxs, int kz0) {
+                      hipStream_t s, int kxs, int kz0, int order_zc) {
   if (kxs <= 0) kxs = n0 / 2 + 1;
   static const GridDev no_grid{};
   const GridDev& g = G ? G->g : no_grid;
   double2* out = reinterpret_cast<double2*>(phat);
   const double2* w = reinterpret_cast<const double2*>(tw);
-#define CALL(LG) launch_xfwd<LG>(g, src, from_u, out, n1, n2, w, kxs, s, kz0)
+#define CALL(LG) launch_xfwd<LG>(g, src, from_u, out, n1, n2, w, kxs, s, kz0, order_zc)
   INS_POW2_SWITCH(n0, CALL)
 #undef CALL
 }
diff --git a/incompressiblenavierstokes.jl_amd/csrc/ins_flux64.hip b/incompressiblenavierstokes.jl_amd/csrc/ins_flux64.hip
--- a/incompressiblenavierstokes.jl_amd/csrc/ins_flux64.hip
+++ b/incompressiblenavierstokes.jl_amd/csrc/ins_flux64.hip
@@ -559,7 +559,7 @@
 
 constexpr int ZB = 4;
 template <typename T, int R, int XW, bool FUSE, int NW = 4>
-int launch(const ins_grid* G, FluxArgs& a, int corr_mode, int part, hipStream_t s) {
+int launch(const ins_grid* G, FluxArgs& a, int corr_mode, int part, hipStream_t s, StageChunks* chunks) {
   const GridDev& g = G->g;
   a.ntx = cdiv(g.N[0] - 2, 64 * XW);
   a.nty = cdiv(g.N[1] - 2, (NW / XW) * R);
@@ -579,7 +579,13 @@
     a.kB = nzl + 1 - ZB;
   }
   a.ntz = part == 2 ? 2 : cdiv(a.k_hi - a.k_lo, a.zc);
-  return launch_range<T, R, XW, FUSE, NW>(G, a, corr_mode, s);
+  const int rc = launch_range<T, R, XW, FUSE, NW>(G, a, corr_mode, s);
+  if (rc == INS_OK && chunks && part == 0 && sizeof(T) == 8 && corr_mode != 2) {
+    chunks->zc = a.zc;
+    chunks->k_lo = a.k_lo;
+    chunks->k_hi = a.k_hi;
+  }
+  return rc;
 }
 
 }
@@ -601,7 +607,8 @@
 }
 
 template <typename T>
-static int flux64_dispatch(const ins_grid* G, double visc, const T* u, T* F, const RkEpi* epi, const T* pI, int corr_mode, hipStream_t s, int part) {
+static int flux64_dispatch(const ins_grid* G, double visc, const T* u, T* F, const RkEpi* epi, const T* pI, int corr_mode, hipStream_t s, int part,
+                           StageChunks* chunks = nullptr) {
   const GridDev& g = G->g;
   FluxArgs a;
   memset(&a, 0, sizeof(a));
@@ -675,19 +682,19 @@
     if (rows == RR) {                                                                 \
       if constexpr (RR == 2 && !F32) {                                                \
         if (nw == 16) {                                                               \
-          if (xw == 4) return launch<T, RR, 4, FUSE, 16>(G, a, corr_mode, part, s);   \
-          if (xw == 2) return launch<T, RR, 2, FUSE, 16>(G, a, corr_mode, part, s);   \
-          return launch<T, RR, 1, FUSE, 16>(G, a, corr_mode, part, s);                \
+          if (xw == 4) return launch<T, RR, 4, FUSE, 16>(G, a, corr_mode, part, s, chunks);   \
+          if (xw == 2) return launch<T, RR, 2, FUSE, 16>(G, a, corr_mode, part, s, chunks);   \
+          return launch<T, RR, 1, FUSE, 16>(G, a, corr_mode, part, s, chunks);                \
         }                                                                             \
       }                                                                               \
       if (nw >= 8) {                                                                  \
-        if (xw == 4) return launch<T, RR, 4, FUSE, 8>(G, a, corr_mode, part, s);      \
-        if (xw == 2) return launch<T, RR, 2, FUSE, 8>(G, a, corr_mode, part, s);      \
-        return launch<T, RR, 1, FUSE, 8>(G, a, corr_mode, part, s);                   \
+        if (xw == 4) return launch<T, RR, 4, FUSE, 8>(G, a, corr_mode, part, s, chunks);      \
+        if (xw == 2) return launch<T, RR, 2, FUSE, 8>(G, a, corr_mode, part, s, chunks);      \
+        return launch<T, RR, 1, FUSE, 8>(G, a, corr_mode, part, s, chunks);                   \
       }                                                                               \
-      if (xw == 4) return launch<T, RR, 4, FUSE>(G, a, corr_mode, part, s);           \
-      if (xw == 2) return launch<T, RR, 2, FUSE>(G, a, corr_mode, part, s);           \
-      return launch<T, RR, 1, FUSE>(G, a, corr_mode, part, s);                        \
+      if (xw == 4) return launch<T, RR, 4, FUSE>(G, a, corr_mode, part, s, chunks);           \
+      if (xw == 2) return launch<T, RR, 2, FUSE>(G, a, corr_mode, part, s, chunks);           \
+      return launch<T, RR, 1, FUSE>(G, a, corr_mode, part, s, chunks);                        \
     }                                                                                 \
   }
   if (epi) {
@@ -712,9 +719,9 @@
 int ins_k_flux128_f32(const ins_grid* G, double visc, const float* u, float* F, const RkEpi* epi, const float* pI, int corr_mode, hipStream_t s, int part);
 
 int ins_k_flux64(const ins_grid* G, double visc, const double* u, double* F, const RkEpi* epi, const double* pI, int corr_mode, hipStream_t s,
-                 int part) {
+                 int part, StageChunks* chunks) {
   if (ins_flux128_supported(G, epi, corr_mode, false)) return ins_k_flux128(G, visc, u, F, epi, pI, corr_mode, s, part);
-  return flux64_dispatch<double>(G, visc, u, F, epi, pI, corr_mode, s, part);
+  return flux64_dispatch<double>(G, visc, u, F, epi, pI, corr_mode, s, part, chunks);
 }
 int ins_k_flux64_f32(const ins_grid* G, double visc, const float* u, float* F, const RkEpi* epi, const float* pI, int corr_mode, hipStream_t s,
                      int part) {
diff --git a/incompressiblenavierstokes.jl_amd/csrc/ins_internal.h b/incompressiblenavierstokes.jl_amd/csrc/ins_internal.h
--- a/incompressiblenavierstokes.jl_amd/csrc/ins_internal.h
+++ b/incompressiblenavierstokes.jl_amd/csrc/ins_internal.h
@@ -117,6 +117,7 @@
   X(INS_DISABLE_CORR2D)          \
   X(INS_SPECTRUM_ROCFFT)         \
   X(INS_X_SKEL)                  \
+  X(INS_XFWD_PLANE_ORDER)        \
   X(INS_LINE3_TK)                \
   X(INS_LINE3_WGS)               \
   X(INS_STEP_GRAPH)              \
@@ -298,13 +299,18 @@
 int ins_k_applypressure(const ins_grid* grid, double* u, const double* p, hipStream_t s);
 int ins_k_laplacian(const ins_grid* grid, const double* p, double* L, hipStream_t s);
 int ins_k_project(const ins_grid* grid, ins_poisson* ps, double* u, double* p, hipStream_t s);
-int ins_k_momentum_rk_fused(const ins_grid* G, double visc, const double* u_in, double* k_out, const RkEpi& epi, hipStream_t s);
+struct StageChunks {
+  int zc = 0;
+  int k_lo = 0;
+  int k_hi = 0;
+};
+int ins_k_momentum_rk_fused(const ins_grid* G, double visc, const double* u_in, double* k_out, const RkEpi& epi, hipStream_t s, StageChunks* chunks = nullptr);
 bool ins_flux2d_supported(const ins_grid* G);
 int ins_k_flux2d(const ins_grid* G, double visc, const double* u, double* F, const RkEpi* epi, hipStream_t s, const double* pI = nullptr);
 int ins_k_project_periodic_solve_only_2d(const ins_grid* G, ins_poisson* ps, const double* u, hipStream_t s);
 int ins_k_momentum_rk_fused_generic(const ins_grid* G, double visc, const double* u_in, double* k_out, const RkEpi& epi, hipStream_t s);
 int ins_k_momentum_rk_fused_corr(const ins_grid* G, double visc, const double* ustar_prev, const double* pI, double* k_out, const RkEpi& epi,
-                                 hipStream_t s);
+                                 hipStream_t s, StageChunks* chunks = nullptr);
 int ins_k_momentum_rk_fused_corr_slab(const ins_grid* G, double visc, const double* ustar_prev, const double* p_ext, double* k_out,
                                       const RkEpi& epi, hipStream_t s, int part = 0);
 bool ins_corr3_supported(const ins_grid* G);
@@ -314,7 +320,9 @@
 int ins_k_project_fdm_solve_only(const ins_grid* G, ins_poisson* ps, const double* u, double* p, hipStream_t s);
 int ins_k_project_periodic_fused_2d(const ins_grid* G, ins_poisson* ps, double* u, double* p, bool keep_p, hipStream_t s);
 bool ins_poisson_own2d(const ins_poisson* ps);
-int ins_k_project_periodic_solve_only(const ins_grid* G, ins_poisson* ps, const double* u, hipStream_t s);
+int ins_k_project_periodic_solve_only(const ins_grid* G, ins_poisson* ps, const double* u, hipStream_t s, const StageChunks* chunks = nullptr);
+int ins_k_project_periodic_fused(const ins_grid* G, ins_poisson* ps, double* u, double* p, bool keep_p, hipStream_t s, double* uout = nullptr,
+                                 const StageChunks* chunks = nullptr);
 int ins_k_poisson_solve(ins_poisson* ps, double* p, hipStream_t s);
 int ins_k_reduce(const ins_grid* grid, int op, const double* a, const double* b, const int lo[3], const int hi[3], double* out,
                  hipStream_t s);
@@ -328,7 +336,7 @@
 bool ins_ownfft_supported_mixed(const int np[3]);
 void ins_ownfft_permute_symbol(int n, const double* ay, double* out);
 int ins_k_ownfft_xfwd(const ins_grid* G, const double* src, int from_u, double* phat, int n0, int n1, int n2, const double* tw, hipStream_t s,
-                      int kxs = 0, int kz0 = 0);
+                      int kxs = 0, int kz0 = 0, int order_zc = 0);
 int ins_k_ownfft_xinv(const double* phat, double* pI, int n0, int n1, int n2, const double* tw, hipStream_t s, int kxs = 0);
 int ins_k_ownfft_y(double* phat, int kxn, int n1, int n2, const double* tw, bool inverse, hipStream_t s, int kxs = 0);
 bool ins_ownfft_xy_supported(int n0, int n1);
diff --git a/incompressiblenavierstokes.jl_amd/csrc/ins_options.hip b/incompressiblenavierstokes.jl_amd/csrc/ins_options.hip
--- a/incompressiblenavierstokes.jl_amd/csrc/ins_options.hip
+++ b/incompressiblenavierstokes.jl_amd/csrc/ins_options.hip
@@ -18,9 +18,16 @@
 
 std::atomic<long long> g_epoch{0};
 
-long long from_env(const char* name) {
+long long default_of(int id) {
+  switch (id) {
+    case OPT_INS_XFWD_PLANE_ORDER: return 0;
+    default: return 0;
+  }
+}
+
+long long from_env(const char* name, long long dflt) {
   const char* v = getenv(name);
-  if (!v) return 0;
+  if (!v) return dflt;
   if (!*v) return 1;
   char* end = nullptr;
   const long long x = strtoll(v, &end, 10);
@@ -35,7 +42,7 @@
 long long ins_opt(int id) {
   Opt& o = g_opts[id];
   if (o.state.load(std::memory_order_acquire) == 0) {
-    o.value.store(from_env(o.name), std::memory_order_relaxed);
+    o.value.store(from_env(o.name, default_of(id)), std::memory_order_relaxed);
     o.state.store(1, std::memory_order_release);
   }
   return o.value.load(std::memory_order_relaxed);
diff --git a/incompressiblenavierstokes.jl_amd/csrc/ins_poisson.hip b/incompressiblenavierstokes.jl_amd/csrc/ins_poisson.hip
--- a/incompressiblenavierstokes.jl_amd/csrc/ins_poisson.hip
+++ b/incompressiblenavierstokes.jl_amd/csrc/ins_poisson.hip
@@ -810,7 +810,13 @@
   return INS_OK;
 }
 
-static int ownfft_transform(ins_poisson* ps, const double* from_u, hipStream_t s, int src_code = 1) {
+static int xfwd_order_zc(const ins_poisson* ps, const StageChunks* chunks) {
+  if (!chunks || chunks->zc <= 0 || ins_opt(OPT_INS_XFWD_PLANE_ORDER) != 1) return 0;
+  if (chunks->k_lo != 1 || chunks->k_hi != ps->np[2] + 1) return 0;
+  return chunks->zc;
+}
+
+static int ownfft_transform(ins_poisson* ps, const double* from_u, hipStream_t s, int src_code = 1, const StageChunks* chunks = nullptr) {
   const int n0 = ps->np[0], n1 = ps->np[1], n2 = ps->np[2], kxn = ps->kmax[0], kxs = ps->kxs;
   double* ph = reinterpret_cast<double*>(ps->phat);
   int rc;
@@ -827,7 +833,8 @@
     if ((rc = ins_k_zsolve(ph, n2, (long long)kxs * n1, ps->ahat[0], kxn, ps->ahat[1], ps->ahat[2], ps->tw, inv_n, true, s, kxs))) return rc;
     return ins_k_ownfft_xy(nullptr, nullptr, 0, ph, ps->pI, n0, n1, n2, ps->tw_x, ps->tw_y, true, s, kxs);
   }
-  if ((rc = ins_k_ownfft_xfwd(ps->grid, from_u ? from_u : ps->pI, from_u ? src_code : 0, ph, n0, n1, n2, ps->tw_x, s, kxs))) return rc;
+  const int order_zc = (from_u && src_code == 1) ? xfwd_order_zc(ps, chunks) : 0;
+  if ((rc = ins_k_ownfft_xfwd(ps->grid, from_u ? from_u : ps->pI, from_u ? src_code : 0, ph, n0, n1, n2, ps->tw_x, s, kxs, 0, order_zc))) return rc;
   if (ps->yz_P && !ins_opt(OPT_INS_DISABLE_YZ_FUSED)) {
     const ins_grid* G = ps->grid;
     const double c = G->h[0] * G->h[1] / G->h[2];
@@ -1363,13 +1370,13 @@
   return ins_k_applypressure(G, u, p, s);
 }
 
-int ins_k_project_periodic_fused(const ins_grid* G, ins_poisson* ps, double* u, double* p, bool keep_p, hipStream_t s, double* uout) {
+int ins_k_project_periodic_fused(const ins_grid* G, ins_poisson* ps, double* u, double* p, bool keep_p, hipStream_t s, double* uout, const StageChunks* chunks) {
   const GridDev& g = G->g;
   dim3 block(64, 4, 1), grid(cdiv(ps->np[0], 64), cdiv(ps->np[1], 4), ps->np[2]);
   int rc;
   double* dst = uout ? uout : u;
   if (ps->ownfft) {
-    rc = ownfft_transform(ps, u, s);
+    rc = ownfft_transform(ps, u, s, 1, chunks);
   } else {
     hipLaunchKernelGGL((k_div_to_pI<3, true>), grid, block, 0, s, g, u, ps->pI, ps->np[0], ps->np[1]);
     INS_LAUNCH_CHECK();
@@ -1417,9 +1424,9 @@
 
 bool ins_poisson_own2d(const ins_poisson* ps) { return ps->kind == POISSON_SPECTRAL && ps->ownfft && ps->grid->g.D == 2; }
 
-int ins_k_project_periodic_solve_only(const ins_grid* G, ins_poisson* ps, const double* u, hipStream_t s) {
+int ins_k_project_periodic_solve_only(const ins_grid* G, ins_poisson* ps, const double* u, hipStream_t s, const StageChunks* chunks) {
   const GridDev& g = G->g;
-  if (ps->ownfft) return ownfft_transform(ps, u, s);
+  if (ps->ownfft) return ownfft_transform(ps, u, s, 1, chunks);
   dim3 block(64, 4, 1), grid(cdiv(ps->np[0], 64), cdiv(ps->np[1], 4), ps->np[2]);
   hipLaunchKernelGGL((k_div_to_pI<3, true>), grid, block, 0, s, g, u, ps->pI, ps->np[0], ps->np[1]);
   INS_LAUNCH_CHECK();
@@ -1451,6 +1458,43 @@
   return ins_k_ownfft_xinv_f32(phat32, pI32, n0, n1, n2, twx, s, kxs32);
 }
 
+extern "C" int ins_dbg_poisson_xfwd(const ins_grid_t* G, ins_poisson_t* ps, const double* u, int zc, int k_lo, int k_hi, double* ms, void* stream) {
+  INS_REQUIRE(G && ps && u, "null argument");
+  INS_REQUIRE(ps->grid == G && ps->kind == POISSON_SPECTRAL && ps->ownfft && G->g.D == 3, "own-FFT spectral solver of this 3-D grid needed");
+  hipStream_t s = as_stream(stream);
+  StageChunks ch;
+  ch.zc = zc;
+  ch.k_lo = k_lo;
+  ch.k_hi = k_hi;
+  hipEvent_t e0 = nullptr, e1 = nullptr;
+  if (ms) {
+    INS_HIP_TRY(hipEventCreate(&e0));
+    INS_HIP_TRY(hipEventCreate(&e1));
+    INS_HIP_TRY(hipEventRecord(e0, s));
+  }
+  const int rc = ins_k_ownfft_xfwd(G, u, 1, reinterpret_cast<double*>(ps->phat), ps->np[0], ps->np[1], ps->np[2], ps->tw_x, s, ps->kxs, 0, xfwd_order_zc(ps, &ch));
+  if (ms) {
+    float t = 0.f;
+    INS_HIP_TRY(hipEventRecord(e1, s));
+    INS_HIP_TRY(hipEventSynchronize(e1));
+    INS_HIP_TRY(hipEventElapsedTime(&t, e0, e1));
+    INS_HIP_TRY(hipEventDestroy(e0));
+    INS_HIP_TRY(hipEventDestroy(e1));
+    *ms = t;
+  }
+  return rc;
+}
+extern "C" long long ins_dbg_poisson_copy(const ins_poisson_t* ps, int which, double* out, long long n, void* stream) {
+  if (!ps || ps->kind != POISSON_SPECTRAL || ps->grid->g.D != 3) return -1;
+  const long long planes = (long long)ps->np[1] * ps->np[2];
+  const long long len = which == 0 ? 2LL * (ps->ownfft ? ps->kxs : ps->kmax[0]) * planes : (long long)ps->np[0] * planes;
+  if (!out) return len;
+  if (n < len) return -1;
+  const void* srcp = which == 0 ? static_cast<const void*>(ps->phat) : static_cast<const void*>(ps->pI);
+  if (hipMemcpyAsync(out, srcp, (size_t)len * sizeof(double), hipMemcpyDeviceToDevice, as_stream(stream)) != hipSuccess) return -1;
+  return len;
+}
+
 extern "C" int ins_project_f64(const ins_grid_t* G, ins_poisson_t* ps, double* u, double* p, void* stream) {
   INS_REQUIRE(G && ps && u && p, "null argument");
   INS_REQUIRE(ps->grid == G, "psolver was created for a different grid");
diff --git a/incompressiblenavierstokes.jl_amd/csrc/ins_rk.hip b/incompressiblenavierstokes.jl_amd/csrc/ins_rk.hip
--- a/incompressiblenavierstokes.jl_amd/csrc/ins_rk.hip
+++ b/incompressiblenavierstokes.jl_amd/csrc/ins_rk.hip
@@ -9,8 +9,6 @@
 bool ins_fast3d_supported(const ins_grid* G);
 bool ins_flux64_supported(const ins_grid* G);
 
-int ins_k_momentum_rk_fused(const ins_grid* G, double visc, const double* u_in, double* k_out, const RkEpi& epi, hipStream_t s);
-int ins_k_project_periodic_fused(const ins_grid* G, ins_poisson* ps, double* u, double* p, bool keep_p, hipStream_t s, double* uout = nullptr);
 
 int ins_k_momentum(const ins_grid* G, double visc, const double* u, double* F, hipStream_t s) {
   if (ins_fast3d_supported(G)) return ins_k_momentum_fast3d(G, visc, u, F, s);
@@ -248,21 +246,55 @@
       INS_HIP_TRY(hipEventCreate(&e1));
       INS_HIP_TRY(hipEventRecord(e0, s));
     }
-    rc = (inkernel && (i > 0 || raw_in)) ? ins_k_momentum_rk_fused_corr(G, visc, in, rk->ps->pI, rk->ku[i], epi, s)
-                             : ins_k_momentum_rk_fused(G, visc, in, rk->ku[i], epi, s);
+    StageChunks chunks;
+    rc = (inkernel && (i > 0 || raw_in)) ? ins_k_momentum_rk_fused_corr(G, visc, in, rk->ps->pI, rk->ku[i], epi, s, &chunks)
+                             : ins_k_momentum_rk_fused(G, visc, in, rk->ku[i], epi, s, &chunks);
     if (rc) return rc;
     if (rk->profiling) {
       INS_HIP_TRY(hipEventRecord(e1, s));
       rk->prof_events.push_back(e0);
       rk->prof_events.push_back(e1);
     }
-    rc = (inkernel && (i < ns - 1 || raw_out)) ? ins_k_project_periodic_solve_only(G, rk->ps, out, s)
-                                               : ins_k_project_periodic_fused(G, rk->ps, out, rk->p, i == ns - 1, s);
+    rc = (inkernel && (i < ns - 1 || raw_out)) ? ins_k_project_periodic_solve_only(G, rk->ps, out, s, &chunks)
+                                               : ins_k_project_periodic_fused(G, rk->ps, out, rk->p, i == ns - 1, s, nullptr, &chunks);
     if (rc) return rc;
     in = out;
   }
   if (ns == 1) INS_HIP_TRY(hipMemcpyAsync(u, rk->ub[0], vbytes, hipMemcpyDeviceToDevice, s));
   return INS_OK;
+}
+
+extern "C" int ins_dbg_rk_stage_pair_ms(ins_rk_t* rk, double visc, double dt, int reps, double* ms, void* stream) {
+  INS_REQUIRE(rk && ms && reps > 0, "null argument");
+  INS_REQUIRE(rk->vb.size() >= 3 && rk->vb[0] && rk->vb[1] && rk->vb[2] && rk->ps && rk->ps->pI && ins_flux64_supported(rk->grid),
+              "run an RK44 step on the 64-wide stage kernels first");
+  const ins_grid* G = rk->grid;
+  hipStream_t s = as_stream(stream);
+  RkEpi epi;
+  memset(&epi, 0, sizeof(epi));
+  epi.c0m1 = -1.0;
+  epi.self_in = 1.0;
+  epi.coef_self = 0.5 * dt;
+  epi.ustart = rk->vb[2];
+  epi.ustar = rk->vb[1];
+  hipEvent_t e0, e1;
+  INS_HIP_TRY(hipEventCreate(&e0));
+  INS_HIP_TRY(hipEventCreate(&e1));
+  INS_HIP_TRY(hipEventRecord(e0, s));
+  int rc = INS_OK;
+  for (int r = 0; r < reps && rc == INS_OK; ++r) {
+    StageChunks chunks;
+    rc = ins_k_momentum_rk_fused_corr(G, visc, rk->vb[0], rk->ps->pI, rk->ku[1], epi, s, &chunks);
+    if (rc == INS_OK) rc = ins_k_project_periodic_solve_only(G, rk->ps, rk->vb[1], s, &chunks);
+  }
+  float t = 0.f;
+  INS_HIP_TRY(hipEventRecord(e1, s));
+  INS_HIP_TRY(hipEventSynchronize(e1));
+  INS_HIP_TRY(hipEventElapsedTime(&t, e0, e1));
+  INS_HIP_TRY(hipEventDestroy(e0));
+  INS_HIP_TRY(hipEventDestroy(e1));
+  *ms = t / reps;
+  return rc;
 }
 
 static int rk_step_fused_periodic_2d(ins_rk* rk, double visc, double* u, double dt, hipStream_t s, int chain = 0) {
diff --git a/incompressiblenavierstokes.jl_amd/csrc/ins_rk_ext.hip b/incompressiblenavierstokes.jl_amd/csrc/ins_rk_ext.hip
--- a/incompressiblenavierstokes.jl_amd/csrc/ins_rk_ext.hip
+++ b/incompressiblenavierstokes.jl_amd/csrc/ins_rk_ext.hip
@@ -5,8 +5,6 @@
 
 int ins_k_momentum_generic(const ins_grid* G, double visc, const double* u, double* F, hipStream_t s);
 int ins_k_momentum_fast3d_opts(const ins_grid* G, double visc, const double* u, double* F, bool zero_shell, hipStream_t s);
-int ins_k_momentum_rk_fused(const ins_grid* G, double visc, const double* u_in, double* k_out, const RkEpi& epi, hipStream_t s);
-int ins_k_project_periodic_fused(const ins_grid* G, ins_poisson* ps, double* u, double* p, bool keep_p, hipStream_t s, double* uout = nullptr);
 int ins_k_project(const ins_grid* G, ins_poisson* ps, double* u, double* p, hipStream_t s);
 bool ins_fast3d_supported(const ins_grid* G);
 bool ins_flux64_supported(const ins_grid* G);
@@ -18,8 +16,6 @@
 bool ins_smagforce_supported(const ins_grid* G);
 int ins_k_smagforce(const ins_grid* G, double theta, const double* u, const double* pI, double* sout, hipStream_t s);
 int ins_k_diffusion_flux3d(const ins_grid* G, double visc, const double* u, double* F, bool zero_shell, hipStream_t s);
-int ins_k_momentum_rk_fused_corr(const ins_grid* G, double visc, const double* ustar_prev, const double* pI, double* k_out, const RkEpi& epi, hipStream_t s);
-int ins_k_project_periodic_solve_only(const ins_grid* G, ins_poisson* ps, const double* u, hipStream_t s);
 int ins_k_smagtensor_corr(const ins_grid* G, double theta, const double* ustar, const double* pI, double* sig, hipStream_t s);
 
 struct ins_rk_ext {
```
